# riveSunder/therldaisyworld

Hardware: AMD Instinct MI355X
Metric: cell-updates/sec (grid x batch), fused stencil+growth step (higher is better)
Workload: dtype f32

## Files before the change

### therldaisyworld_amd/csrc/dw_api.hip

```cpp
#include <hip/hip_runtime.h>

#include <cmath>
#include <cstdarg>
#include <cstdio>
#include <cstdlib>
#include <cstring>
#include <memory>
#include <new>
#include <optional>
#include <type_traits>
#include <vector>

#include "../../include/daisyworld_hip.h"
#include "dw_kernels.hpp"
#include "dw_host_util.hpp"
#include "dw_plan.hpp"
#include "dw_series.hpp"
#include "dw_episode_staging.hpp"

using namespace dw;

static thread_local char g_err[512] = "";

static int fail(int code, const char* fmt, ...) {
    va_list ap;
    va_start(ap, fmt);
    vsnprintf(g_err, sizeof(g_err), fmt, ap);
    va_end(ap);
    return code;
}

#define HIPCHK(expr)                                                                           \
    do {                                                                                       \
        hipError_t e_ = (expr);                                                                \
        if (e_ != hipSuccess)                                                                  \
            return fail(e_ == hipErrorOutOfMemory ? DW_ENOMEM : DW_EHIP, "%s failed: %s (%s:%d)", \
                        #expr, hipGetErrorString(e_), __FILE__, __LINE__);                      \
    } while (0)

#define NEED(cond, code, ...)                      \
    do {                                           \
        if (!(cond)) return fail(code, __VA_ARGS__); \
    } while (0)

enum UnqKind { UNQ_F64 = 1, UNQ_F32 = 2 };
enum UnqOwner { OWN_NONE = 0, OWN_CUR = 1, OWN_PREV = 2 };

static thread_local int t_fail_in = 0;
struct DeviceMem {
    static int alloc(void** p, size_t n) {
        if (t_fail_in > 0 && --t_fail_in == 0) return hipErrorOutOfMemory;
        return hipMalloc(p, n);
    }
    static int release(void* p) { return hipFree(p); }
};
struct PinnedMem {
    static int alloc(void** p, size_t n) { return hipHostMalloc(p, n, hipHostMallocDefault); }
    static int release(void* p) { return hipHostFree(p); }
};
template <class T> using DevBuf = Buf<T, DeviceMem>;
template <class T> using PinnedBuf = Buf<T, PinnedMem>;

struct dw_handle {
    dw_params prm;
    hipStream_t stream = nullptr;
    bool own_stream = false;
    size_t cells = 0;
    DevBuf<plane_t> L16[2];
    DevBuf<plane_t> D16[2];
    int cur = 0;
    DevBuf<double> L64;
    DevBuf<double> D64;
    DevBuf<float> U32L;
    DevBuf<float> U32D;
    UnqKind unq_kind = UNQ_F64;
    UnqOwner unq = OWN_NONE;
    bool have_state = false;
    bool stepped = false;
    double L_last = 0.0;
    bool L_per_world = false;
    bool P_per_world = false;
    DevBuf<int> idx;
    DevBuf<double> st;
    DevBuf<int> action;
    DevBuf<int> action_tmp;
    bool have_agents = false;
    DevBuf<StatsDev> stats2[2];
    size_t stats_bytes = 0;
    int sp = 0;
    DevBuf<uint4> fixq;
    unsigned int qcap = 0;
    DevBuf<int> redo_tiles;
    Switches sw{};
    StepPlan plan{};
    DevBuf<int> done_at;
    DevBuf<int> agents_done_at;
    DevBuf<int> n_alive;
    DevBuf<double> scratch;
    DevBuf<unsigned char> ep_buf;
    DevBuf<double> mlp_w;
    int mlp_members = 0;
    PinnedBuf<unsigned char> ep_pinned;
    DevBuf<double> reward_d;
    DevBuf<unsigned char> done_d;
    hipEvent_t ev0 = nullptr, ev1 = nullptr;
    hipEvent_t evf0 = nullptr, evf1 = nullptr;
    int fused_launches = 0;
    DevBuf<StatsDev> side_stats;
    DevBuf<StatsDev> trace_d;
    DevBuf<TempStatsDev> temp_d;
    DevBuf<TempPartial> temp_part;
    DevBuf<unsigned char> pw_tab;
    PinnedBuf<unsigned char> pw_pinned;
    PinnedBuf<unsigned char> pinned;
    struct Snapshot {
        DevBuf<plane_t> L, D;
        DevBuf<plane_t> PL, PD;
        bool stepped = false;
        double L_last = 0.0;
        bool L_per_world = false, P_per_world = false;
        UnqOwner unq = OWN_NONE;
        DevBuf<int> idx;
        DevBuf<double> st;
        DevBuf<unsigned char> stats;
        bool valid = false, agents = false;
    } snap[DW_SNAPSHOT_SLOTS];
    std::vector<std::pair<const void*, size_t>> lds_limit;
    bool created = false;
};

static inline bool cur_quantised(const dw_handle* h) { return h->unq != OWN_CUR; }

static inline bool lacks_shared_L(const dw_handle* h) { return h->stepped && h->L_per_world; }
#define NEED_SHARED_L(h, what)                                                                                          \
    NEED(!lacks_shared_L(h), DW_ESTATE,                                                                                 \
         "%s derives its temperature channels from the last step's luminosity, and the last step "                      \
         "(dw_step_n_trace_per_world) took a per-world luminosity: take a shared-L step or upload a state first", what)
static inline bool lacks_shared_constants(const dw_handle* h) { return lacks_shared_L(h) && h->P_per_world; }
#define NEED_SHARED_CONSTANTS(h, what)                                                                                  \
    NEED(!lacks_shared_constants(h), DW_ESTATE,                                                                         \
         "%s evaluates the last step's input state with one set of constants, and the last step "                       \
         "(dw_step_n_trace_ensemble) took per-world constants: take a shared-L step or upload a state first", what)

template <int V> using int_c = std::integral_constant<int, V>;

template <int V, int... Vs, class F>
static decltype(auto) with_int(int v, F&& f) {
    if constexpr (sizeof...(Vs) == 0) return f(int_c<V>{});
    else return v == V ? f(int_c<V>{}) : with_int<Vs...>(v, f);
}

template <class F>
static decltype(auto) with_bool(bool b, F&& f) { return b ? f(std::true_type{}) : f(std::false_type{}); }

template <class P> using elem_t = std::remove_cv_t<std::remove_pointer_t<P>>;

template <class F>
static decltype(auto) with_unq_planes(const dw_handle* h, F&& f) {
    return h->unq_kind == UNQ_F64 ? f(h->L64.get(), h->D64.get()) : f(h->U32L.get(), h->U32D.get());
}

template <class F>
static decltype(auto) with_planes(const dw_handle* h, bool unq, int buf, F&& f) {
    return unq ? with_unq_planes(h, f) : f(h->L16[buf].get(), h->D16[buf].get());
// ... 225 lines not shown
    }
    return DW_OK;
}

static dim3 generic_grid(const dw_params& p, int* cpt) {
    *cpt = generic_cells_per_thread(p.batch, (long long)p.height * p.width);
    return dim3((unsigned)(((long long)p.height * p.width + 256LL * *cpt - 1) / (256LL * *cpt)), (unsigned)p.batch);
}

template <class T, int PREC>
static auto launch_generic(dw_handle* h, const T* iL, const T* iD, const StepOut& o, const FirstStepBound& fb = {}) {
    const dw_params& p = h->prm;
    int cpt;
    const dim3 grid = generic_grid(p, &cpt);
    hipLaunchKernelGGL((step_generic<T, PREC>), grid, dim3(256), 0, h->stream, iL, iD, o.L, o.D, p.height, p.width, o.P, o.P64,
                       o.stats, o.fixups, o.zero_me, o.zero_n, cpt, fb);
}

static int launch_first_step(dw_handle* h, double L, const StepOut& o) {
    const StepPlan& pl = h->plan;
    const FirstStepBound fb = pl.first_prec == 3 ? derive_first_bound(h->prm, L, o.P, h->unq_kind == UNQ_F64, h->sw.first_slack)
                                                 : FirstStepBound{};
    if (pl.first_stream) {
        const dim3 grid((unsigned)((pl.first_geom.nstrips + 3) / 4));
        with_unq_planes(h, [&](auto* iL, auto* iD) {
            with_int<1, 3>(pl.first_prec, [&](auto PR) {
                with_int<0, 1, 2, 3>(pl.halo, [&](auto HL) {
                    hipLaunchKernelGGL((step_first_stream<elem_t<decltype(iL)>, PR, HL>), grid, dim3(256), 0, h->stream, iL, iD,
                                       o.L, o.D, pl.first_geom, o.P, o.P64, o.stats, o.fixups, o.zero_me, o.zero_n, fb);
                });
            });
        });
    } else {
        with_unq_planes(h, [&](auto* iL, auto* iD) {
            with_int<1, 3, 2>(pl.first_prec, [&](auto PR) { launch_generic<elem_t<decltype(iL)>, PR>(h, iL, iD, o, fb); });
        });
    }
    HIPCHK(hipGetLastError());
    return DW_OK;
}

static int launch_step(dw_handle* h, const StepOut& o) {
    const dw_params& p = h->prm;
    const StepPlan& pl = h->plan;
    const plane_t* iL = h->L16[h->cur].get();
    const plane_t* iD = h->D16[h->cur].get();
    const bool ex = p.precision == DW_PRECISION_EXACT;
    if (pl.kind == STEP_GENERIC) {
        const int prec = p.precision == DW_PRECISION_F64 ? 2 : (ex ? 0 : 1);
        with_int<2, 0, 1>(prec, [&](auto PR) { launch_generic<plane_t, PR>(h, iL, iD, o); });
    } else if (pl.kind == STEP_STREAM && ex) {
        const StreamExactArgs A{iL, iD, o.L, o.D, pl.sgeom, o.P, o.stats, o.fixups, o.zero_me, o.zero_n, o.P64};
        with_int<0, 1, 2, 3>(pl.halo, [&](auto HL) {
            with_bool(pl.sym_albedo, [&](auto SYM) {
                hipLaunchKernelGGL((step_stream_exact<HL, SYM>), dim3((unsigned)pl.sgeom.chunk * 8u), dim3(256), 0, h->stream, A);
            });
        });
    } else if (pl.kind == STEP_STREAM) {
        with_int<0, 1, 2, 3>(pl.halo, [&](auto HL) {
            hipLaunchKernelGGL((step_stream_fast<HL>), dim3((unsigned)pl.sgeom.chunk * 8u), dim3(256), 0, h->stream, iL, iD, o.L,
                               o.D, pl.sgeom, o.P, o.P64, o.stats, o.fixups, o.zero_me, o.zero_n);
        });
    } else {
        FixQ fq;
        fq.entries = h->fixq.get();
        fq.counts = reinterpret_cast<unsigned int*>(o.stats + p.batch + 1);
        fq.qcap = h->qcap;
        fq.redo_tiles = h->redo_tiles.get();
        auto tiled = [&](auto TCQ, auto RPT) {
            return with_bool(ex, [&](auto EX) { return launch_tiled<TCQ, RPT, EX>(h, iL, iD, o, fq); });
        };
        if (pl.tcq == 64) return with_int<8, 4, 2>(pl.rpt, [&](auto RPT) { return tiled(int_c<64>{}, RPT); });
        return pl.tcq == 32 ? tiled(int_c<32>{}, int_c<4>{}) : tiled(int_c<16>{}, int_c<2>{});
    }
    HIPCHK(hipGetLastError());
    return DW_OK;
}

static void step_done(dw_handle* h, double L, bool stepped, bool per_world = false, bool per_world_constants = false) {
    h->cur = 1 - h->cur;
    h->sp = 1 - h->sp;
    h->unq = h->unq == OWN_CUR ? OWN_PREV : OWN_NONE;
    h->stepped = stepped;
    h->L_last = L;
    h->L_per_world = per_world;
    h->P_per_world = per_world && per_world_constants;
    release_unquantised(h);
}

static void episode_done(dw_handle* h, double L_last, bool per_world) {
    h->unq = OWN_NONE;
    h->stepped = true;
    h->L_last = per_world ? 0.0 : L_last;
    h->L_per_world = per_world;
    h->P_per_world = per_world;
}

static int launch_forward(dw_handle* h, double L) {
    const dw_params& p = h->prm;
    NEED(h->have_state, DW_ESTATE, "no state uploaded (call dw_upload_state_* or dw_init_random)");
    StepOut o = step_out(h);
    o.P = derive_f32(p, L);
    o.P64 = make_f64(p, L);
#ifdef DW_TUNING
    if (const char* e = std::getenv("DW_ABLATE")) {
        if (std::strcmp(e, "copy") == 0) {
            const int in = h->cur;
            const size_t n4 = h->cells * sizeof(plane_t) / 16;
            hipLaunchKernelGGL(copy_planes, dim3((unsigned)((n4 + 255) / 256)), dim3(256), 0, h->stream,
                               reinterpret_cast<const float4*>(h->L16[in].get()), reinterpret_cast<const float4*>(h->D16[in].get()),
                               reinterpret_cast<float4*>(o.L), reinterpret_cast<float4*>(o.D), n4);
            HIPCHK(hipGetLastError());
            step_done(h, L, true);
            return DW_OK;
        }
        const int v = std::strcmp(e, "nomath") == 0 ? 1 : 0;
        HIPCHK(hipMemcpyToSymbolAsync(HIP_SYMBOL(g_ablate), &v, sizeof(int), 0, hipMemcpyHostToDevice, h->stream));
    }
#endif
    if (int rc = h->unq == OWN_CUR ? launch_first_step(h, L, o) : launch_step(h, o)) return rc;
    step_done(h, L, true);
    return DW_OK;
}

static int launch_forward_pw(dw_handle* h, const PhysF32* row32, const PhysF64* row64, const FirstStepBound* rowfb, bool sym,
                             bool constants) {
    const dw_params& p = h->prm;
    const StepPlan& pl = h->plan;
    const StepOut o = step_out(h);
    const bool ex = p.precision == DW_PRECISION_EXACT;
    auto generic = [&](auto* iL, auto* iD, auto PR) {
        int cpt;
        const dim3 grid = generic_grid(p, &cpt);
        hipLaunchKernelGGL((step_generic_pw<elem_t<decltype(iL)>, PR>), grid, dim3(256), 0, h->stream, iL, iD, o.L, o.D,
                           p.height, p.width, row32, row64, rowfb, o.stats, o.fixups, o.zero_me, o.zero_n, cpt);
    };
    const plane_t* iL = h->L16[h->cur].get();
    const plane_t* iD = h->D16[h->cur].get();
    if (h->unq == OWN_CUR) {
        with_unq_planes(h, [&](auto* uL, auto* uD) {
            with_int<1, 3, 2>(pl.first_prec, [&](auto PR) { generic(uL, uD, PR); });
        });
    } else if (pl.pw_stream && ex) {
        const StreamExactPwArgs A{iL, iD, o.L, o.D, pl.sgeom, row32, row64, o.stats, o.fixups, o.zero_me, o.zero_n};
        with_int<0, 1, 2>(pl.halo, [&](auto HL) {
            with_bool(sym, [&](auto SYM) {
                hipLaunchKernelGGL((step_stream_exact_pw<HL, SYM>), dim3((unsigned)pl.sgeom.chunk * 8u), dim3(256), 0, h->stream, A);
            });
        });
    } else if (pl.pw_stream) {
        with_int<0, 1, 2>(pl.halo, [&](auto HL) {
            hipLaunchKernelGGL((step_stream_fast_pw<HL>), dim3((unsigned)pl.sgeom.chunk * 8u), dim3(256), 0, h->stream, iL, iD, o.L,
                               o.D, pl.sgeom, row32, row64, o.stats, o.fixups, o.zero_me, o.zero_n);
        });
    } else {
        const int prec = p.precision == DW_PRECISION_F64 ? 2 : (ex ? 0 : 1);
        with_int<2, 0, 1>(prec, [&](auto PR) { generic(iL, iD, PR); });
    }
    HIPCHK(hipGetLastError());
    step_done(h, 0.0, true, true, constants);
    return DW_OK;
}

static int launch_forward_fused2_pw(dw_handle* h, const PairPw* row, StatsDev* trace) {
    const StepPlan& pl = h->plan;
    const StepOut o = step_out(h);
    const FusedGeom& g = pl.fgeom;
    const dim3 grid((unsigned)g.chunk * 8u);
    const plane_t *inL = h->L16[h->cur].get(), *inD = h->D16[h->cur].get();
    with_int<kFusedRot, kFusedOvl>(pl.fused_mode, [&](auto MODE) {
        hipLaunchKernelGGL((trace_pair_fast_pw<MODE>), grid, dim3(256), 0, h->stream, inL, inD, o.L, o.D, g, row, o.zero_me,
                           o.zero_n, trace);
    });
    HIPCHK(hipGetLastError());
    step_done(h, 0.0, false, true, true);
    return DW_OK;
}

static int temp_chunks(const dw_handle* h) {
    return (int)(((long long)h->prm.height * h->prm.width + kTempChunk - 1) / kTempChunk);
}
static size_t temp_part_bytes(const dw_handle* h) { return sizeof(TempPartial) * (size_t)h->prm.batch * temp_chunks(h); }

static int launch_temp_moments(dw_handle* h, bool current, double L, const PhysF64* row64, TempStatsDev* out) {
    const dw_params& p = h->prm;
    const int chunks = temp_chunks(h);
    const PhysF64 P = row64 ? PhysF64{} : make_f64(p, L);
    TempPartial* part = h->temp_part.get();
    auto reduce = [&](auto* iL, auto* iD) {
        with_bool(row64 != nullptr, [&](auto TABLE) {
            hipLaunchKernelGGL((temp_moments_pw<elem_t<decltype(iL)>, TABLE>), dim3((unsigned)chunks, (unsigned)p.batch), dim3(256),
                               0, h->stream, iL, iD, p.height, p.width, P, row64, part);
        });
    };
    if (current) with_planes(h, h->unq == OWN_CUR, h->cur, reduce);
    else with_derived_from(h, [&](auto* iL, auto* iD, auto) { reduce(iL, iD); });
    HIPCHK(hipGetLastError());
    hipLaunchKernelGGL(temp_moments_finish_pw, dim3((unsigned)((p.batch + 63) / 64)), dim3(64), 0, h->stream, part, p.batch, chunks,
                       (double)p.height * (double)p.width, out);
    HIPCHK(hipGetLastError());
    return DW_OK;
}

template <class F>
static auto with_fused_layout(const StepPlan& pl, F&& f) {
    if (pl.packed) return f(int_c<kFusedRot>{}, std::true_type{});
    return with_int<kFusedRot, kFusedRing, kFusedOvl>(pl.fused_mode, [&](auto MODE) { return f(MODE, std::false_type{}); });
}

static int launch_forward_fused2(dw_handle* h, double L1, double L2, unsigned int* pstats = nullptr,
                                 float thr_hi = 0.f, StatsDev* trace = nullptr) {
    const dw_params& p = h->prm;
    const StepPlan& pl = h->plan;
    const bool exact = p.precision == DW_PRECISION_EXACT;
    PhysF32 P1, P2;
    if (exact) derive_f32_pair(p, L1, L2, &P1, &P2);
    else { P1 = derive_f32(p, L1); P2 = derive_f32(p, L2); }
    const StepOut o = step_out(h);
    const FusedGeom& g = pl.fgeom;
    const dim3 grid((unsigned)g.chunk * 8u);
    const plane_t *inL = h->L16[h->cur].get(), *inD = h->D16[h->cur].get();
    auto exact_args = [&] {
        return FusedExactArgs{inL, inD, o.L, o.D, g, P1, lum_part(P2), o.zero_me, o.zero_n, pstats, thr_hi, make_f64(p, L1), L1, L2};
    };
    if (trace && exact) {
        const TraceExactArgs A{exact_args(), trace, h->sw.force_rescan ? 1 : 0};
        with_int<kFusedRot, kFusedOvl>(pl.fused_mode, [&](auto MODE) {
            with_bool(pl.sym_albedo, [&](auto SYM) {
                hipLaunchKernelGGL((trace_pair_exact<MODE, SYM>), grid, dim3(256), 0, h->stream, A);
            });
        });
    } else if (trace) {
        with_int<kFusedRot, kFusedOvl>(pl.fused_mode, [&](auto MODE) {
            hipLaunchKernelGGL((trace_pair_fast<MODE>), grid, dim3(256), 0, h->stream, inL, inD, o.L, o.D, g, P1, P2, o.zero_me,
                               o.zero_n, trace);
        });
    } else if (pl.seam_strips && !pstats && !exact) {
        const FusedGeom &gs = pl.seam_geom, &gl = pl.left_geom;
        hipLaunchKernelGGL(step_stream_fused2_seam_pw, dim3((unsigned)gs.chunk * 8u), dim3(256), 0, h->stream, inL, inD, o.L, o.D,
                           gs, P1, P2, o.zero_me, o.zero_n);
        if (gl.nstrips)
            hipLaunchKernelGGL(step_stream_fused2_left_pw, dim3((unsigned)gl.chunk * 8u), dim3(256), 0, h->stream, inL, inD, o.L,
                               o.D, gl, P1, P2, o.zero_me, 0);
    } else if (pl.fmt_planes && !pstats && !exact) {
        hipLaunchKernelGGL((step_stream_fused2_fmt_pw<kFusedOvl>), grid, dim3(256), 0, h->stream, inL, inD, o.L, o.D, g, P1, P2,
                           o.zero_me, o.zero_n);
    } else if (exact) {
        const FusedExactArgs A = exact_args();
        with_bool(pstats != nullptr, [&](auto STATS) {
            with_fused_layout(pl, [&](auto MODE, auto PACK) {
                with_bool(pl.sym_albedo, [&](auto SYM) {
                    hipLaunchKernelGGL((step_stream_fused2_exact<MODE, PACK, STATS, SYM>), grid, dim3(256), 0, h->stream, A);
                });
            });
        });
    } else {
        with_bool(pstats != nullptr, [&](auto STATS) {
            with_fused_layout(pl, [&](auto MODE, auto PACK) {
                hipLaunchKernelGGL((step_stream_fused2<MODE, PACK, STATS>), grid, dim3(256), 0, h->stream, inL, inD, o.L, o.D, g,
                                   P1, P2, o.zero_me, o.zero_n, pstats, thr_hi);
            });
        });
    }
    HIPCHK(hipGetLastError());
    step_done(h, L2, false);
    return DW_OK;
}

static int launch_agents(dw_handle* h, const int* d_action, int act_b, int act_n, bool standalone = false,
                         double* d_reward = nullptr, unsigned char* d_done = nullptr, unsigned char* d_ok = nullptr) {
    const dw_params& p = h->prm;
    if (p.n_agents == 0) return DW_OK;
    NEED(h->have_state, DW_ESTATE, "no state uploaded");
    NEED(h->have_agents, DW_ESTATE, "no agents uploaded (call dw_upload_agents or dw_init_random)");
    NEED(p.collision_mode == 0 || standalone, DW_EINVAL,
         "collision_mode=1: call dw_update_agents, apply the collision pass (it consumes the caller's RNG) to the "
         "downloaded agent states, upload them, then dw_step without actions");
    const int blocks = (p.batch + 63) / 64;
    with_planes(h, h->unq == OWN_CUR, h->cur, [&](auto* L, auto* D) {
        using T = elem_t<decltype(L)>;
        hipLaunchKernelGGL(agents_update<T>, dim3(blocks), dim3(64), 0, h->stream, L, D, h->idx.get(), h->st.get(), d_action,
                           act_b, act_n, p.batch, p.n_agents, p.height, p.width, p.agent_gamma,
                           p.collision_mode == 0 ? 1 : 0, d_reward, d_done, d_ok);
    });
    HIPCHK(hipGetLastError());
    return DW_OK;
}

static int stage_host_actions(dw_handle* h, const int32_t* action, int b, int n) {
    const dw_params& p = h->prm;
    NEED(b >= 0 && n >= 0 && b <= p.batch && n <= p.n_agents, DW_EINVAL,
         "action block %dx%d exceeds (B,N)=(%d,%d)", b, n, p.batch, p.n_agents);
    if ((size_t)b * n)
        HIPCHK(hipMemcpyAsync(h->action_tmp.get(), action, sizeof(int) * (size_t)b * n, hipMemcpyHostToDevice,
                              h->stream));
    return DW_OK;
}

static int clear_stats(dw_handle* h) {
    for (int i = 0; i < 2; ++i) HIPCHK(hipMemsetAsync(h->stats2[i].get(), 0, h->stats_bytes, h->stream));
    return DW_OK;
}

static void state_arrived(dw_handle* h, UnqOwner unq, UnqKind kind = UNQ_F64) {
    if (unq == OWN_CUR) h->unq_kind = kind;
    h->unq = unq;
    h->have_state = true;
    h->stepped = false;
    for (auto& sn : h->snap) sn.valid = false;
}

template <class T>
static auto init_random_into(dw_handle* h, uint64_t seed, T* L, T* D) {
    const dw_params& p = h->prm;
    if (int crc = clear_stats(h)) return crc;
    const int ncell = p.height * p.width;
    const dim3 g((unsigned)((ncell + kInitChunk - 1) / kInitChunk), (unsigned)p.batch);
    hipLaunchKernelGGL((init_random_cells<T>), g, dim3(256), 0, h->stream, L, D, ncell,
                       (long long)p.world_offset, (unsigned long long)seed, (float)p.light_proportion,
                       (float)p.dark_proportion, (float)p.initial_al, (float)p.initial_ad, h->stats2[h->sp].get());
    HIPCHK(hipGetLastError());
    if (p.n_agents) {
        const int bn = p.batch * p.n_agents;
        hipLaunchKernelGGL(init_random_agents, dim3((bn + 255) / 256), dim3(256), 0, h->stream, h->idx.get(), h->st.get(),
                           p.batch, p.n_agents, p.height, p.width, (long long)p.world_offset,
                           (unsigned long long)seed);
        HIPCHK(hipGetLastError());
    }
    h->have_agents = true;
    return (int)DW_OK;
}

extern "C" {

const char* dw_last_error(void) { return g_err; }
int dw_abi_version(void) { return DW_ABI_VERSION; }

int dw_pinned_alloc(size_t bytes, void** out) {
    NEED(out && bytes > 0, DW_EINVAL, "null argument");
    int ndev = 0;
    NEED(hipGetDeviceCount(&ndev) == hipSuccess && ndev > 0, DW_ENODEVICE, "no HIP device");
    HIPCHK(hipHostMalloc(out, bytes, hipHostMallocDefault));
    return DW_OK;
}
int dw_pinned_free(void* p) {
    if (p) HIPCHK(hipHostFree(p));
    return DW_OK;
}

#ifndef DW_BUILD_ID
#define DW_BUILD_ID "unknown"
#endif
static const char kBuildId[] = "DW_BUILD_ID=" DW_BUILD_ID;
const char* dw_build_id(void) { return kBuildId + 12; }

int dw_default_params(dw_params* p, int32_t batch, int32_t height, int32_t width, int32_t n_agents) {
    NEED(p, DW_EINVAL, "null params");
    std::memset(p, 0, sizeof(*p));
    p->abi_version = DW_ABI_VERSION;
    p->batch = batch; p->height = height; p->width = width; p->n_agents = n_agents;
    p->device = 0; p->precision = DW_PRECISION_EXACT; p->obs_mask = 0x0BA; p->collision_mode = 0;
    p->world_offset = 0;
    p->p = 1.0; p->g = 0.003265; p->S = 1000.0; p->sigma = 5.67e-8; p->gamma = 0.25;
    p->q = 0.2 * p->S / p->sigma; p->q2 = p->q / 8.0; p->dt = 1.0;
    p->albedo_bare = 0.5; p->albedo_light = 0.75; p->albedo_dark = 0.25; p->temp_optimal = 295.5;
    p->agent_gamma = 0.05; p->food_chain_penalty = 0.5;
    p->initial_al = 0.2; p->initial_ad = 0.2; p->light_proportion = 0.33; p->dark_proportion = 0.33;
    return DW_OK;
}

static int check_params(const dw_params* p) {
    NEED(p, DW_EINVAL, "null params");
    NEED(p->abi_version == DW_ABI_VERSION, DW_EINVAL, "ABI version %d != %d", p->abi_version, DW_ABI_VERSION);
    NEED(p->batch >= 1 && p->height >= 3 && p->width >= 3, DW_EINVAL,
         "need batch>=1 and grid >= 3x3 (got B=%d H=%d W=%d)", p->batch, p->height, p->width);
    NEED(p->height <= 65535 && p->width <= 65532, DW_EINVAL, "grid dimension too large");
    NEED((long long)p->height * p->width <= 0x7fffffffLL, DW_EINVAL,
         "a world of %dx%d cells exceeds the 2^31-1 cells per world the kernels index", p->height, p->width);
    NEED(p->n_agents >= 0, DW_EINVAL, "n_agents < 0");
    NEED(p->precision >= 0 && p->precision <= 2, DW_EINVAL, "bad precision %d", p->precision);
    NEED(p->precision == DW_PRECISION_F64 || p->g >= 0.0, DW_EINVAL,
         "g < 0 (a growth curve opening upwards) is evaluated by DW_PRECISION_F64 only");
    NEED((double)p->batch * p->height * p->width < 9.0e18, DW_EINVAL, "too many cells");
    return DW_OK;
}

int dw_create(const dw_params* p, dw_handle** out) {
    NEED(out, DW_EINVAL, "null out");
    *out = nullptr;
    int rc = check_params(p);
    if (rc) return rc;
    int ndev = 0;
    if (hipGetDeviceCount(&ndev) != hipSuccess || ndev <= 0)
        return fail(DW_ENODEVICE, "no HIP device available (this library has no CPU fallback)");
    NEED(p->device >= 0 && p->device < ndev, DW_ENODEVICE, "device %d out of range (%d devices)", p->device, ndev);
    HIPCHK(hipSetDevice(p->device));
    hipDeviceProp_t prop;
    HIPCHK(hipGetDeviceProperties(&prop, p->device));
    if (std::strncmp(prop.gcnArchName, "gfx950", 6) != 0)
        return fail(DW_ENODEVICE, "device %d is %s; this library is built for gfx950 only", p->device,
                    prop.gcnArchName);
    std::unique_ptr<dw_handle, int (*)(dw_handle*)> h(new (std::nothrow) dw_handle(), dw_destroy);
    NEED(h, DW_ENOMEM, "host allocation failed");
    h->prm = *p;
    h->cells = (size_t)p->batch * p->height * p->width;
    HIPCHK(hipStreamCreateWithFlags(&h->stream, hipStreamNonBlocking));
    h->own_stream = true;
    const size_t bn = (size_t)p->batch * (p->n_agents > 0 ? p->n_agents : 1);
    const size_t pb = sizeof(plane_t) * h->cells;
    h->stats_bytes = sizeof(StatsDev) * (p->batch + 1) + sizeof(unsigned int) * (kNumQueues + 1) * 16;
    if (int rc = alloc_group(h.get(), "the handle's state",
                             {{h->L16[0], pb}, {h->D16[0], pb}, {h->L16[1], pb}, {h->D16[1], pb},
                              {h->idx, sizeof(int) * bn * 2}, {h->st, sizeof(double) * bn}, {h->action, sizeof(int) * bn},
                              {h->action_tmp, sizeof(int) * bn}, {h->reward_d, sizeof(double) * bn}, {h->done_d, bn},
                              {h->agents_done_at, sizeof(int) * bn}, {h->done_at, sizeof(int) * p->batch},
                              {h->n_alive, sizeof(int)}, {h->stats2[0], h->stats_bytes}, {h->stats2[1], h->stats_bytes},
                              {h->side_stats, sizeof(StatsDev) * (p->batch + 1)}}))
        return rc;
    for (int i = 0; i < 2; ++i) HIPCHK(hipMemsetAsync(h->stats2[i].get(), 0, h->stats_bytes, h->stream));
    h->sw = read_switches();
    h->plan = plan_steps(*p, h->sw);
    if (int rc = ensure_fixq(h.get(), h->plan)) return rc;
    HIPCHK(hipMemsetAsync(h->action.get(), 0, sizeof(int) * bn, h->stream));
    HIPCHK(hipMemsetAsync(h->done_at.get(), 0, sizeof(int) * p->batch, h->stream));
    HIPCHK(hipMemsetAsync(h->agents_done_at.get(), 0, sizeof(int) * bn, h->stream));
    HIPCHK(hipMemsetAsync(h->n_alive.get(), 0, sizeof(int), h->stream));
    HIPCHK(hipEventCreate(&h->ev0));
    HIPCHK(hipEventCreate(&h->ev1));
    HIPCHK(hipEventCreate(&h->evf0));
    HIPCHK(hipEventCreate(&h->evf1));
    h->created = true;
    *out = h.release();
    return DW_OK;
}

int dw_destroy(dw_handle* h) {
    if (!h) return DW_OK;
    (void)hipSetDevice(h->prm.device);
    if (h->stream) (void)hipStreamSynchronize(h->stream);
    if (h->ev0) (void)hipEventDestroy(h->ev0);
    if (h->ev1) (void)hipEventDestroy(h->ev1);
    if (h->evf0) (void)hipEventDestroy(h->evf0);
    if (h->evf1) (void)hipEventDestroy(h->evf1);
    if (h->own_stream && h->stream) (void)hipStreamDestroy(h->stream);
    delete h;
    return DW_OK;
}

int dw_set_params(dw_handle* h, const dw_params* p) {
    NEED(h, DW_EINVAL, "null handle");
    int rc = check_params(p);
    if (rc) return rc;
    const dw_params& o = h->prm;
    NEED(p->batch == o.batch && p->height == o.height && p->width == o.width && p->n_agents == o.n_agents &&
             p->device == o.device,
         DW_EINVAL, "dw_set_params cannot change shape or device; create a new handle");
    HIPCHK(hipSetDevice(p->device));
    const StepPlan plan = plan_steps(*p, h->sw);
    if ((rc = ensure_fixq(h, plan))) return rc;
    h->prm = *p;
    h->plan = plan;
    return DW_OK;
}

int dw_get_params(const dw_handle* h, dw_params* out) {
    NEED(h && out, DW_EINVAL, "null argument");
    *out = h->prm;
    return DW_OK;
}


static int refresh_stats(dw_handle* h) {
    const dw_params& p = h->prm;
    if (int rc = clear_stats(h)) return rc;
    const int n = p.height * p.width;
    const dim3 g((unsigned)((n + kInitChunk - 1) / kInitChunk), (unsigned)p.batch);
    auto reduce = [&](auto* L, auto* D) {
        hipLaunchKernelGGL((stats_only<elem_t<decltype(L)>>), g, dim3(256), 0, h->stream, L, D, n, h->stats2[h->sp].get());
    };
    if (cur_quantised(h)) reduce(h->L16[h->cur].get(), h->D16[h->cur].get());
    else with_unq_planes(h, reduce);
    HIPCHK(hipGetLastError());
    return DW_OK;
}

int dw_upload_state_f64(dw_handle* h, const double* light, const double* dark) {
    NEED(h && light && dark, DW_EINVAL, "null argument");
    HIPCHK(hipSetDevice(h->prm.device));
    if (int arc = ensure_f64(h)) return arc;
    HIPCHK(hipMemcpyAsync(h->L64.get(), light, sizeof(double) * h->cells, hipMemcpyHostToDevice, h->stream));
    HIPCHK(hipMemcpyAsync(h->D64.get(), dark, sizeof(double) * h->cells, hipMemcpyHostToDevice, h->stream));
    state_arrived(h, OWN_CUR, UNQ_F64);
    int rc = refresh_stats(h);
    if (rc) return rc;
    HIPCHK(hipStreamSynchronize(h->stream));
    return DW_OK;
}

int dw_upload_state_f32(dw_handle* h, const float* light, const float* dark, int quantised) {
    NEED(h && light && dark, DW_EINVAL, "null argument");
    HIPCHK(hipSetDevice(h->prm.device));
    const unsigned blocks = (unsigned)((h->cells + 255) / 256);
    if (quantised) {
        int rc = ensure_scratch(h, sizeof(float) * 2 * h->cells);
        if (rc) return rc;
        float* sL = reinterpret_cast<float*>(h->scratch.get());
        float* sD = sL + h->cells;
        HIPCHK(hipMemcpyAsync(sL, light, sizeof(float) * h->cells, hipMemcpyHostToDevice, h->stream));
        HIPCHK(hipMemcpyAsync(sD, dark, sizeof(float) * h->cells, hipMemcpyHostToDevice, h->stream));
        hipLaunchKernelGGL(f32nat_to_plane, dim3(blocks), dim3(256), 0, h->stream, sL, h->L16[h->cur].get(), h->cells);
        hipLaunchKernelGGL(f32nat_to_plane, dim3(blocks), dim3(256), 0, h->stream, sD, h->D16[h->cur].get(), h->cells);
        HIPCHK(hipGetLastError());
        state_arrived(h, OWN_NONE);
    } else {
        int rc = ensure_u32(h);
        if (rc) return rc;
        HIPCHK(hipMemcpyAsync(h->U32L.get(), light, sizeof(float) * h->cells, hipMemcpyHostToDevice, h->stream));
        HIPCHK(hipMemcpyAsync(h->U32D.get(), dark, sizeof(float) * h->cells, hipMemcpyHostToDevice, h->stream));
        hipLaunchKernelGGL(f32nat_to_permille, dim3(blocks), dim3(256), 0, h->stream, h->U32L.get(), h->U32L.get(), h->cells);
        hipLaunchKernelGGL(f32nat_to_permille, dim3(blocks), dim3(256), 0, h->stream, h->U32D.get(), h->U32D.get(), h->cells);
        HIPCHK(hipGetLastError());
        state_arrived(h, OWN_CUR, UNQ_F32);
    }
    int rc = refresh_stats(h);
    if (rc) return rc;
    HIPCHK(hipStreamSynchronize(h->stream));
    return DW_OK;
}

int dw_upload_agents(dw_handle* h, const int32_t* indices, const double* states) {
    NEED(h, DW_EINVAL, "null handle");
    const dw_params& p = h->prm;
    HIPCHK(hipSetDevice(p.device));
    const size_t bn = (size_t)p.batch * p.n_agents;
    if (bn) {
        NEED(indices && states, DW_EINVAL, "null argument");
        for (size_t i = 0; i < bn; ++i) {
            NEED(indices[2 * i] >= 0 && indices[2 * i] < p.height && indices[2 * i + 1] >= 0 &&
                     indices[2 * i + 1] < p.width,
                 DW_EINVAL, "agent %zu position (%d,%d) outside the %dx%d grid", i, indices[2 * i],
                 indices[2 * i + 1], p.height, p.width);
        }
        HIPCHK(hipMemcpyAsync(h->idx.get(), indices, sizeof(int) * bn * 2, hipMemcpyHostToDevice, h->stream));
        HIPCHK(hipMemcpyAsync(h->st.get(), states, sizeof(double) * bn, hipMemcpyHostToDevice, h->stream));
        HIPCHK(hipStreamSynchronize(h->stream));
    }
    h->have_agents = true;
    return DW_OK;
}

int dw_download_agents(dw_handle* h, int32_t* indices, double* states) {
    NEED(h, DW_EINVAL, "null handle");
    const dw_params& p = h->prm;
    HIPCHK(hipSetDevice(p.device));
    const size_t bn = (size_t)p.batch * p.n_agents;
    if (bn) {
        NEED(h->have_agents, DW_ESTATE, "no agents");
        if (indices) HIPCHK(hipMemcpyAsync(indices, h->idx.get(), sizeof(int) * bn * 2, hipMemcpyDeviceToHost, h->stream));
        if (states) HIPCHK(hipMemcpyAsync(states, h->st.get(), sizeof(double) * bn, hipMemcpyDeviceToHost, h->stream));
    }
    HIPCHK(hipStreamSynchronize(h->stream));
    return DW_OK;
}

int dw_init_random(dw_handle* h, uint64_t seed) {
    NEED(h, DW_EINVAL, "null handle");
    HIPCHK(hipSetDevice(h->prm.device));
    if (int rc = ensure_u32(h)) return rc;
    if (int rc = init_random_into(h, seed, h->U32L.get(), h->U32D.get())) return rc;
    state_arrived(h, OWN_CUR, UNQ_F32);
    return DW_OK;
}

int dw_init_random_quantised(dw_handle* h, uint64_t seed) {
    NEED(h, DW_EINVAL, "null handle");
    HIPCHK(hipSetDevice(h->prm.device));
    if (int rc = init_random_into(h, seed, h->L16[h->cur].get(), h->D16[h->cur].get())) return rc;
    state_arrived(h, OWN_NONE);
    release_unquantised(h);
    return DW_OK;
}

int dw_download_planes(dw_handle* h, int which, double* light, double* dark) {
    NEED(h, DW_EINVAL, "null handle");
    NEED(h->have_state, DW_ESTATE, "no state");
    HIPCHK(hipSetDevice(h->prm.device));
    NEED(which == DW_STATE_CURRENT || which == DW_STATE_PREVIOUS, DW_EINVAL, "bad state selector");
    NEED(which == DW_STATE_CURRENT || h->stepped, DW_ESTATE, "no previous state before the first step");
    const int buf = which == DW_STATE_CURRENT ? h->cur : 1 - h->cur;
    const bool unq = (which == DW_STATE_CURRENT && h->unq == OWN_CUR) || (which == DW_STATE_PREVIOUS && h->unq == OWN_PREV);
    const size_t bytes = sizeof(double) * h->cells;
    if (unq && h->unq_kind == UNQ_F64) {
        if (light) HIPCHK(hipMemcpyAsync(light, h->L64.get(), bytes, hipMemcpyDeviceToHost, h->stream));
        if (dark) HIPCHK(hipMemcpyAsync(dark, h->D64.get(), bytes, hipMemcpyDeviceToHost, h->stream));
    } else {
        int rc = ensure_scratch(h, bytes);
        if (rc) return rc;
        const unsigned blocks = (unsigned)((h->cells + 255) / 256);
        for (int pl = 0; pl < 2; ++pl) {
            double* dst = pl == 0 ? light : dark;
            if (!dst) continue;
            if (unq)
                hipLaunchKernelGGL((plane_to_f64<float>), dim3(blocks), dim3(256), 0, h->stream,
                                   pl == 0 ? h->U32L.get() : h->U32D.get(), h->scratch.get(), h->cells);
            else
                hipLaunchKernelGGL((plane_to_f64<plane_t>), dim3(blocks), dim3(256), 0, h->stream,
                                   pl == 0 ? h->L16[buf].get() : h->D16[buf].get(), h->scratch.get(), h->cells);
            HIPCHK(hipGetLastError());
            HIPCHK(hipMemcpyAsync(dst, h->scratch.get(), bytes, hipMemcpyDeviceToHost, h->stream));
        }
    }
    HIPCHK(hipStreamSynchronize(h->stream));
    return DW_OK;
}

static int run_materialise(dw_handle* h, double L, double* d_grid7, double* d_temps, double* d_betas,
                           double* d_growth, double* d_teff) {
    const dw_params& p = h->prm;
    const dim3 g((unsigned)((p.height * p.width + 255) / 256), (unsigned)p.batch);
    const PhysF64 P = make_f64(p, h->stepped && !h->L_per_world ? h->L_last : L);
    const plane_t* cL = h->L16[h->cur].get();
    const plane_t* cD = h->D16[h->cur].get();
    with_derived_from(h, [&](auto* pL, auto* pD, auto POST) {
        hipLaunchKernelGGL((materialise<elem_t<decltype(pL)>, POST>), g, dim3(256), 0, h->stream, pL, pD, cL, cD, p.height,
                           p.width, P, d_grid7, d_temps, d_betas, d_growth, d_teff);
    });
    HIPCHK(hipGetLastError());
    if (h->stepped && d_grid7 && p.n_agents && h->have_agents) {
        hipLaunchKernelGGL(agents_stamp, dim3((p.batch + 63) / 64), dim3(64), 0, h->stream, d_grid7, h->idx.get(),
                           h->st.get(), p.batch, p.n_agents, p.height, p.width);
        HIPCHK(hipGetLastError());
    }
    return DW_OK;
}

int dw_download_grid(dw_handle* h, double L_init, double* grid7) {
    NEED(h && grid7, DW_EINVAL, "null argument");
    NEED(h->have_state, DW_ESTATE, "no state");
    NEED_SHARED_L(h, "dw_download_grid");
    HIPCHK(hipSetDevice(h->prm.device));
    const size_t bytes = sizeof(double) * 7 * h->cells;
    int rc = ensure_scratch(h, bytes);
    if (rc) return rc;
    rc = run_materialise(h, L_init, h->scratch.get(), nullptr, nullptr, nullptr, nullptr);
    if (rc) return rc;
    HIPCHK(hipMemcpyAsync(grid7, h->scratch.get(), bytes, hipMemcpyDeviceToHost, h->stream));
    HIPCHK(hipStreamSynchronize(h->stream));
    return DW_OK;
}

int dw_download_caches(dw_handle* h, double L, double* temps, double* betas, double* growth,
                       double* temp_effective) {
    NEED(h, DW_EINVAL, "null handle");
    NEED(h->have_state, DW_ESTATE, "no state");
    NEED_SHARED_CONSTANTS(h, "dw_download_caches");
    HIPCHK(hipSetDevice(h->prm.device));
    const size_t n = h->cells;
    int rc = ensure_scratch(h, sizeof(double) * 9 * n);
    if (rc) return rc;
    double* d_t = h->scratch.get();
    double* d_b = d_t + 3 * n;
    double* d_g = d_b + 3 * n;
    double* d_e = d_g + 2 * n;
    rc = run_materialise(h, L, nullptr, temps ? d_t : nullptr, betas ? d_b : nullptr, growth ? d_g : nullptr,
                         temp_effective ? d_e : nullptr);
    if (rc) return rc;
    if (temps) HIPCHK(hipMemcpyAsync(temps, d_t, sizeof(double) * 3 * n, hipMemcpyDeviceToHost, h->stream));
    if (betas) HIPCHK(hipMemcpyAsync(betas, d_b, sizeof(double) * 3 * n, hipMemcpyDeviceToHost, h->stream));
    if (growth) HIPCHK(hipMemcpyAsync(growth, d_g, sizeof(double) * 2 * n, hipMemcpyDeviceToHost, h->stream));
    if (temp_effective) HIPCHK(hipMemcpyAsync(temp_effective, d_e, sizeof(double) * n, hipMemcpyDeviceToHost, h->stream));
    HIPCHK(hipStreamSynchronize(h->stream));
    return DW_OK;
}

int dw_reduce_temperature(dw_handle* h, double L, dw_temp_stats* per_world) {
    NEED(h && per_world, DW_EINVAL, "null argument");
    NEED(h->have_state, DW_ESTATE, "no state");
    NEED_SHARED_CONSTANTS(h, "dw_reduce_temperature");
    static_assert(sizeof(dw_temp_stats) == sizeof(TempStatsDev), "temperature record layout");
    HIPCHK(hipSetDevice(h->prm.device));
    const size_t bytes = sizeof(TempStatsDev) * (size_t)h->prm.batch;
    if (int rc = alloc_group(h, "the temperature reduction", {{h->temp_part, temp_part_bytes(h)}, {h->temp_d, bytes}})) return rc;
    if (int rc = launch_temp_moments(h, false, h->stepped && !h->L_per_world ? h->L_last : L, nullptr, h->temp_d.get())) return rc;
    HIPCHK(hipMemcpyAsync(per_world, h->temp_d.get(), bytes, hipMemcpyDeviceToHost, h->stream));
    HIPCHK(hipStreamSynchronize(h->stream));
    return DW_OK;
}


int dw_update_agents(dw_handle* h, const int32_t* action, int32_t action_b, int32_t action_n) {
    NEED(h && action, DW_EINVAL, "null argument");
    HIPCHK(hipSetDevice(h->prm.device));
    int rc = stage_host_actions(h, action, action_b, action_n);
    if (rc) return rc;
    return launch_agents(h, h->action_tmp.get(), action_b, action_n, true);
}

int dw_step(dw_handle* h, const int32_t* action, int32_t action_b, int32_t action_n, double L) {
    NEED(h, DW_EINVAL, "null handle");
    HIPCHK(hipSetDevice(h->prm.device));
    if (action) {
        int rc = stage_host_actions(h, action, action_b, action_n);
        if (rc) return rc;
        rc = launch_agents(h, h->action_tmp.get(), action_b, action_n);
        if (rc) return rc;
    }
    return launch_forward(h, L);
}

int dw_step_device_actions(dw_handle* h, double L) {
    NEED(h, DW_EINVAL, "null handle");
    HIPCHK(hipSetDevice(h->prm.device));
    int rc = launch_agents(h, h->action.get(), h->prm.batch, h->prm.n_agents);
    if (rc) return rc;
    return launch_forward(h, L);
}

int dw_upload_actions(dw_handle* h, const int32_t* action) {
    NEED(h && action, DW_EINVAL, "null argument");
    HIPCHK(hipSetDevice(h->prm.device));
    const size_t bn = (size_t)h->prm.batch * h->prm.n_agents;
    if (bn) {
        HIPCHK(hipMemcpyAsync(h->action.get(), action, sizeof(int) * bn, hipMemcpyHostToDevice, h->stream));
        HIPCHK(hipStreamSynchronize(h->stream));
    }
    return DW_OK;
}

int dw_download_actions(dw_handle* h, int32_t* action) {
    NEED(h && action, DW_EINVAL, "null argument");
    HIPCHK(hipSetDevice(h->prm.device));
    const size_t bn = (size_t)h->prm.batch * h->prm.n_agents;
    if (bn) HIPCHK(hipMemcpyAsync(action, h->action.get(), sizeof(int) * bn, hipMemcpyDeviceToHost, h->stream));
    HIPCHK(hipStreamSynchronize(h->stream));
    return DW_OK;
}

int dw_step_n(dw_handle* h, int32_t nsteps, double* L_io, double dL, double min_L, double max_L,
              int use_device_actions) {
    NEED(h && L_io, DW_EINVAL, "null argument");
    NEED(nsteps >= 0, DW_EINVAL, "nsteps < 0");
    HIPCHK(hipSetDevice(h->prm.device));
    double L = *L_io;
    auto advance = [&]() { L += dL; L = L > max_L ? max_L : L; L = L < min_L ? min_L : L; };
    int s0 = 0;
    h->fused_launches = 0;
    if (!use_device_actions && nsteps >= 1 && h->have_state && !cur_quantised(h)) {
        int rc = launch_forward(h, L);
        if (rc) return rc;
        advance();
        s0 = 1;
    }
    const bool big_packed = h->plan.allow_fuse && h->plan.packed && h->cells >= ((size_t)1 << 23);
    if (!use_device_actions && nsteps - s0 > 1 && h->have_state && h->prm.height * h->prm.width <= 4096 && !big_packed &&
        episode_kernel_applies(h)) {
        std::vector<double> Ls;
        while (s0 < nsteps) {
            const int k = nsteps - s0 < 4096 ? nsteps - s0 : 4096;
            Ls.resize(k);
            for (int i = 0; i < k; ++i) { Ls[i] = L; advance(); }
            int rc = run_episode_impl(h, k, Ls.data(), kPolicySkipAgents, nullptr, nullptr, 5, nullptr, nullptr);
            if (rc) return rc;
            s0 += k;
        }
        *L_io = L;
        return DW_OK;
    }
    if (!use_device_actions && h->plan.allow_fuse && h->have_state && nsteps - s0 >= 3) {
        drop_unquantised_previous(h);
        HIPCHK(hipEventRecord(h->evf0, h->stream));
        int launched = 0;
        while (nsteps - s0 >= 3) {
            const double L1 = L;
            advance();
            const double L2 = L;
            advance();
            int rc = launch_forward_fused2(h, L1, L2);
            if (rc) return rc;
            s0 += 2;
            launched += 1;
        }
        HIPCHK(hipEventRecord(h->evf1, h->stream));
        h->fused_launches = launched;
    }
    for (int s = s0; s < nsteps; ++s) {
        int rc;
        if (use_device_actions) {
            rc = launch_agents(h, h->action.get(), h->prm.batch, h->prm.n_agents);
            if (rc) return rc;
        }
        rc = launch_forward(h, L);
        if (rc) return rc;
        advance();
    }
    *L_io = L;
    return DW_OK;
}

static bool ensemble_pairs(const dw_handle* h) { return h->plan.trace_pairs && h->prm.precision == DW_PRECISION_FAST; }

static int check_per_world(const WorldRows& rows, const dw_world_params* worlds, const double* L_schedule, size_t nsteps, size_t B) {
    for (size_t i = 0; i < nsteps * B; ++i)
        NEED(std::isfinite(L_schedule[i]) && L_schedule[i] >= 0.0, DW_EINVAL,
             "L_schedule[step %zu][world %zu] = %g: a luminosity is finite and not negative", i / B, i % B, L_schedule[i]);
    for (size_t b = 0; worlds && b < B; ++b) {
        if (check_params(&rows.params(b)) != DW_OK) {
            char why[sizeof(g_err)];
            snprintf(why, sizeof(why), "%s", g_err);
            return fail(DW_EINVAL, "worlds[%zu].g = %g: %s", b, worlds[b].g, why);
        }
    }
    return DW_OK;
}

struct PwTable {
    dw_handle* h;
    const PwLayout lay;
    hipEvent_t uploaded = nullptr;
    bool in_flight = false;
    PwTable(dw_handle* h_, const PwLayout& lay_) : h(h_), lay(lay_) {}
    PwTable(const PwTable&) = delete;
    ~PwTable() { if (uploaded) (void)hipEventDestroy(uploaded); }
    unsigned char* img() const { return h->pw_pinned.get(); }
    unsigned char* dev() const { return h->pw_tab.get(); }
    GroupItem<DeviceMem> item() const { return {h->pw_tab, lay.bytes}; }
    int alloc(const char* what, std::initializer_list<GroupItem<DeviceMem>> group) {
        if (int rc = alloc_group(h, what, group)) return rc;
        if (int rc = reserve(h->pw_pinned, "the page-locked image of the per-world constants", lay.bytes)) {
            h->pw_tab.reset();
            return rc;
        }
        HIPCHK(hipEventCreateWithFlags(&uploaded, hipEventDisableTiming));
        return DW_OK;
    }
    int next_chunk(const SeriesSchedule& q, size_t c, const double* Ls, WorldRows& worlds, bool first_bound = false) {
        if (in_flight) HIPCHK(hipEventSynchronize(uploaded));
        fill_chunk(q, c, Ls, worlds, lay, img());
        if (first_bound) worlds.first_bound(Ls, lay.p32(img(), 0), h->unq_kind == UNQ_F64, h->sw.first_slack, lay.fb(img()));
        auto part = [&](size_t off, size_t bytes) { return hipMemcpyAsync(dev() + off, img() + off, bytes, hipMemcpyHostToDevice, h->stream); };
        const size_t singles = q.chunks[c].singles, pairs = q.chunks[c].pairs;
        if (singles) {
            HIPCHK(part(0, sizeof(PhysF32) * singles * lay.B));
            HIPCHK(part(lay.o64, sizeof(PhysF64) * singles * lay.B));
        }
        if (first_bound) HIPCHK(part(lay.ofb, sizeof(FirstStepBound) * lay.B));
        if (pairs) HIPCHK(part(lay.opair, sizeof(PairPw) * pairs * lay.B));
        HIPCHK(hipEventRecord(uploaded, h->stream));
        in_flight = true;
        return DW_OK;
    }
};

struct SeriesRun {
    dw_handle* h;
    const SeriesSchedule& q;
    const double* Ls;
    dw_world_stats* trace;
    dw_temp_stats* temps;
    PwTable* table;
    bool sym, constants;
    size_t B, row_bytes, trow_bytes;
    bool first_pair = true;
    bool keep_rows() const { return trace || q.even; }

    int alloc() {
        const GroupItem<DeviceMem> tr{h->trace_d, keep_rows() ? q.rows * row_bytes : 0}, part{h->temp_part, temp_part_bytes(h)},
            td{h->temp_d, q.rows * trow_bytes};
        if (!table) return temps ? alloc_group(h, "the trace buffer and the temperature reduction", {tr, part, td})
                                 : alloc_group(h, "the trace buffer", {tr});
        if (temps) return table->alloc("the per-world constants, the trace buffer and the temperature reduction", {table->item(), tr, part, td});
        return keep_rows() ? table->alloc("the per-world constants and the trace buffer", {table->item(), tr})
                           : table->alloc("the per-world constants", {table->item()});
    }
    int step(int t) {
        const size_t sr = (size_t)t % q.rows, tr = table ? q.row_of[(size_t)t] : 0;
        StatsDev* row = keep_rows() ? h->trace_d.get() + sr * B : nullptr;
        unsigned char* tab = table ? table->dev() : nullptr;
        if (q.is_pair[(size_t)t]) {
            if (first_pair) drop_unquantised_previous(h);
            first_pair = false;
            return table ? launch_forward_fused2_pw(h, table->lay.pair(tab, tr), row)
                         : launch_forward_fused2(h, Ls[t], Ls[t + 1], nullptr, 0.f, row);
        }
        const PhysF64* r64 = table ? table->lay.p64(tab, tr) : nullptr;
        if (temps)
            if (int rc = launch_temp_moments(h, true, table ? 0.0 : Ls[t], r64, h->temp_d.get() + sr * B)) return rc;
        if (int rc = table ? launch_forward_pw(h, table->lay.p32(tab, tr), r64, table->lay.fb(tab), sym, constants)
                           : launch_forward(h, Ls[t])) return rc;
        if (row) HIPCHK(hipMemcpyAsync(row, h->stats2[h->sp].get(), row_bytes, hipMemcpyDeviceToDevice, h->stream));
        return DW_OK;
    }
    int run(WorldRows* worlds) {
        const int nsteps = (int)q.is_pair.size();
        const bool first_bound = h->unq == OWN_CUR && h->plan.first_prec == 3;
        size_t c = 0;
        for (int t = 0; t < nsteps; t += q.took(t)) {
            const size_t sr = (size_t)t % q.rows, left = (size_t)(nsteps - t), filled = sr + (size_t)q.took(t);
            if (table && t == (c ? q.chunks[c - 1].end : 0)) {
                if (int rc = table->next_chunk(q, c, Ls, *worlds, c == 0 && first_bound)) return rc;
                ++c;
            }
            if (q.even && sr == 0)
                HIPCHK(hipMemsetAsync(h->trace_d.get(), 0, (left < q.rows ? left : q.rows) * row_bytes, h->stream));
            if (int rc = step(t)) return rc;
            if (filled != q.rows && t + q.took(t) != nsteps) continue;
            const size_t r0 = ((size_t)t - sr) * B;
            if (temps) HIPCHK(hipMemcpyAsync(temps + r0, h->temp_d.get(), filled * trow_bytes, hipMemcpyDeviceToHost, h->stream));
            if (trace) HIPCHK(hipMemcpyAsync(trace + r0, h->trace_d.get(), filled * row_bytes, hipMemcpyDeviceToHost, h->stream));
        }
        return DW_OK;
    }
};

enum SeriesForm { SHARED_L, PER_WORLD_L, PER_WORLD_CONSTANTS };
static int run_series(dw_handle* h, int32_t nsteps, const double* L_schedule, dw_world_stats* trace, dw_temp_stats* temps,
                      bool always_even, bool may_pair, SeriesForm form = SHARED_L, const dw_world_params* worlds = nullptr) {
    const bool pw = form != SHARED_L;
    NEED(nsteps >= 0, DW_EINVAL, "nsteps < 0");
    if (nsteps == 0) return DW_OK;
    NEED(h->have_state, DW_ESTATE, "no state uploaded (call dw_upload_state_* or dw_init_random)");
    static_assert(sizeof(dw_world_stats) == sizeof(StatsDev), "stats layout");
    static_assert(sizeof(dw_temp_stats) == sizeof(TempStatsDev), "temperature record layout");
    const dw_params& p = h->prm;
    const size_t B = (size_t)p.batch;
    std::unique_ptr<WorldRows> rows(pw ? new WorldRows(p, worlds, B) : nullptr);
    if (int rc = pw ? check_per_world(*rows, worlds, L_schedule, (size_t)nsteps, B) : DW_OK) return rc;
    const bool sym = worlds ? worlds_symmetric(worlds, B) && !h->sw.no_sym : h->plan.sym_albedo;
    HIPCHK(hipSetDevice(p.device));
    const SeriesSchedule q = plan_series(SeriesSpec{nsteps, B, sizeof(StatsDev), sizeof(TempStatsDev), h->sw.trace_rows, always_even,
                                                    may_pair, cur_quantised(h), temps != nullptr, pw ? L_schedule : nullptr});
    std::unique_ptr<PwTable> table(pw ? new PwTable(h, PwLayout(B, q.trows, q.prows)) : nullptr);
    SeriesRun run{h, q, L_schedule, trace, temps, table.get(), sym, form == PER_WORLD_CONSTANTS, B, sizeof(StatsDev) * B, sizeof(TempStatsDev) * B};
    if (int rc = run.alloc()) return rc;
    SyncOnExit sync(h->stream);
    h->fused_launches = 0;
    if (int rc = run.run(rows.get())) return rc;
    HIPCHK(hipStreamSynchronize(h->stream));
    sync.disarm();
    return DW_OK;
}

int dw_step_n_trace(dw_handle* h, int32_t nsteps, const double* L_schedule, dw_world_stats* trace) {
    NEED(h && L_schedule && trace, DW_EINVAL, "null argument");
    return run_series(h, nsteps, L_schedule, trace, nullptr, true, h->plan.trace_pairs);
}

int dw_step_n_trace_per_world(dw_handle* h, int32_t nsteps, const double* L_schedule, dw_world_stats* trace) {
    NEED(h && L_schedule, DW_EINVAL, "null argument");
    return run_series(h, nsteps, L_schedule, trace, nullptr, false, false, PER_WORLD_L);
}

int dw_world_params_of(const dw_handle* h, dw_world_params* out) {
    NEED(h && out, DW_EINVAL, "null argument");
    *out = world_params_of(h->prm);
    return DW_OK;
}

int dw_step_n_trace_ensemble(dw_handle* h, int32_t nsteps, const dw_world_params* worlds, const double* L_schedule,
                             dw_world_stats* trace, dw_temp_stats* temps) {
    static_assert(sizeof(dw_world_params) == 96, "dw_world_params layout");
    NEED(h && worlds && L_schedule, DW_EINVAL, "null argument");
    return run_series(h, nsteps, L_schedule, trace, temps, false, ensemble_pairs(h), PER_WORLD_CONSTANTS, worlds);
}

int dw_step_n_trace_temperature(dw_handle* h, int32_t nsteps, const double* L_schedule, int per_world, dw_world_stats* trace,
                                dw_temp_stats* temps) {
    NEED(h && L_schedule && temps, DW_EINVAL, "null argument");
    return run_series(h, nsteps, L_schedule, trace, temps, false, false, per_world ? PER_WORLD_L : SHARED_L);
}

int dw_last_step_n_timing(dw_handle* h, float* fused_ms, int32_t* fused_launches, int32_t* plane_elem_bytes) {
    NEED(h && fused_ms && fused_launches && plane_elem_bytes, DW_EINVAL, "null argument");
    HIPCHK(hipSetDevice(h->prm.device));
    *fused_ms = 0.f;
    *fused_launches = h->fused_launches;
    *plane_elem_bytes = (int32_t)sizeof(plane_t);
    if (h->fused_launches > 0) {
        HIPCHK(hipEventSynchronize(h->evf1));
        HIPCHK(hipEventElapsedTime(fused_ms, h->evf0, h->evf1));
    }
    return DW_OK;
}

int dw_forward_f64(dw_handle* h, const double* light, const double* dark, double L, double* grid7,
                   double* temps, double* betas, double* growth, double* temp_effective) {
    NEED(h && light && dark && grid7, DW_EINVAL, "null argument");
    const dw_params& p = h->prm;
    HIPCHK(hipSetDevice(p.device));
    const size_t n = h->cells;
    int rc = ensure_scratch(h, sizeof(double) * 18 * n + sizeof(plane_t) * 2 * n + 16);
    if (rc) return rc;
    double* dL = h->scratch.get();
    double* dD = dL + n;
    double* dG = dD + n;
    double* d_t = dG + 7 * n;
    double* d_b = d_t + 3 * n;
    double* d_g = d_b + 3 * n;
    double* d_e = d_g + 2 * n;
    plane_t* nL = reinterpret_cast<plane_t*>(d_e + n);
    plane_t* nD = nL + n;
    StatsDev* tmp_stats = h->side_stats.get();
    HIPCHK(hipMemsetAsync(tmp_stats, 0, sizeof(StatsDev) * (p.batch + 1), h->stream));
    HIPCHK(hipMemcpyAsync(dL, light, sizeof(double) * n, hipMemcpyHostToDevice, h->stream));
    {
        const hipError_t e2 = hipMemcpyAsync(dD, dark, sizeof(double) * n, hipMemcpyHostToDevice, h->stream);
        if (e2 != hipSuccess) {
            (void)hipStreamSynchronize(h->stream);
            return fail(DW_EHIP, "dw_forward_f64: %s", hipGetErrorString(e2));
        }
    }
    const PhysF32 P = derive_f32(p, L);
    const PhysF64 P64 = make_f64(p, L);
    const dim3 g((unsigned)((p.height * p.width + 255) / 256), (unsigned)p.batch);
    unsigned long long* tmp_fix = &tmp_stats[p.batch].sum_l;
    hipLaunchKernelGGL((step_generic<double, 2>), g, dim3(256), 0, h->stream, dL, dD, nL, nD, p.height, p.width, P,
                       P64, tmp_stats, tmp_fix, (unsigned long long*)nullptr, 0);
    hipLaunchKernelGGL((materialise<double, true>), g, dim3(256), 0, h->stream, dL, dD, nL, nD, p.height, p.width,
                       P64, dG, temps ? d_t : (double*)nullptr, betas ? d_b : (double*)nullptr,
                       growth ? d_g : (double*)nullptr, temp_effective ? d_e : (double*)nullptr);
    hipError_t le = hipGetLastError();
    if (le == hipSuccess && p.n_agents && h->have_agents) {
        hipLaunchKernelGGL(agents_stamp, dim3((p.batch + 63) / 64), dim3(64), 0, h->stream, dG, h->idx.get(), h->st.get(),
                           p.batch, p.n_agents, p.height, p.width);
        le = hipGetLastError();
    }
    if (le == hipSuccess) le = hipMemcpyAsync(grid7, dG, sizeof(double) * 7 * n, hipMemcpyDeviceToHost, h->stream);
    if (le == hipSuccess && temps) le = hipMemcpyAsync(temps, d_t, sizeof(double) * 3 * n, hipMemcpyDeviceToHost, h->stream);
    if (le == hipSuccess && betas) le = hipMemcpyAsync(betas, d_b, sizeof(double) * 3 * n, hipMemcpyDeviceToHost, h->stream);
    if (le == hipSuccess && growth) le = hipMemcpyAsync(growth, d_g, sizeof(double) * 2 * n, hipMemcpyDeviceToHost, h->stream);
    if (le == hipSuccess && temp_effective)
        le = hipMemcpyAsync(temp_effective, d_e, sizeof(double) * n, hipMemcpyDeviceToHost, h->stream);
    const hipError_t se = hipStreamSynchronize(h->stream);
    if (le == hipSuccess) le = se;
    if (le != hipSuccess) return fail(DW_EHIP, "dw_forward_f64: %s", hipGetErrorString(le));
    return DW_OK;
}

int dw_conv3x3_f64(dw_handle* h, const double* plane, const double kernel[9], double* out) {
    NEED(h && plane && kernel && out, DW_EINVAL, "null argument");
    const dw_params& p = h->prm;
    HIPCHK(hipSetDevice(p.device));
    const size_t n = h->cells;
    int rc = ensure_scratch(h, sizeof(double) * 2 * n);
    if (rc) return rc;
    double* d_in = h->scratch.get();
    double* d_out = d_in + n;
    Kernel9 K;
    for (int i = 0; i < 9; ++i) K.k[i] = kernel[i];
    SyncOnExit guard(h->stream);
    HIPCHK(hipMemcpyAsync(d_in, plane, sizeof(double) * n, hipMemcpyHostToDevice, h->stream));
    const dim3 g((unsigned)((p.height * p.width + 255) / 256), (unsigned)p.batch);
    hipLaunchKernelGGL(conv3x3_f64, g, dim3(256), 0, h->stream, d_in, d_out, p.height, p.width, K);
    HIPCHK(hipGetLastError());
    HIPCHK(hipMemcpyAsync(out, d_out, sizeof(double) * n, hipMemcpyDeviceToHost, h->stream));
    HIPCHK(hipStreamSynchronize(h->stream));
    guard.disarm();
    return DW_OK;
}

int dw_stage_f64(dw_handle* h, int stage, const double* in, double* out, double L, const double kernel[9]) {
    NEED(h && in && out, DW_EINVAL, "null argument");
    NEED(stage >= kStageAlbedo && stage <= kStageGrowth, DW_EINVAL, "bad stage %d", stage);
    NEED(kernel || stage > kStageDensity, DW_EINVAL, "the stencil stages need their 3x3 kernel");
    const dw_params& p = h->prm;
    HIPCHK(hipSetDevice(p.device));
    const size_t n = h->cells, nin = (size_t)stage_inputs(stage), nout = (size_t)stage_outputs(stage);
    int rc = ensure_scratch(h, sizeof(double) * (nin + nout) * n);
    if (rc) return rc;
    double* d_in = h->scratch.get();
    double* d_out = d_in + nin * n;
    Kernel9 K{};
    if (kernel) for (int i = 0; i < 9; ++i) K.k[i] = kernel[i];
    const PhysF64 P = make_f64(p, L);
    SyncOnExit guard(h->stream);
    HIPCHK(hipMemcpyAsync(d_in, in, sizeof(double) * nin * n, hipMemcpyHostToDevice, h->stream));
    const dim3 g((unsigned)((p.height * p.width + 255) / 256), (unsigned)p.batch);
    with_int<kStageAlbedo, kStageDensity, kStageTemperature, kStageGrowthRate, kStageGrowth>(stage, [&](auto S) {
        hipLaunchKernelGGL((stage_f64<S>), g, dim3(256), 0, h->stream, d_in, d_out, p.batch, p.height, p.width, P, K);
    });
    HIPCHK(hipGetLastError());
    HIPCHK(hipMemcpyAsync(out, d_out, sizeof(double) * nout * n, hipMemcpyDeviceToHost, h->stream));
    HIPCHK(hipStreamSynchronize(h->stream));
    guard.disarm();
    return DW_OK;
}

int dw_get_obs(dw_handle* h, double L_init, double* obs) {
    NEED(h, DW_EINVAL, "null handle");
    const dw_params& p = h->prm;
    HIPCHK(hipSetDevice(p.device));
    const size_t bn = (size_t)p.batch * p.n_agents;
    if (bn == 0) return DW_OK;
    NEED(obs, DW_EINVAL, "null obs");
    NEED(h->have_state && h->have_agents, DW_ESTATE, "no state / agents");
    int rc = observe_into_scratch(h, L_init, 0);
    if (rc) return rc;
    HIPCHK(hipMemcpyAsync(obs, h->scratch.get(), sizeof(double) * bn * 63, hipMemcpyDeviceToHost, h->stream));
    HIPCHK(hipStreamSynchronize(h->stream));
    return DW_OK;
}

int dw_env_step(dw_handle* h, const int32_t* action, int32_t action_b, int32_t action_n, double L, double* obs,
                double* reward, uint8_t* done) {
    NEED(h, DW_EINVAL, "null handle");
    const dw_params& p = h->prm;
    HIPCHK(hipSetDevice(p.device));
    const size_t bn = (size_t)p.batch * p.n_agents;
    auto up = [](size_t v) { return (v + 255) / 256 * 256; };
    const bool big_obs = sizeof(double) * bn * 63 > ((size_t)512 << 10);
    const size_t o_act = 0, o_obs = up(sizeof(int) * bn), o_rew = o_obs + sizeof(double) * bn * 63;
    const size_t total = up(o_rew + sizeof(double) * bn + bn) + 256;
    if (int rc = reserve(h->pinned, "the page-locked step staging", total)) return rc;
    if (action) {
        NEED(action_b >= 0 && action_n >= 0 && action_b <= p.batch && action_n <= p.n_agents, DW_EINVAL,
             "action block %dx%d exceeds (B,N)=(%d,%d)", action_b, action_n, p.batch, p.n_agents);
        const size_t na = (size_t)action_b * action_n;
        if (na) {
            std::memcpy(h->pinned.get() + o_act, action, sizeof(int) * na);
            HIPCHK(hipMemcpyAsync(h->action_tmp.get(), h->pinned.get() + o_act, sizeof(int) * na, hipMemcpyHostToDevice, h->stream));
        }
        int rc = launch_agents(h, h->action_tmp.get(), action_b, action_n);
        if (rc) return rc;
    }
    int rc = launch_forward(h, L);
    if (rc) return rc;
    if (bn) {
        NEED(h->have_agents, DW_ESTATE, "no agents");
        const size_t d_rew = sizeof(double) * bn * 63, d_done = d_rew + sizeof(double) * bn, d_total = d_done + bn;
        rc = observe_into_scratch(h, L, d_total - d_rew + 64, true);
        if (rc) return rc;
        unsigned char* blk = reinterpret_cast<unsigned char*>(h->scratch.get());
        if (big_obs) {
            if (obs) HIPCHK(hipMemcpyAsync(obs, blk, d_rew, hipMemcpyDeviceToHost, h->stream));
            HIPCHK(hipMemcpyAsync(h->pinned.get() + o_rew, blk + d_rew, d_total - d_rew, hipMemcpyDeviceToHost, h->stream));
        } else {
            HIPCHK(hipMemcpyAsync(h->pinned.get() + o_obs, blk, d_total, hipMemcpyDeviceToHost, h->stream));
        }
        HIPCHK(hipStreamSynchronize(h->stream));
        const unsigned char* src = big_obs ? h->pinned.get() + o_rew - d_rew : h->pinned.get() + o_obs;
        if (obs && !big_obs) std::memcpy(obs, src, d_rew);
        if (reward) std::memcpy(reward, src + d_rew, sizeof(double) * bn);
        if (done) std::memcpy(done, src + d_done, bn);
    }
    return DW_OK;
}

int dw_get_reward_done(dw_handle* h, double* reward, uint8_t* done) {
    NEED(h, DW_EINVAL, "null handle");
    const dw_params& p = h->prm;
    HIPCHK(hipSetDevice(p.device));
    const int bn = p.batch * p.n_agents;
    if (bn == 0) return DW_OK;
    NEED(h->have_agents, DW_ESTATE, "no agents");
    hipLaunchKernelGGL(reward_done, dim3((bn + 255) / 256), dim3(256), 0, h->stream, h->st.get(), h->reward_d.get(), h->done_d.get(), bn);
    HIPCHK(hipGetLastError());
    if (reward) HIPCHK(hipMemcpyAsync(reward, h->reward_d.get(), sizeof(double) * bn, hipMemcpyDeviceToHost, h->stream));
    if (done) HIPCHK(hipMemcpyAsync(done, h->done_d.get(), (size_t)bn, hipMemcpyDeviceToHost, h->stream));
    HIPCHK(hipStreamSynchronize(h->stream));
    return DW_OK;
}

int dw_reduce(dw_handle* h, dw_world_stats* per_world) {
    NEED(h && per_world, DW_EINVAL, "null argument");
    NEED(h->have_state, DW_ESTATE, "no state");
    static_assert(sizeof(dw_world_stats) == sizeof(StatsDev), "stats layout");
    HIPCHK(hipSetDevice(h->prm.device));
    HIPCHK(hipMemcpyAsync(per_world, h->stats2[h->sp].get(), sizeof(StatsDev) * h->prm.batch, hipMemcpyDeviceToHost,
                          h->stream));
    HIPCHK(hipStreamSynchronize(h->stream));
    return DW_OK;
}

static int launch_policy_greedy(dw_handle* h, int argmin, const int* agent_mode, int codes) {
    const dw_params& p = h->prm;
    const int bn = p.batch * p.n_agents;
    const dim3 g((unsigned)((bn + 255) / 256));
    if (h->unq == OWN_CUR && h->unq_kind == UNQ_F32)
        hipLaunchKernelGGL(policy_greedy<float>, g, dim3(256), 0, h->stream, h->U32L.get(), h->U32D.get(), h->idx.get(), p.batch, p.n_agents,
                           p.height, p.width, p.obs_mask, argmin, agent_mode, h->action.get(), codes);
    else
        hipLaunchKernelGGL(policy_greedy<plane_t>, g, dim3(256), 0, h->stream, h->L16[h->cur].get(), h->D16[h->cur].get(), h->idx.get(),
                           p.batch, p.n_agents, p.height, p.width, p.obs_mask, argmin, agent_mode, h->action.get(), codes);
    HIPCHK(hipGetLastError());
    return DW_OK;
}

int dw_policy_greedy(dw_handle* h, int mode) {
    NEED(h, DW_EINVAL, "null handle");
    const dw_params& p = h->prm;
    HIPCHK(hipSetDevice(p.device));
    const int bn = p.batch * p.n_agents;
    if (bn == 0) return DW_OK;
    NEED(h->have_state && h->have_agents, DW_ESTATE, "no state / agents");
    NEED(mode == DW_POLICY_ARGMAX || mode == DW_POLICY_ARGMIN, DW_EINVAL, "bad policy mode");
    NEED(cur_quantised(h) || h->unq_kind != UNQ_F64, DW_ESTATE,
         "device policy on an exact float64 initial state is not supported; compute the action on the host");
    return launch_policy_greedy(h, mode == DW_POLICY_ARGMIN ? 1 : 0, nullptr, 0);
}

int dw_policy_per_agent(dw_handle* h, const int32_t* agent_mode) {
    NEED(h && agent_mode, DW_EINVAL, "null argument");
    const dw_params& p = h->prm;
    HIPCHK(hipSetDevice(p.device));
    const int bn = p.batch * p.n_agents;
    if (bn == 0) return DW_OK;
    NEED(h->have_state && h->have_agents, DW_ESTATE, "no state / agents");
    NEED(cur_quantised(h) || h->unq_kind != UNQ_F64, DW_ESTATE,
         "device policy on an exact float64 initial state is not supported; compute the action on the host");
    for (int n = 0; n < p.n_agents; ++n)
        NEED(agent_mode[n] == DW_POLICY_ARGMAX || agent_mode[n] == DW_POLICY_ARGMIN || agent_mode[n] == DW_POLICY_TABLE,
             DW_EINVAL, "agent %d: bad policy mode %d", n, agent_mode[n]);
    std::vector<int> m(p.n_agents);
    for (int n = 0; n < p.n_agents; ++n) m[n] = agent_mode[n] == DW_POLICY_TABLE ? 2 : agent_mode[n];
    HIPCHK(hipMemcpyAsync(h->action_tmp.get(), m.data(), sizeof(int) * p.n_agents, hipMemcpyHostToDevice, h->stream));
    const int prc = launch_policy_greedy(h, 0, h->action_tmp.get(), 0);
    HIPCHK(hipStreamSynchronize(h->stream));
    return prc;
}

static int observe_into_scratch(dw_handle* h, double L_init, size_t extra_bytes, bool reward_tail) {
    const dw_params& p = h->prm;
    const size_t bn = (size_t)p.batch * p.n_agents;
    NEED_SHARED_L(h, "an observation");
    int rc = ensure_scratch(h, sizeof(double) * bn * 63 + extra_bytes);
    if (rc) return rc;
    double* d_rew = reward_tail ? h->scratch.get() + bn * 63 : nullptr;
    unsigned char* d_done = reward_tail ? reinterpret_cast<unsigned char*>(h->scratch.get() + bn * 64) : nullptr;
    const int threads = (int)(bn * 9);
    const dim3 g((threads + 127) / 128);
    const PhysF64 P = make_f64(p, h->stepped ? h->L_last : L_init);
    const plane_t* cL = h->L16[h->cur].get();
    const plane_t* cD = h->D16[h->cur].get();
    with_derived_from(h, [&](auto* pL, auto* pD, auto POST) {
        hipLaunchKernelGGL((observe<elem_t<decltype(pL)>, POST>), g, dim3(128), 0, h->stream, pL, pD, cL, cD, h->idx.get(),
                           h->st.get(), p.batch, p.n_agents, p.height, p.width, P, p.obs_mask, h->scratch.get(), d_rew, d_done);
    });
    HIPCHK(hipGetLastError());
    return DW_OK;
}

static int policy_mlp_impl(dw_handle* h, const double* params, int32_t n_members, const int32_t* world_member,
                           int32_t agent_begin, int32_t agent_end, double L_init) {
    const dw_params& p = h->prm;
    NEED(agent_begin >= 0 && agent_begin <= agent_end && agent_end <= p.n_agents, DW_EINVAL, "bad agent range");
    NEED(h->have_state && h->have_agents, DW_ESTATE, "no state / agents");
    const size_t bn = (size_t)p.batch * p.n_agents;
    if (bn == 0 || agent_begin == agent_end) return DW_OK;
    if (world_member)
        for (int b = 0; b < p.batch; ++b)
            NEED(world_member[b] >= 0 && world_member[b] < n_members, DW_EINVAL, "world %d: member %d out of range", b,
                 world_member[b]);
    const size_t wbytes = sizeof(double) * 1808 * (size_t)n_members;
    const size_t mbytes = world_member ? sizeof(int) * (size_t)p.batch : 0;
    int rc = observe_into_scratch(h, L_init, wbytes + mbytes + 16);
    if (rc) return rc;
    double* d_w = h->scratch.get() + bn * 63;
    int* d_m = world_member ? reinterpret_cast<int*>(d_w + 1808 * (size_t)n_members) : nullptr;
    SyncOnExit guard(h->stream);
    HIPCHK(hipMemcpyAsync(d_w, params, wbytes, hipMemcpyHostToDevice, h->stream));
    if (world_member) HIPCHK(hipMemcpyAsync(d_m, world_member, mbytes, hipMemcpyHostToDevice, h->stream));
    const int n = p.batch * (agent_end - agent_begin);
    hipLaunchKernelGGL(policy_mlp, dim3((n + 3) / 4), dim3(64), 0, h->stream, h->scratch.get(), d_w, d_m, p.batch,
                       p.n_agents, agent_begin, agent_end, h->action.get());
    HIPCHK(hipGetLastError());
    HIPCHK(hipStreamSynchronize(h->stream));
    guard.disarm();
    return DW_OK;
}

int dw_policy_mlp(dw_handle* h, const double* params, int32_t n_params, int32_t agent_begin, int32_t agent_end,
                  double L_init) {
    NEED(h && params, DW_EINVAL, "null argument");
    HIPCHK(hipSetDevice(h->prm.device));
    NEED(n_params == 63 * 16 + 16 * 32 + 32 * 9, DW_EINVAL, "the MLP policy has 1808 parameters (63-16-32-9), got %d", n_params);
    return policy_mlp_impl(h, params, 1, nullptr, agent_begin, agent_end, L_init);
}

int dw_policy_mlp_population(dw_handle* h, const double* params, int32_t n_members, const int32_t* world_member,
                             int32_t agent_begin, int32_t agent_end, double L_init) {
    NEED(h && params && world_member, DW_EINVAL, "null argument");
    HIPCHK(hipSetDevice(h->prm.device));
    NEED(n_members >= 1, DW_EINVAL, "n_members < 1");
    return policy_mlp_impl(h, params, n_members, world_member, agent_begin, agent_end, L_init);
}

int dw_run_episode_mlp(dw_handle* h, int32_t nsteps, const double* L_schedule, const double* params, int32_t n_members,
                       const int32_t* member_a, const int32_t* member_b, int32_t split, double L_init, double* reward,
                       uint8_t* done) {
    NEED(h && L_schedule, DW_EINVAL, "null argument");
    const dw_params& p = h->prm;
    HIPCHK(hipSetDevice(p.device));
    NEED(nsteps >= 1 && nsteps <= 4096, DW_EINVAL, "nsteps must be in 1..4096");
    NEED(n_members >= 1, DW_EINVAL, "n_members < 1");
    NEED(params || (h->mlp_w.get() && h->mlp_members == n_members), DW_ESTATE,
         "params == NULL but no parameter sets of %d members are on the device", n_members);
    NEED(p.collision_mode == 0, DW_EINVAL, "collision_mode=1 is not implemented on the device");
    NEED(split >= 0 && split <= p.n_agents, DW_EINVAL, "split outside 0..n_agents");
    NEED(h->have_state && h->have_agents, DW_ESTATE, "no state / agents");
    const int B = p.batch, N = p.n_agents;
    const size_t K = (size_t)nsteps, bn = (size_t)B * N;
    NEED(bn > 0, DW_EINVAL, "no agents");
    for (int b = 0; b < B; ++b) {
        NEED(!member_a || (member_a[b] >= 0 && member_a[b] < n_members), DW_EINVAL, "world %d: member out of range", b);
        NEED(!member_b || (member_b[b] >= 0 && member_b[b] < n_members), DW_EINVAL, "world %d: member out of range", b);
    }
    NEED(n_members == 1 || (member_a && member_b), DW_EINVAL, "several parameter sets need both member maps");
    const size_t wbytes = sizeof(double) * 1808 * (size_t)n_members;
    EpisodeRegions regions;
    regions.rows = K; regions.mlp = true;
    const EpisodeStaging S(K, (size_t)B, (size_t)N, regions);
    using R = EpisodeStaging;
    const size_t o_ma = S.off[R::MEMBER_A], o_mb = S.off[R::MEMBER_B], o_p32 = S.off[R::P32], o_ls = S.off[R::LS];
    if (int erc = ensure_ep_buf(h, S.total)) return erc;
    if (params) {
        if (h->mlp_members != n_members) {
            h->mlp_w.reset();
            h->mlp_members = 0;
            if (int rc = reserve(h->mlp_w, "the parameter sets", wbytes)) return rc;
            h->mlp_members = n_members;
        }
    }
    const double* d_w = h->mlp_w.get();
    const int* d_ma = member_a ? reinterpret_cast<const int*>(h->ep_buf.get() + o_ma) : nullptr;
    const int* d_mb = member_b ? reinterpret_cast<const int*>(h->ep_buf.get() + o_mb) : nullptr;
    double* d_r = S.at<double>(h->ep_buf.get(), R::REWARD);
    unsigned char* d_d = S.at<unsigned char>(h->ep_buf.get(), R::DONE);
    SyncOnExit guard(h->stream);
    if (params) HIPCHK(hipMemcpyAsync(h->mlp_w.get(), params, wbytes, hipMemcpyHostToDevice, h->stream));
    if (member_a) HIPCHK(hipMemcpyAsync(h->ep_buf.get() + o_ma, member_a, sizeof(int) * B, hipMemcpyHostToDevice, h->stream));
    if (member_b) HIPCHK(hipMemcpyAsync(h->ep_buf.get() + o_mb, member_b, sizeof(int) * B, hipMemcpyHostToDevice, h->stream));
    const int Cc = p.height * p.width;
    const int wpb = worlds_per_block(Cc);
    size_t lds = 0;
    const EpisodeForm form = episode_mlp_form(h, &lds);
    const bool wave_kernel = form == EPISODE_WAVE, small = form != EPISODE_STEPWISE;
    std::vector<PhysF32> p32;
    SyncOnExit guard2(h->stream);
    size_t t = 0;
    while (t < K) {
        if (small && cur_quantised(h) && h->stepped && h->unq == OWN_NONE) {
            NEED_SHARED_L(h, "the episode's first observation");
            const size_t Kr = K - t;
            p32.resize(Kr);
            for (size_t i = 0; i < Kr; ++i) p32[i] = derive_f32(p, L_schedule[t + i]);
            HIPCHK(hipMemcpyAsync(h->ep_buf.get() + o_p32, p32.data(), sizeof(PhysF32) * Kr, hipMemcpyHostToDevice, h->stream));
            HIPCHK(hipMemcpyAsync(h->ep_buf.get() + o_ls, L_schedule + t, sizeof(double) * Kr, hipMemcpyHostToDevice, h->stream));
            StatsDev* stats = h->stats2[h->sp].get();
            if (!wave_kernel) HIPCHK(hipMemsetAsync(stats, 0, sizeof(StatsDev) * (B + 1), h->stream));
            EpisodeMlpIO io;
            fill_episode_io(io, h, S);
            io.weights = d_w; io.member_a = d_ma; io.member_b = d_mb;
            io.reward = d_r + t * bn; io.done = d_d + t * bn;
            io.action = h->action.get();
            const bool ex = p.precision == DW_PRECISION_EXACT;
            if (wave_kernel) {
                auto kern = ex ? episode_mlp_wave<true> : episode_mlp_wave<false>;
                if (int rc = set_lds_limit(h, kern, lds)) return rc;
                const EpisodeMlpWaveArgs A{io, B, N, p.height, p.width, (int)Kr, p.obs_mask, (int)split, p.agent_gamma,
                                           h->L_last, make_f64(p, L_schedule[t])};
                hipLaunchKernelGGL(kern, dim3((unsigned)((B + 3) / 4)), dim3(256), lds, h->stream, A);
            } else {
                auto kern = ex ? episode_mlp<true> : episode_mlp<false>;
                if (int rc = set_lds_limit(h, kern, lds)) return rc;
                hipLaunchKernelGGL(kern, dim3((unsigned)((B + wpb - 1) / wpb)), dim3(256), lds, h->stream, io, B, N, p.height,
                                   p.width, wpb, (int)Kr, p.obs_mask, p.agent_gamma, make_f64(p, L_schedule[t]), h->L_last,
                                   (int)split);
            }
            HIPCHK(hipGetLastError());
            h->stepped = true;
            h->L_last = L_schedule[K - 1];
            h->L_per_world = false;
            t = K;
            break;
        }
        int rc = observe_into_scratch(h, L_init, 0);
        if (rc) return rc;
        hipLaunchKernelGGL(policy_mlp, dim3((unsigned)((bn + 3) / 4)), dim3(64), 0, h->stream, h->scratch.get(), d_w, d_ma, B, N,
                           0, N, h->action.get(), d_mb, split);
        HIPCHK(hipGetLastError());
        rc = launch_agents(h, h->action.get(), B, N, false, d_r + t * bn, d_d + t * bn);
        if (rc) return rc;
        rc = launch_forward(h, L_schedule[t]);
        if (rc) return rc;
        ++t;
    }
    if (reward) HIPCHK(hipMemcpyAsync(reward, d_r, sizeof(double) * K * bn, hipMemcpyDeviceToHost, h->stream));
    if (done) HIPCHK(hipMemcpyAsync(done, d_d, K * bn, hipMemcpyDeviceToHost, h->stream));
    HIPCHK(hipStreamSynchronize(h->stream));
    guard2.disarm();
    guard.disarm();
    return DW_OK;
}

int dw_lifespan_reset(dw_handle* h) {
    NEED(h, DW_EINVAL, "null handle");
    const dw_params& p = h->prm;
    HIPCHK(hipSetDevice(p.device));
    const size_t bn = (size_t)p.batch * (p.n_agents > 0 ? p.n_agents : 1);
    HIPCHK(hipMemsetAsync(h->done_at.get(), 0, sizeof(int) * p.batch, h->stream));
    HIPCHK(hipMemsetAsync(h->agents_done_at.get(), 0, sizeof(int) * bn, h->stream));
    HIPCHK(hipMemsetAsync(h->n_alive.get(), 0, sizeof(int), h->stream));
    return DW_OK;
}

int dw_lifespan_accumulate(dw_handle* h, uint32_t threshold_k) {
    NEED(h, DW_EINVAL, "null handle");
    const dw_params& p = h->prm;
    HIPCHK(hipSetDevice(p.device));
    HIPCHK(hipMemsetAsync(h->n_alive.get(), 0, sizeof(int), h->stream));
    const int n = p.batch * (p.n_agents > 0 ? p.n_agents : 1);
    hipLaunchKernelGGL(lifespan_accumulate, dim3((n + 255) / 256), dim3(256), 0, h->stream, h->stats2[h->sp].get(), h->st.get(), p.batch,
                       p.n_agents, threshold_k, h->done_at.get(), h->agents_done_at.get(), h->n_alive.get());
    HIPCHK(hipGetLastError());
    return DW_OK;
}

int dw_lifespan_download(dw_handle* h, int32_t* done_at, int32_t* agents_done_at, int32_t* n_worlds_alive) {
    NEED(h, DW_EINVAL, "null handle");
    const dw_params& p = h->prm;
    HIPCHK(hipSetDevice(p.device));
    if (done_at) HIPCHK(hipMemcpyAsync(done_at, h->done_at.get(), sizeof(int) * p.batch, hipMemcpyDeviceToHost, h->stream));
    if (agents_done_at && p.n_agents)
        HIPCHK(hipMemcpyAsync(agents_done_at, h->agents_done_at.get(), sizeof(int) * (size_t)p.batch * p.n_agents,
                              hipMemcpyDeviceToHost, h->stream));
    if (n_worlds_alive) HIPCHK(hipMemcpyAsync(n_worlds_alive, h->n_alive.get(), sizeof(int), hipMemcpyDeviceToHost, h->stream));
    HIPCHK(hipStreamSynchronize(h->stream));
    return DW_OK;
}

int dw_run_episode(dw_handle* h, int32_t nsteps, const double* L_schedule, int policy_mode,
                   const uint8_t* use_table, const int8_t* table, uint32_t threshold_k, uint8_t* world_alive,
                   uint8_t* agent_ok) {
    NEED(h && L_schedule, DW_EINVAL, "null argument");
    NEED(policy_mode >= 0 && policy_mode <= 3, DW_EINVAL, "bad policy mode");
    return run_episode_impl(h, nsteps, L_schedule, policy_mode, use_table, table, threshold_k, world_alive, agent_ok);
}

static EpisodeForm episode_form(const dw_handle* h) {
    const dw_params& p = h->prm;
    const int C = p.height * p.width, N = p.n_agents;
    if (C > 4096 || p.precision == DW_PRECISION_F64 || p.collision_mode != 0 || h->sw.no_episode_kernel)
        return EPISODE_STEPWISE;
    return C <= kEwMaxCells && N <= 64 && !h->sw.no_episode_wave ? EPISODE_WAVE : EPISODE_WORKGROUP;
}

static EpisodeForm episode_mlp_form(const dw_handle* h, size_t* lds_bytes) {
    const dw_params& p = h->prm;
    const int Cc = p.height * p.width, N = p.n_agents;
    const int wpb = worlds_per_block(Cc);
    const bool wave_kernel = Cc <= kEwMaxCells && 16 * N <= 64 && !h->sw.no_episode_wave;
    const size_t lds = wave_kernel ? episode_wave_shared_bytes() + episode_mlp_wave_world_bytes(Cc, N) * 4
                                   : episode_mlp_world_bytes(Cc, N) * wpb;
    if (lds_bytes) *lds_bytes = lds;
    const bool small = Cc <= 4096 && lds <= 160 * 1024 && p.precision != DW_PRECISION_F64 && p.collision_mode == 0 &&
                       !h->sw.no_episode_kernel;
    return !small ? EPISODE_STEPWISE : (wave_kernel ? EPISODE_WAVE : EPISODE_WORKGROUP);
}

static bool episode_kernel_applies(const dw_handle* h) { return episode_form(h) != EPISODE_STEPWISE && cur_quantised(h); }

static int launch_policy(dw_handle* h, int policy_mode, bool from_table, const unsigned char* codes, unsigned char* d_ok = nullptr) {
    const size_t bn = (size_t)h->prm.batch * h->prm.n_agents;
    if (policy_mode == DW_POLICY_TABLE || from_table) {
        hipLaunchKernelGGL(actions_from_table, dim3((unsigned)((bn + 255) / 256)), dim3(256), 0, h->stream,
                           reinterpret_cast<const signed char*>(codes), (int)bn, h->action.get());
        if (int rc = launch_policy_greedy(h, 0, nullptr, 1)) return rc;
    } else if (policy_mode == DW_POLICY_ZEROS) {
        HIPCHK(hipMemsetAsync(h->action.get(), 0, sizeof(int) * bn, h->stream));
    } else if (int rc = launch_policy_greedy(h, policy_mode == DW_POLICY_ARGMIN ? 1 : 0, nullptr, 0)) {
        return rc;
    }
    HIPCHK(hipGetLastError());
    return launch_agents(h, h->action.get(), h->prm.batch, h->prm.n_agents, false, nullptr, nullptr, d_ok);
}

static EpisodeIO episode_io(const dw_handle* h, int policy_mode, const EpisodeStaging& S, size_t t0, bool wave, bool have_use_table,
                            bool have_table) {
    using R = EpisodeStaging;
    unsigned char* dev = h->ep_buf.get();
    EpisodeIO io{};
    fill_episode_io(io, h, S);
    io.use_table = wave && !have_use_table ? nullptr : dev + S.off[R::USE_TABLE] + t0;
    io.table = wave && !have_table ? nullptr : reinterpret_cast<const signed char*>(dev + S.off[R::TABLE] + t0 * S.bn);
    io.world_alive = dev + S.off[R::WORLD_ALIVE] + t0 * S.B;
    io.agent_ok = dev + S.off[R::AGENT_OK] + t0 * S.bn;
    io.action = (h->prm.n_agents > 0 && policy_mode != kPolicySkipAgents) ? h->action.get() : nullptr;
    return io;
}

static int run_episode_stepwise(dw_handle* h, int32_t nsteps, const double* L_schedule, int policy_mode,
                                const uint8_t* use_table, const int8_t* table, uint32_t threshold_k, uint8_t* world_alive,
                                uint8_t* agent_ok, dw_world_stats* trace, WorldRows* worlds = nullptr, bool sym = false) {
    using R = EpisodeStaging;
    const dw_params& p = h->prm;
    const int N = p.n_agents, B = p.batch;
    const size_t K = (size_t)nsteps, Bz = (size_t)B, bn = Bz * N;
    const bool plain = !trace && !worlds;
    EpisodeRegions regions;
    regions.trace = trace != nullptr; regions.pairs = plain; regions.slack = 256;
    EpisodeBuffers E(h, EpisodeStaging(K, Bz, (size_t)N, regions));
    SeriesSchedule q;
    std::optional<PwTable> tab;
    if (worlds) {
        q = plan_series(SeriesSpec{nsteps, Bz, sizeof(StatsDev), 0, 0, false, false, true, false, L_schedule});
        tab.emplace(h, PwLayout(Bz, q.trows));
    }
    if (int rc = E.alloc(false)) return rc;
    if (tab)
        if (int rc = tab->alloc("the per-world constants", {tab->item()})) return rc;
    SyncOnExit guard(h->stream);
    if (int rc = E.upload(nullptr, 0, true, nullptr, table)) return rc;
    unsigned char* const d_tab = E.dev(R::TABLE);
    unsigned char* const d_wa = E.dev(R::WORLD_ALIVE);
    unsigned char* const d_ok = E.dev(R::AGENT_OK);
    unsigned char* const d_code = E.dev(R::CODE);
    StatsDev* const rows = E.dev<StatsDev>(R::TRACE);
// ... 64 lines not shown
        if (trace)
            hipLaunchKernelGGL(episode_stats_row_pw, dim3((unsigned)((B + 255) / 256)), dim3(256), 0, h->stream,
                               h->stats2[h->sp].get(), B, rows + t * Bz);
        HIPCHK(hipGetLastError());
    }
    if (int rc = E.finish(world_alive, agent_ok, trace)) return rc;
    guard.disarm();
    return DW_OK;
}

static int check_episode_call(const dw_handle* h, int32_t nsteps, int policy_mode, const uint8_t* use_table, const int8_t* table) {
    const dw_params& p = h->prm;
    NEED(nsteps >= 1 && nsteps <= 4096, DW_EINVAL, "nsteps must be in 1..4096");
    NEED(p.precision != DW_PRECISION_F64, DW_EINVAL, "dw_run_episode supports exact and fast precision");
    NEED(p.collision_mode == 0, DW_EINVAL, "collision_mode=1 is not implemented on the device");
    NEED(h->have_state, DW_ESTATE, "no state uploaded");
    NEED(p.n_agents == 0 || h->have_agents, DW_ESTATE, "no agents uploaded");
    NEED(cur_quantised(h), DW_ESTATE, "the current state is not quantised yet; take the first step with dw_step");
    NEED(policy_mode != DW_POLICY_TABLE || table, DW_EINVAL, "DW_POLICY_TABLE needs a table");
    if (use_table && !table)
        for (int t = 0; t < nsteps; ++t) NEED(!use_table[t], DW_EINVAL, "use_table set but no table given");
    return DW_OK;
}

static int run_episode_impl(dw_handle* h, int32_t nsteps, const double* L_schedule, int policy_mode,
                            const uint8_t* use_table, const int8_t* table, uint32_t threshold_k,
                            uint8_t* world_alive, uint8_t* agent_ok, dw_world_stats* trace) {
    const dw_params& p = h->prm;
    HIPCHK(hipSetDevice(p.device));
    if (int rc = check_episode_call(h, nsteps, policy_mode, use_table, table)) return rc;
    const int C = p.height * p.width, N = p.n_agents, B = p.batch;
    const EpisodeForm form = episode_form(h);
    if (form == EPISODE_STEPWISE || (trace && form != EPISODE_WAVE))
        return run_episode_stepwise(h, nsteps, L_schedule, policy_mode, use_table, table, threshold_k, world_alive, agent_ok, trace);
    const bool wave_kernel = form == EPISODE_WAVE;
    const int wpb = worlds_per_block(C);
    const size_t world_bytes = wave_kernel ? episode_wave_world_bytes(C, N) : episode_world_bytes(C, N);
    const size_t lds = trace ? episode_wave_stats_lds_bytes(C, N)
                             : world_bytes * wpb + (wave_kernel ? episode_wave_shared_bytes() : 0);
    NEED(lds <= 160 * 1024, DW_EINVAL, "too many agents for the LDS-resident episode kernel");
    const size_t K = (size_t)nsteps;
    EpisodeRegions regions;
    regions.rows = K; regions.use_table = true; regions.trace = trace != nullptr;
    EpisodeBuffers E(h, EpisodeStaging(K, (size_t)B, (size_t)N, regions));
    if (int rc = E.alloc(E.S.fits_image())) return rc;
    PhysF32* p32 = E.p32();
    for (size_t t = 0; t < K; ++t) p32[t] = derive_f32(p, L_schedule[t]);
    SyncOnExit guard(h->stream);
    if (int rc = E.upload(L_schedule, K, true, use_table, table)) return rc;
    StatsDev* stats = h->stats2[h->sp].get();
    if (!wave_kernel) HIPCHK(hipMemsetAsync(stats, 0, sizeof(StatsDev) * (B + 1), h->stream));
    const EpisodeIO io = episode_io(h, policy_mode, E.S, 0, wave_kernel, use_table != nullptr, table && E.S.bn);
    const PhysF64 P64 = make_f64(p, L_schedule[0]);
    const dim3 grid((unsigned)((B + wpb - 1) / wpb));
    const bool ex = p.precision == DW_PRECISION_EXACT;
    if (trace) {
        auto kern = ex ? episode_wave_stats_pw<true> : episode_wave_stats_pw<false>;
        const EpisodeWaveStatsArgs A{io, E.dev<StatsDev>(EpisodeStaging::TRACE), B, N, p.height, p.width, nsteps,
                                     policy_mode, p.obs_mask, threshold_k, p.agent_gamma, P64};
        hipLaunchKernelGGL(kern, grid, dim3(256), lds, h->stream, A);
    } else if (wave_kernel) {
        auto kern = ex ? episode_wave<true> : episode_wave<false>;
        if (int rc = set_lds_limit(h, kern, lds)) return rc;
        const EpisodeWaveArgs A{io, B, N, p.height, p.width, nsteps, policy_mode, p.obs_mask, threshold_k, p.agent_gamma, P64};
        hipLaunchKernelGGL(kern, grid, dim3(256), lds, h->stream, A);
    } else {
        auto kern = ex ? episode_small<true> : episode_small<false>;
        if (int rc = set_lds_limit(h, kern, lds)) return rc;
        hipLaunchKernelGGL(kern, grid, dim3(256), lds, h->stream, io, B, N, p.height, p.width, wpb, nsteps, policy_mode,
                           p.obs_mask, p.agent_gamma, threshold_k, P64);
    }
    HIPCHK(hipGetLastError());
    episode_done(h, L_schedule[K - 1], false);
    release_unquantised(h);
    if (int rc = E.finish(world_alive, agent_ok, trace)) return rc;
    guard.disarm();
    return DW_OK;
}

int dw_run_episode_trace(dw_handle* h, int32_t nsteps, const double* L_schedule, int policy_mode,
                         const uint8_t* use_table, const int8_t* table, uint32_t threshold_k, uint8_t* world_alive,
                         uint8_t* agent_ok, dw_world_stats* trace) {
    NEED(h && L_schedule, DW_EINVAL, "null argument");
    NEED(trace, DW_EINVAL, "dw_run_episode_trace needs a trace array");
    NEED(policy_mode >= 0 && policy_mode <= 3, DW_EINVAL, "bad policy mode");
    return run_episode_impl(h, nsteps, L_schedule, policy_mode, use_table, table, threshold_k, world_alive, agent_ok, trace);
}

int dw_run_episode_ensemble(dw_handle* h, int32_t nsteps, const dw_world_params* worlds, const double* L_schedule, int policy_mode,
                            const uint8_t* use_table, const int8_t* table, uint32_t threshold_k, uint8_t* world_alive,
                            uint8_t* agent_ok) {
    NEED(h && worlds && L_schedule, DW_EINVAL, "null argument");
    NEED(policy_mode >= 0 && policy_mode <= 3, DW_EINVAL, "bad policy mode");
    const dw_params& p = h->prm;
    HIPCHK(hipSetDevice(p.device));
    if (int rc = check_episode_call(h, nsteps, policy_mode, use_table, table)) return rc;
    const int C = p.height * p.width, N = p.n_agents, B = p.batch;
    const size_t K = (size_t)nsteps, Bz = (size_t)B;
    const bool wave = episode_form(h) == EPISODE_WAVE;
    WorldRows rows_of(p, worlds, Bz, !wave);
    if (int rc = check_per_world(rows_of, worlds, L_schedule, K, Bz)) return rc;
    if (!wave)
        return run_episode_stepwise(h, nsteps, L_schedule, policy_mode, use_table, table, threshold_k, world_alive, agent_ok, nullptr,
                                    &rows_of, worlds_symmetric(worlds, Bz) && !h->sw.no_sym);
    const size_t lds = episode_wave_pw_shared_bytes() + episode_wave_pw_world_bytes(C, N) * 4;
    NEED(lds <= 160 * 1024, DW_EINVAL, "too many agents for the LDS-resident episode kernel");
    const size_t row_bytes = (sizeof(PhysF32) + sizeof(double)) * Bz;
    size_t rows = ((size_t)32 << 20) / row_bytes / kEwSeg * kEwSeg;
    rows = rows < (size_t)kEwSeg ? (size_t)kEwSeg : rows;
    rows = rows > K ? K : rows;
    EpisodeRegions regions;
    regions.rows = rows; regions.per_world = true; regions.use_table = true;
    EpisodeBuffers E(h, EpisodeStaging(K, Bz, (size_t)N, regions));
    if (int rc = E.alloc(true)) return rc;
    SyncOnExit guard(h->stream);
    PhysF64* p64 = E.S.at<PhysF64>(E.img, EpisodeStaging::P64);
    for (size_t b = 0; b < Bz; ++b) p64[b] = make_f64(rows_of.params(b), 0.0);
    const bool ex = p.precision == DW_PRECISION_EXACT;
    auto kern = ex ? episode_wave_pw<true> : episode_wave_pw<false>;
    if (int rc = set_lds_limit(h, kern, lds)) return rc;
    PhysF32* r32 = E.p32();
    for (size_t t0 = 0; t0 < K; t0 += rows) {
        const size_t kk = K - t0 < rows ? K - t0 : rows;
        if (t0) HIPCHK(hipStreamSynchronize(h->stream));
        for (size_t t = 0; t < kk; ++t) rows_of.single(L_schedule + (t0 + t) * Bz, r32 + t * Bz, nullptr);
        if (int rc = E.upload(L_schedule + t0 * Bz, kk * Bz, t0 == 0, use_table, table)) return rc;
        const EpisodeWavePwArgs A{episode_io(h, policy_mode, E.S, t0, true, use_table != nullptr, table && E.S.bn),
                                  E.dev<const PhysF64>(EpisodeStaging::P64), B, N, p.height, p.width, (int)kk, policy_mode,
                                  p.obs_mask, threshold_k, p.agent_gamma};
        hipLaunchKernelGGL(kern, dim3((unsigned)((B + 3) / 4)), dim3(256), lds, h->stream, A);
        HIPCHK(hipGetLastError());
        episode_done(h, 0.0, true);
    }
    release_unquantised(h);
    if (int rc = E.finish(world_alive, agent_ok, nullptr)) return rc;
    guard.disarm();
    return DW_OK;
}

struct CopyJobs {
    const void* src[8];
    void* dst[8];
    unsigned long long bytes[8];
    int n;
};
__global__ __launch_bounds__(256) void copy_regions(CopyJobs J) {
    const size_t stride = (size_t)gridDim.x * blockDim.x, t0 = (size_t)blockIdx.x * blockDim.x + threadIdx.x;
    for (int j = 0; j < J.n; ++j) {
        const size_t nb = J.bytes[j];
        const uint4* s16 = static_cast<const uint4*>(J.src[j]);
        uint4* d16 = static_cast<uint4*>(J.dst[j]);
        for (size_t i = t0; i < nb / 16; i += stride) d16[i] = s16[i];
        const unsigned char* s1 = static_cast<const unsigned char*>(J.src[j]);
        unsigned char* d1 = static_cast<unsigned char*>(J.dst[j]);
        for (size_t i = (nb & ~(size_t)15) + t0; i < nb; i += stride) d1[i] = s1[i];
    }
}
static int launch_copy_regions(dw_handle* h, const CopyJobs& J) {
    size_t most = 0;
    for (int j = 0; j < J.n; ++j) {
        NEED(J.src[j] && J.dst[j], DW_EINVAL, "snapshot region not allocated");
        NEED(((reinterpret_cast<uintptr_t>(J.src[j]) | reinterpret_cast<uintptr_t>(J.dst[j])) & 15) == 0, DW_EINVAL,
             "snapshot region not 16-byte aligned");
        most = J.bytes[j] > most ? J.bytes[j] : most;
    }
    if (J.n == 0 || most == 0) return DW_OK;
    size_t blocks = (most / 16 + 255) / 256;
    blocks = blocks < 1 ? 1 : (blocks > 8192 ? 8192 : blocks);
    hipLaunchKernelGGL(copy_regions, dim3((unsigned)blocks), dim3(256), 0, h->stream, J);
    HIPCHK(hipGetLastError());
    return DW_OK;
}

int dw_snapshot_save_slot(dw_handle* h, int32_t slot) {
    NEED(h, DW_EINVAL, "null handle");
    NEED(slot >= 0 && slot < DW_SNAPSHOT_SLOTS, DW_EINVAL, "snapshot slot out of range");
    const dw_params& p = h->prm;
    HIPCHK(hipSetDevice(p.device));
    NEED(h->have_state, DW_ESTATE, "no state uploaded");
    NEED(cur_quantised(h), DW_ESTATE, "the current state is an un-quantised upload; take a step first");
    dw_handle::Snapshot& sn = h->snap[slot];
    sn.valid = false;
    const size_t bn = (size_t)p.batch * p.n_agents;
    const size_t pb = sizeof(plane_t) * h->cells;
    const int rc = bn ? alloc_group(h, "a snapshot", {{sn.L, pb}, {sn.D, pb}, {sn.stats, h->stats_bytes},
                                                      {sn.idx, sizeof(int) * 2 * bn}, {sn.st, sizeof(double) * bn}})
                      : alloc_group(h, "a snapshot", {{sn.L, pb}, {sn.D, pb}, {sn.stats, h->stats_bytes}});
    if (rc) return rc;
    const bool keep_prev = h->stepped && h->unq != OWN_PREV;
    if (keep_prev)
        if (int prc = alloc_group(h, "a snapshot's previous state", {{sn.PL, pb}, {sn.PD, pb}})) return prc;
    CopyJobs J;
    J.n = 0;
    auto job = [&J](void* dst, const void* src, size_t bytes) { J.dst[J.n] = dst; J.src[J.n] = src; J.bytes[J.n] = bytes; ++J.n; };
    job(sn.L.get(), h->L16[h->cur].get(), pb);
    job(sn.D.get(), h->D16[h->cur].get(), pb);
    job(sn.stats.get(), h->stats2[h->sp].get(), h->stats_bytes);
    if (keep_prev) {
        job(sn.PL.get(), h->L16[1 - h->cur].get(), pb);
        job(sn.PD.get(), h->D16[1 - h->cur].get(), pb);
    }
    sn.stepped = h->stepped;
    sn.L_last = h->L_last;
    sn.L_per_world = h->L_per_world;
    sn.P_per_world = h->P_per_world;
    sn.unq = h->unq;
    sn.agents = bn && h->have_agents;
    if (sn.agents) {
        job(sn.idx.get(), h->idx.get(), sizeof(int) * 2 * bn);
        job(sn.st.get(), h->st.get(), sizeof(double) * bn);
    }
    if (int crc = launch_copy_regions(h, J)) return crc;
    sn.valid = true;
    return DW_OK;
}

int dw_snapshot_restore_slot(dw_handle* h, int32_t slot) {
    NEED(h, DW_EINVAL, "null handle");
    NEED(slot >= 0 && slot < DW_SNAPSHOT_SLOTS, DW_EINVAL, "snapshot slot out of range");
    const dw_params& p = h->prm;
    HIPCHK(hipSetDevice(p.device));
    const dw_handle::Snapshot& sn = h->snap[slot];
    NEED(sn.valid, DW_ESTATE, "no snapshot saved in this slot (or a later upload / dw_init_random invalidated it)");
    const size_t bn = (size_t)p.batch * p.n_agents;
    const size_t pb = sizeof(plane_t) * h->cells;
    CopyJobs J;
    J.n = 0;
    auto job = [&J](void* dst, const void* src, size_t bytes) { J.dst[J.n] = dst; J.src[J.n] = src; J.bytes[J.n] = bytes; ++J.n; };
    job(h->L16[h->cur].get(), sn.L.get(), pb);
    job(h->D16[h->cur].get(), sn.D.get(), pb);
    job(h->stats2[h->sp].get(), sn.stats.get(), h->stats_bytes);
    if (sn.agents) {
        job(h->idx.get(), sn.idx.get(), sizeof(int) * 2 * bn);
        job(h->st.get(), sn.st.get(), sizeof(double) * bn);
    }
    if (sn.stepped && sn.unq != OWN_PREV) {
        job(h->L16[1 - h->cur].get(), sn.PL.get(), pb);
        job(h->D16[1 - h->cur].get(), sn.PD.get(), pb);
    }
    if (int rc = launch_copy_regions(h, J)) return rc;
    HIPCHK(hipMemsetAsync(h->stats2[1 - h->sp].get(), 0, h->stats_bytes, h->stream));
    h->unq = sn.unq;
    h->stepped = sn.stepped;
    h->L_last = sn.L_last;
    h->L_per_world = sn.L_per_world;
    h->P_per_world = sn.P_per_world;
    return DW_OK;
}

int dw_snapshot_save(dw_handle* h) { return dw_snapshot_save_slot(h, 0); }
int dw_snapshot_restore(dw_handle* h) { return dw_snapshot_restore_slot(h, 0); }


int dw_set_stream(dw_handle* h, void* hip_stream) {
    NEED(h, DW_EINVAL, "null handle");
    HIPCHK(hipSetDevice(h->prm.device));
    HIPCHK(hipStreamSynchronize(h->stream));
    if (h->own_stream) HIPCHK(hipStreamDestroy(h->stream));
    h->stream = reinterpret_cast<hipStream_t>(hip_stream);
    h->own_stream = false;
    return DW_OK;
}

int dw_sync(dw_handle* h) {
    NEED(h, DW_EINVAL, "null handle");
    HIPCHK(hipSetDevice(h->prm.device));
    HIPCHK(hipStreamSynchronize(h->stream));
    return DW_OK;
}

int dw_timer_start(dw_handle* h) {
    NEED(h, DW_EINVAL, "null handle");
    HIPCHK(hipSetDevice(h->prm.device));
    HIPCHK(hipEventRecord(h->ev0, h->stream));
    return DW_OK;
}

int dw_timer_stop(dw_handle* h, float* elapsed_ms) {
    NEED(h && elapsed_ms, DW_EINVAL, "null argument");
    HIPCHK(hipSetDevice(h->prm.device));
    HIPCHK(hipEventRecord(h->ev1, h->stream));
    HIPCHK(hipEventSynchronize(h->ev1));
    HIPCHK(hipEventElapsedTime(elapsed_ms, h->ev0, h->ev1));
    return DW_OK;
}

int dw_device_planes(dw_handle* h, int which, void** light, void** dark) {
    NEED(h && light && dark, DW_EINVAL, "null argument");
    NEED(which == DW_STATE_CURRENT || which == DW_STATE_PREVIOUS, DW_EINVAL, "bad state selector");
    const int buf = which == DW_STATE_CURRENT ? h->cur : 1 - h->cur;
    NEED(which != DW_STATE_CURRENT || cur_quantised(h), DW_ESTATE,
         "the current state is an un-quantised upload: it has no binary16 planes before the first step");
    *light = h->L16[buf].get();
    *dark = h->D16[buf].get();
    return DW_OK;
}

int dw_kernel_info(dw_handle* h, char* buf, size_t buflen) {
    NEED(h && buf && buflen, DW_EINVAL, "null argument");
    const dw_params& p = h->prm;
    const StepPlan& pl = h->plan;
    const char* prec = p.precision == DW_PRECISION_EXACT ? "exact" : (p.precision == DW_PRECISION_FAST ? "fast" : "f64");
    static const char* const halo_name[] = {"rotate", "dpp-old", "general", "packed"};
    if (pl.kind == STEP_STREAM) {
        const StripGeom& g = pl.sgeom;
        snprintf(buf, buflen,
                 "step_stream_%s<halo=%s> wave-strip=%dx256 cells, register window + DPP neighbours, %d-row blocks in "
                 "flight%s, %d strips, grid=%d x 256 threads (4 strips each), XCD-chunked",
                 prec, halo_name[pl.halo], g.SR,
                 p.precision == DW_PRECISION_EXACT ? DW_STREAM_RB_EXACT : DW_STREAM_RB_FAST,
                 p.precision == DW_PRECISION_EXACT ? ", in-wave float64 fix-up from an LDS queue" : "", g.nstrips,
                 g.chunk * 8);
        if (pl.allow_fuse) {
            const size_t n = std::strlen(buf);
            snprintf(buf + n, buflen - n, "; dw_step_n fuses step pairs (step_stream_fused2%s%s",
                     p.precision == DW_PRECISION_EXACT ? "_exact" : "",
                     pl.seam_strips ? "_seam_pw, format buffer accesses" : (pl.fmt_planes ? "_fmt_pw, format buffer accesses" : ""));
            if (pl.seam_strips) {
                const size_t m = std::strlen(buf);
                snprintf(buf + m, buflen - m, ", seam strips: %d x %d columns + %d columns of %d row bands per wave", pl.seam_geom.ncs,
                         kSeamCols, pl.left_geom.cols_per_strip, pl.left_geom.wpr);
            }
            const size_t m = std::strlen(buf);
            snprintf(buf + m, buflen - m, ")");
        }
    } else if (pl.kind == STEP_TILED) {
        const int TR = (256 / pl.tcq) * pl.rpt;
        snprintf(buf, buflen,
                 "step_tiled<TCQ=%d,RPT=%d,%s> tile=%dx%d cells, %zu B LDS/workgroup, %d tiles, grid=%d x 256 threads, "
                 "XCD-chunked",
                 pl.tcq, pl.rpt, prec, TR, pl.tcq * 4, pl.tile_lds, pl.geom.ntiles, pl.geom.chunk * 8);
    } else {
        snprintf(buf, buflen, "step_generic<%s> one thread per cell, grid=(%d,%d) x 256 threads", prec,
                 (p.height * p.width + 255) / 256, p.batch);
    }
    {
        const size_t n = std::strlen(buf);
        snprintf(buf + n, buflen - n, pl.trace_pairs ? "; trace: step pairs" : "; trace: single steps");
    }
    {
        const size_t n = std::strlen(buf);
        snprintf(buf + n, buflen - n, pl.pw_stream ? "; per-world L: wave strips" : "; per-world L: generic");
    }
    {
        static const char* const form_name[] = {"launches per step", "workgroup (LDS)", "one wave per world"};
        const size_t n = std::strlen(buf);
        snprintf(buf + n, buflen - n, "; episode: %s; mlp episode: %s", form_name[episode_form(h)], form_name[episode_mlp_form(h)]);
    }
    {
        const size_t n = std::strlen(buf);
        snprintf(buf + n, buflen - n, "; ensemble episode: %s", episode_form(h) == EPISODE_WAVE ? "one wave per world" : "launches per step");
    }
    {
        const size_t n = std::strlen(buf);
        snprintf(buf + n, buflen - n, "; episode trace: %s", episode_form(h) == EPISODE_WAVE ? "one wave per world" : "launches per step");
    }
    if (pl.first_stream) {
        const size_t n = std::strlen(buf);
        snprintf(buf + n, buflen - n, "; first step: wave-strip=%dx256", pl.first_geom.SR);
    }
    if (h->sw.text[0]) {
        const size_t n = std::strlen(buf);
        snprintf(buf + n, buflen - n, "; switches[%s]", h->sw.text);
    }
    {
        const size_t n = std::strlen(buf);
        snprintf(buf + n, buflen - n, "; per-world constants: %s",
                 ensemble_pairs(h) ? "step pairs" : (pl.pw_stream ? "wave strips" : "generic"));
    }
    return DW_OK;
}

int dw_audit_tie_bound(dw_handle* h, double L, double out[4]) {
    NEED(h && out, DW_EINVAL, "null argument");
    const dw_params& p = h->prm;
    HIPCHK(hipSetDevice(p.device));
    NEED(h->have_state && cur_quantised(h), DW_ESTATE, "the audit needs a quantised current state");
    const StepPlan& pl = h->plan;
    int rc = ensure_scratch(h, 4 * sizeof(unsigned long long));
    if (rc) return rc;
    unsigned long long* d = reinterpret_cast<unsigned long long*>(h->scratch.get());
    HIPCHK(hipMemsetAsync(d, 0, 4 * sizeof(unsigned long long), h->stream));
    const dim3 g((unsigned)((p.height * p.width + 255) / 256), (unsigned)p.batch);
    hipLaunchKernelGGL(tie_audit, g, dim3(256), 0, h->stream, h->L16[h->cur].get(), h->D16[h->cur].get(), p.height, p.width,
                       derive_f32(p, L), make_f64(p, L), d, pl.sym_albedo && pl.kind == STEP_STREAM ? 1 : 0);
    HIPCHK(hipGetLastError());
    unsigned long long r[4];
    HIPCHK(hipMemcpyAsync(r, d, sizeof(r), hipMemcpyDeviceToHost, h->stream));
    HIPCHK(hipStreamSynchronize(h->stream));
    std::memcpy(&out[0], &r[0], sizeof(double));
    std::memcpy(&out[1], &r[1], sizeof(double));
    out[2] = (double)r[2];
    out[3] = (double)r[3];
    return DW_OK;
}

int dw_last_fixup_count(dw_handle* h, uint64_t* count) {
    NEED(h && count, DW_EINVAL, "null argument");
    HIPCHK(hipSetDevice(h->prm.device));
    std::vector<StatsDev> st((size_t)h->prm.batch + 1);
    HIPCHK(hipMemcpyAsync(st.data(), h->stats2[h->sp].get(), sizeof(StatsDev) * st.size(), hipMemcpyDeviceToHost, h->stream));
    HIPCHK(hipStreamSynchronize(h->stream));
    unsigned long long v = st[h->prm.batch].sum_l;
    for (int b = 0; b < h->prm.batch; ++b) v += st[b].reserved;
    *count = v;
    return DW_OK;
}

}
```

### therldaisyworld_amd/csrc/dw_plan.hpp

```cpp
#pragma once
#include <climits>
#include <cmath>
#include <cstddef>
#include <cstdio>
#include <cstdlib>
#include <cstring>

#include "../../include/daisyworld_hip.h"
#include "dw_types.hpp"

namespace dw {

struct Switches {
    bool no_sym = false, no_pack = false, no_fuse = false, no_ring = false, no_fmt_planes = false, no_seam_strips = false,
         no_episode_kernel = false,
         no_episode_wave = false, no_agent_fuse = false, no_agent_preapply = false, first_f64 = false,
         first_generic = false, force_rescan = false, test_hooks = false;
    int pack_min_strips = -1, strip_rows = 0, tile_rpt = 0, queue_cap = -1, mismatch_cap = -1, trace_rows = 0;
    double first_slack = -1.0;
    char kernel[16] = {0};
    char text[256] = {0};
};
inline const char* test_hook(const char* name) {
    return std::getenv("DW_TEST_HOOKS") ? std::getenv(name) : nullptr;
}
inline Switches read_switches() {
    Switches w;
    auto note = [&](const char* name, const char* val) {
        const size_t n = std::strlen(w.text);
        snprintf(w.text + n, sizeof(w.text) - n, "%s%s%s%s", n ? " " : "", name, val ? "=" : "", val ? val : "");
    };
    auto flag = [&](const char* name, bool& dst) { if (std::getenv(name)) { dst = true; note(name, nullptr); } };
    auto num = [&](const char* name, int& dst, bool test) {
        if (const char* e = test ? test_hook(name) : std::getenv(name)) { dst = std::atoi(e); note(name, e); }
    };
    w.test_hooks = std::getenv("DW_TEST_HOOKS") != nullptr;
    flag("DW_NO_SYM", w.no_sym); flag("DW_NO_PACK", w.no_pack); flag("DW_NO_FUSE", w.no_fuse); flag("DW_NO_RING", w.no_ring);
    flag("DW_NO_FMT_PLANES", w.no_fmt_planes); flag("DW_NO_SEAM_STRIPS", w.no_seam_strips);
    flag("DW_NO_EPISODE_KERNEL", w.no_episode_kernel); flag("DW_NO_EPISODE_WAVE", w.no_episode_wave);
    flag("DW_NO_AGENT_FUSE", w.no_agent_fuse); flag("DW_NO_AGENT_PREAPPLY", w.no_agent_preapply);
    flag("DW_FIRST_STEP_F64", w.first_f64); flag("DW_FIRST_GENERIC", w.first_generic);
    num("DW_PACK_MIN_STRIPS", w.pack_min_strips, false); num("DW_STRIP_ROWS", w.strip_rows, false);
    num("DW_TILE_RPT", w.tile_rpt, false);
    num("DW_TEST_QUEUE_CAP", w.queue_cap, true); num("DW_TEST_MISMATCH_CAP", w.mismatch_cap, true);
    num("DW_TEST_TRACE_ROWS", w.trace_rows, true);
    if (test_hook("DW_TEST_FORCE_RESCAN")) { w.force_rescan = true; note("DW_TEST_FORCE_RESCAN", nullptr); }
    if (const char* e = test_hook("DW_TEST_FIRST_SLACK")) { w.first_slack = std::atof(e); note("DW_TEST_FIRST_SLACK", e); }
    if (const char* e = std::getenv("DW_KERNEL")) { snprintf(w.kernel, sizeof(w.kernel), "%s", e); note("DW_KERNEL", e); }
    return w;
}

inline dw_params with_world_params(dw_params p, const dw_world_params& w) {
    p.p = w.p; p.g = w.g; p.S = w.S; p.sigma = w.sigma; p.gamma = w.gamma; p.q = w.q; p.q2 = w.q2; p.dt = w.dt;
    p.albedo_bare = w.albedo_bare; p.albedo_light = w.albedo_light; p.albedo_dark = w.albedo_dark;
    p.temp_optimal = w.temp_optimal;
    return p;
}
inline dw_world_params world_params_of(const dw_params& p) {
    return dw_world_params{p.p, p.g, p.S, p.sigma, p.gamma, p.q, p.q2, p.dt, p.albedo_bare, p.albedo_light, p.albedo_dark,
                           p.temp_optimal};
}
inline bool albedo_symmetric(double bare, double light, double dark) { return (dark - bare) == -(light - bare); }
inline bool worlds_symmetric(const dw_world_params* worlds, size_t B) {
    for (size_t b = 0; b < B; ++b)
        if (!albedo_symmetric(worlds[b].albedo_bare, worlds[b].albedo_light, worlds[b].albedo_dark)) return false;
    return true;
}

inline PhysF64 make_f64(const dw_params& p, double L) {
    PhysF64 P;
    P.p = p.p; P.g = p.g; P.S = p.S; P.sigma = p.sigma; P.gamma = p.gamma; P.q = p.q; P.q2 = p.q2;
    P.dt = p.dt; P.ab = p.albedo_bare; P.al = p.albedo_light; P.ad = p.albedo_dark;
    P.To = p.temp_optimal; P.L = L;
    const double e1 = std::exp(-1.0), e2 = std::exp(-2.0);
    const double s = 1.0 + 4.0 * e1 + 4.0 * e2;
    P.w0 = 1.0 / s; P.w1 = e1 / s; P.w2 = e2 / s;
    return P;
}

inline double cbeta_host(const dw_params& p) {
    const double cbeta = p.g * p.temp_optimal * p.temp_optimal;
    return cbeta > 1e-30 ? 1.0 / std::sqrt(cbeta) : 0x1p60;
}

inline void split_hi_lo(double v, double scale, float* hi, float* lo) {
    const double h = std::nearbyint(v * scale) / scale;
    *hi = (float)h;
    *lo = (float)(v - h);
}

inline float round_up(double v) {
    const float f = (float)v;
    return (double)f < v ? std::nextafterf(f, INFINITY) : f;
}

struct EConst { double c0l, c0d; };
inline EConst e_const(const dw_params& p, double L) {
    const double To4 = std::pow(p.temp_optimal, 4), K = p.S * L / p.sigma;
    const double e0 = K * (1.0 - p.albedo_bare * p.p) / To4 - 1.0;
    return EConst{e0 + p.q2 * (p.albedo_bare * p.p - p.albedo_light) / To4,
                  e0 + p.q2 * (p.albedo_bare * p.p - p.albedo_dark) / To4};
}

struct TieChain {
    double emin, emax, vlo;
    bool admissible;
    double ew;
    double kbmax;
    double pu, safety;
};
inline TieChain tie_chain(const dw_params& p, const EConst& c, double a1, double a2, double a3, double a4, double de) {
    const double u = std::ldexp(1.0, -24), kmax = 1000.0;
    TieChain t;
    const double pos = (std::fmax(a1, 0.0) + std::fmax(a2, 0.0)) * 8 * kmax + (std::fmax(a3, 0.0) + std::fmax(a4, 0.0)) * kmax;
    const double neg = (std::fmin(a1, 0.0) + std::fmin(a2, 0.0)) * 8 * kmax + (std::fmin(a3, 0.0) + std::fmin(a4, 0.0)) * kmax;
    t.emax = std::fmax(c.c0l, c.c0d) + pos;
    t.emin = std::fmin(c.c0l, c.c0d) + neg;
    const double vmin = 1.0 + t.emin, vmax = 1.0 + t.emax;
    t.admissible = vmin > 0.02;
    t.vlo = std::fmax(vmin, 0.02);
    const double smax = std::sqrt(std::fmax(vmax, t.vlo));
// ... 41 lines not shown
    P.c0ls = (float)((double)P.c0lh + P.c0ll); P.c0ds = (float)((double)P.c0dh + c0dl);
    const double kbe = cbeta_host(p);
    P.kbeta = (float)kbe;
    const PhysF64 P64 = make_f64(p, L);
    P.dw0 = (float)(p.dt * P64.w0); P.dw1 = (float)(p.dt * P64.w1); P.dw2 = (float)(p.dt * P64.w2);
    P.p = (float)p.p; P.ck = p.dt != 0.0 ? (float)(0.001 / p.dt) : 0.f;
    P.ngamma = (float)(-p.gamma);
    const double u = std::ldexp(1.0, -24);
    const double lo_mag = std::ldexp(1.0, -(hb + 1)) * 18.0 * kmax + std::ldexp(1.0, -(hb + 1));
    const double de_abs = 6.0 * u * lo_mag + 1e-9;
    const TieChain t = tie_chain(p, c0, a1, a2, a3, a4, de_abs);
    auto e_over_D2 = [&](double e) {
        const double v = std::fmax(1.0 + e, t.vlo), sv = std::sqrt(v), yv = std::sqrt(sv);
        const double D = kbe * (yv + 1.0) * (sv + 1.0);
        return std::fabs(e) / (D * D);
    };
    const double Ae = 2.0 * de_abs * std::fmax(e_over_D2(t.emin), e_over_D2(t.emax));
    double A0 = t.safety * (kmax * std::fabs(p.dt) * t.kbmax * Ae + 2e-6);
    if (!t.admissible) A0 = 1.0;
    const double eA = t.safety * 13.0 * u;
    const double eK0d = t.safety * (6.0 * std::fabs(p.p) + t.pu + t.kbmax + 8.0 * std::fabs(p.gamma)) * u;
    const double eK1d = t.safety * ((6.0 * std::fabs(p.p) + t.pu) * u + t.kbmax * (u + 2.0 * t.ew));
    P.tie_lo = (float)(0.5 - A0);
    if ((double)P.tie_lo > 0.5 - A0) P.tie_lo = std::nextafterf(P.tie_lo, -INFINITY);
    P.eA = round_up(eA);
    const float eK0 = round_up(eK0d), eK1 = round_up(eK1d);
    P.eK0s = p.dt < 0.0 ? eK0 : -eK0;
    P.eK1s = p.dt < 0.0 ? eK1 : -eK1;
    P.neK1s = -P.eK1s;
    P.eK01s = (float)((double)P.eK0s + (double)P.eK1s);
    if (std::fabs((double)P.eK01s) < std::fabs((double)P.eK0s + (double)P.eK1s))
        P.eK01s = std::nextafterf(P.eK01s, P.eK01s < 0.f ? -1.f : 1.f);
    return P;
}

inline void derive_f32_pair(const dw_params& p, double L1, double L2, PhysF32* P1, PhysF32* P2) {
    const PhysF32 a = derive_f32(p, L1), b = derive_f32(p, L2);
    const int hb = a.hi_bits < b.hi_bits ? a.hi_bits : b.hi_bits;
    *P1 = derive_f32(p, L1, hb);
    *P2 = derive_f32(p, L2, hb);
    const float tie_lo = P1->tie_lo < P2->tie_lo ? P1->tie_lo : P2->tie_lo;
    P1->tie_lo = tie_lo;
    P2->tie_lo = tie_lo;
}

inline FirstStepBound derive_first_bound(const dw_params& p, double L, const PhysF32& P, bool from_f64,
                                         double test_slack = -1.0) {
    const double u = std::ldexp(1.0, -24), iota = from_f64 ? u : 0.0;
    const double kmax = 1000.0;
    const double a1 = std::fabs((double)P.a1), a2 = std::fabs((double)P.a2), a3 = std::fabs((double)P.a3), a4 = std::fabs((double)P.a4);
    const EConst c0 = e_const(p, L);
    const double c0m = std::fmax(std::fabs(c0.c0l), std::fabs(c0.c0d));
    const double Mmax = (a1 + a2) * 8 * kmax + (a3 + a4) * kmax;
    const double de_max = (8.0 * u + iota) * Mmax + u * c0m;
    const TieChain t = tie_chain(p, c0, P.a1, P.a2, P.a3, P.a4, de_max);
    const double kbe = cbeta_host(p);
    const double Dmin = kbe * (std::sqrt(std::sqrt(t.vlo)) + 1.0) * (std::sqrt(t.vlo) + 1.0);
    const double kK = 5.0 * u + iota;
    const double safety = t.safety, pu = t.pu, kbmax = t.kbmax;
    FirstStepBound B;
    B.a1 = round_up(a1); B.a2 = round_up(a2); B.a3 = round_up(a3); B.a4 = round_up(a4);
    B.c_de = round_up(safety * (8.0 * u + iota) * (1.0 + 8.0 * u));
    B.c_c0 = round_up(safety * u * c0m);
    B.eK0 = round_up(safety * (pu + (kK + 2.0 * u) * std::fabs(p.p) + kbmax * u + ((kK + 3.0 * u) + u) * std::fabs(p.gamma)));
    B.eK1 = round_up(safety * (pu + (kK + 2.0 * u) * std::fabs(p.p) + kbmax * (u + 2.0 * t.ew)));
    B.cW = round_up(safety * 2.0 * kbmax / Dmin);
    B.eA = round_up(safety * ((kK + 3.0 * u) + u + (kK + u)));
    B.cS = round_up(safety * u);
    B.slack = t.admissible ? 4e-6f : 1.0f;
    if (test_slack > (double)B.slack) B.slack = (float)test_slack;
    return B;
}

enum StepKind { STEP_GENERIC, STEP_TILED, STEP_STREAM };
struct StepPlan {
    StepKind kind = STEP_GENERIC;
    int halo = 0;
    bool packed = false;
    bool allow_fuse = false;
    int fused_mode = kFusedOvl;
    bool fmt_planes = false;
    bool seam_strips = false;
    FusedGeom seam_geom{}, left_geom{};
    bool trace_pairs = false;
    bool sym_albedo = false;
    int tcq = 0, rpt = 0;
    Geom geom{};
    size_t tile_lds = 0;
    StripGeom sgeom{};
    FusedGeom fgeom{};
    int first_prec = 2;
    bool first_stream = false;
    FirstGeom first_geom{};
    bool need_fixq = false;
    bool pw_stream = false;
};

inline int halo_form(int W) { return W < 256 ? 3 : (W == 256 ? 0 : (W % 256 == 0 ? 1 : 2)); }

inline int strip_rows(long groups, int H, long target) {
    int sr = 64;
    while (sr > 8 && groups * ((H + sr - 1) / sr) < target) sr >>= 1;
    return H < sr ? H : sr;
}

inline int strip_rows_or_override(const Switches& sw, int cap, long groups, int H, long target) {
    if (sw.strip_rows < 1) return strip_rows(groups, H, target);
    const int want = sw.strip_rows < cap ? sw.strip_rows : cap;
    return H < want ? H : want;
}

inline long seam_waves_per_world(int W, int nrs) {
    const int n_full = W / kSeamCols, L = W - kSeamCols * n_full;
    const int G = L ? 64 / (L / 4 + 2) : 1;
    return (long)nrs * n_full + (L ? (nrs + G - 1) / G : 0);
}
inline bool seam_layout(const FusedGeom& f, FusedGeom* seam, FusedGeom* left) {
    const int n_full = f.W / kSeamCols, L = f.W - kSeamCols * n_full;
    if (n_full < 1 || seam_waves_per_world(f.W, f.nrs) >= (long)f.nrs * f.ncs) return false;
    auto launch = [](FusedGeom& g, long nstrips) {
        g.nstrips = (int)nstrips;
        g.nwg = (g.nstrips + 3) / 4;
        g.chunk = (g.nwg + 7) / 8;
    };
    *seam = f;
    seam->cols_per_strip = kSeamCols;
    seam->ncs = n_full;
    launch(*seam, (long)f.B * f.nrs * n_full);
    *left = *seam;
    left->cols_per_strip = L;
    left->lpw = L ? L / 4 + 2 : 64;
    left->wpr = 64 / left->lpw;
    launch(*left, L ? (long)f.B * ((f.nrs + left->wpr - 1) / left->wpr) : 0);
    return true;
}

inline StepPlan plan_steps(const dw_params& p, const Switches& sw) {
    StepPlan s;
    s.sym_albedo = albedo_symmetric(p.albedo_bare, p.albedo_light, p.albedo_dark) && !sw.no_sym;
    s.halo = halo_form(p.width);
    const int lpw = p.width / 4, wpr = lpw ? 64 / lpw : 0;
    const bool pack_shape = p.width >= 8 && p.width < 256 && wpr >= 1 && wpr * lpw * 10 >= 64 * 7 && !sw.no_pack;
    const long pack_strips = pack_shape ? (long)((p.batch + wpr - 1) / wpr) * ((p.height + 63) / 64) : 0;
    const bool packable = pack_shape && pack_strips >= (sw.pack_min_strips >= 0 ? sw.pack_min_strips : 512);
    const bool quads = p.precision != DW_PRECISION_F64 && p.width % 4 == 0;
    if (quads && (p.width >= 256 || packable) && std::strcmp(sw.kernel, "tiled") != 0) {
        s.kind = STEP_STREAM;
        s.packed = p.width < 256;
        StripGeom& g = s.sgeom;
        g.B = p.batch; g.H = p.height; g.W = p.width;
        g.ncs = (p.width + 255) / 256;
        g.lpw = s.packed ? lpw : 64;
        g.wpr = s.packed ? wpr : 1;
        const long groups = s.packed ? (p.batch + wpr - 1) / wpr : p.batch;
        g.SR = strip_rows_or_override(sw, INT_MAX, groups * g.ncs, p.height, 2048);
        g.nrs = (p.height + g.SR - 1) / g.SR;
        g.nstrips = (int)(groups * g.nrs * g.ncs);
        g.nwg = (g.nstrips + 3) / 4;
        g.chunk = (g.nwg + 7) / 8;
        g.qcap = kWaveQueueCap;
        int mcap = kMismatchCap;
        if (sw.queue_cap >= 0 && sw.queue_cap < kWaveQueueCap) g.qcap = sw.queue_cap;
        if (sw.mismatch_cap >= 0 && sw.mismatch_cap < kMismatchCap) mcap = sw.mismatch_cap;
        g.force_rescan = sw.force_rescan ? 1 : 0;
        s.allow_fuse = !sw.no_fuse;
        const bool ring = p.width == 1024 && !sw.no_ring;
        s.fused_mode = p.width <= 256 ? kFusedRot : (ring ? kFusedRing : kFusedOvl);
        FusedGeom& f = s.fgeom;
        f.B = p.batch; f.H = p.height; f.W = p.width;
        f.SR = g.SR;
        f.nrs = g.nrs;
        f.lpw = g.lpw; f.wpr = g.wpr;
        f.cols_per_strip = p.width <= 256 ? 256 : (ring ? 1024 : 248);
        f.ncs = s.packed ? 1 : (p.width + f.cols_per_strip - 1) / f.cols_per_strip;
        f.nstrips = (int)(groups * f.nrs * f.ncs);
        f.nwg = ring ? f.nstrips : (f.nstrips + 3) / 4;
        f.chunk = (f.nwg + 7) / 8;
        f.qcap = g.qcap;
        f.mcap = mcap;
        f.sure_need = 9 * p.n_agents + 9 * mcap + 1;
        s.trace_pairs = s.allow_fuse && !s.packed && s.fused_mode != kFusedRing;
        s.fmt_planes = p.precision == DW_PRECISION_FAST && s.allow_fuse && !s.packed && s.fused_mode == kFusedOvl && !sw.no_fmt_planes &&
                       (size_t)p.height * p.width * sizeof(plane_t) < ((size_t)1 << 31);
        s.seam_strips = s.fmt_planes && !sw.no_seam_strips && seam_layout(f, &s.seam_geom, &s.left_geom);
    } else if (quads && p.width >= 64) {
        s.kind = STEP_TILED;
        const int Wq = p.width / 4;
        if (Wq >= 64) {
            s.tcq = 64; s.rpt = 4;
            if (sw.tile_rpt == 2 || sw.tile_rpt == 4 || sw.tile_rpt == 8) s.rpt = sw.tile_rpt;
        }
        else if (Wq >= 32) { s.tcq = 32; s.rpt = 4; }
        else { s.tcq = 16; s.rpt = 2; }
        const int TR = (256 / s.tcq) * s.rpt;
        Geom& g = s.geom;
        g.B = p.batch; g.H = p.height; g.W = p.width; g.Wq = Wq;
        g.tiles_r = (p.height + TR - 1) / TR;
        g.tiles_c = (Wq + s.tcq - 1) / s.tcq;
        g.ntiles = p.batch * g.tiles_r * g.tiles_c;
        g.chunk = (g.ntiles + 7) / 8;
        g.qcap = kMaxFix;
        if (sw.queue_cap >= 0 && sw.queue_cap < kMaxFix) g.qcap = sw.queue_cap;
        s.tile_lds = (size_t)2 * (TR + 2) * (s.tcq + 2) * 4 * sizeof(float);
    }
    s.need_fixq = p.precision == DW_PRECISION_EXACT && s.kind == STEP_TILED;
    s.pw_stream = s.kind == STEP_STREAM && !s.packed;
    s.first_prec = p.precision == DW_PRECISION_FAST ? 1 : (p.precision == DW_PRECISION_EXACT && !sw.first_f64 ? 3 : 2);
    s.first_stream = (p.width % 256 == 0 || s.kind == STEP_STREAM) && s.first_prec != 2 && !sw.first_generic;
    if (s.first_stream) {
        FirstGeom& fg = s.first_geom;
        fg.B = p.batch; fg.H = p.height; fg.W = p.width;
        fg.lpw = s.packed ? lpw : 64;
        fg.wpr = s.packed ? wpr : 1;
        fg.ncs = s.packed ? 1 : (p.width + 255) / 256;
        const long groups = s.packed ? (p.batch + fg.wpr - 1) / fg.wpr : p.batch;
        fg.SR = strip_rows_or_override(sw, 64, groups * fg.ncs, p.height, 4096);
        fg.nrs = (p.height + fg.SR - 1) / fg.SR;
        fg.nstrips = (int)(groups * fg.nrs * fg.ncs);
    }
    return s;
}

}
```

### therldaisyworld_amd/csrc/dw_step_fused.hpp

```cpp
#pragma once
#include <type_traits>
#include "dw_step_stream.hpp"
#include "dw_types.hpp"

namespace dw {


template <typename TI>
__device__ inline unsigned int exact1_word(const TI* __restrict__ pL, const TI* __restrict__ pD, int H, int W,
                                           int r, int c, const PhysF64& Pa) {
    const int rr = wrap_near2(r, H), cc = wrap_near2(c, W);
    const int ru = rr == 0 ? H - 1 : rr - 1, rd = rr == H - 1 ? 0 : rr + 1;
    const int cl = cc == 0 ? W - 1 : cc - 1, cr = cc == W - 1 ? 0 : cc + 1;
    const int rows[3] = {ru, rr, rd}, cols[3] = {cl, cc, cr};
    unsigned int w1[9];
#pragma unroll
    for (int x = 0; x < 3; ++x)
#pragma unroll
        for (int y = 0; y < 3; ++y) {
            const size_t o = (size_t)rows[x] * W + cols[y];
            w1[x * 3 + y] = (unsigned)(float)pL[o] | ((unsigned)(float)pD[o] << 16);
        }
    const NewCoverF64 s1 = cell_f64_lean(Pa, w1);
    return (unsigned)dw_round3_k(s1.nl) | ((unsigned)dw_round3_k(s1.nd) << 16);
}

template <typename TI>
__device__ inline void exact2_cell(const TI* __restrict__ pL, const TI* __restrict__ pD, int H, int W, int r,
                                   int c, const PhysF64& Pa, const PhysF64& Pb, float& kl, float& kd) {
    unsigned int w2[9];
#pragma unroll
    for (int a = 0; a < 3; ++a)
#pragma unroll
        for (int e = 0; e < 3; ++e) {
            int rr = r + a - 1, cc = c + e - 1;
            rr = rr < 0 ? rr + H : (rr >= H ? rr - H : rr);
            cc = cc < 0 ? cc + W : (cc >= W ? cc - W : cc);
            const int ru = rr == 0 ? H - 1 : rr - 1, rd = rr == H - 1 ? 0 : rr + 1;
            const int cl = cc == 0 ? W - 1 : cc - 1, cr = cc == W - 1 ? 0 : cc + 1;
            const int rows[3] = {ru, rr, rd}, cols[3] = {cl, cc, cr};
            unsigned int w1[9];
#pragma unroll
            for (int x = 0; x < 3; ++x)
#pragma unroll
                for (int y = 0; y < 3; ++y) {
                    const size_t o = (size_t)rows[x] * W + cols[y];
                    w1[x * 3 + y] = (unsigned)(float)pL[o] | ((unsigned)(float)pD[o] << 16);
                }
            const NewCoverF64 s1 = cell_f64_lean(Pa, w1);
            w2[a * 3 + e] = (unsigned)dw_round3_k(s1.nl) | ((unsigned)dw_round3_k(s1.nd) << 16);
        }
    const NewCoverF64 s2 = cell_f64_lean(Pb, w2);
    kl = (float)dw_round3_k(s2.nl);
    kd = (float)dw_round3_k(s2.nd);
}

template <int MODE, bool EXACT, bool PACK = false, bool STATS = false, bool SYM = false, typename TI = plane_t,
          typename TO = plane_t, bool TRACE = false, bool FMT = false, int SEAM = kSeamNone>
__device__ __forceinline__ void fused2_body(const TI* __restrict__ inL, const TI* __restrict__ inD,
                                            TO* __restrict__ outL, TO* __restrict__ outD, const FusedGeom& G,
                                            const PhysF32& P1_, const PhysF32& P2_, const PhysF64& P64,
                                            const double& La, const double& Lb,
                                            unsigned long long* __restrict__ zero_me, int zero_n,
                                            unsigned int* __restrict__ pstats = nullptr, float thr_hi = 0.f,
                                            StatsDev* __restrict__ trace = nullptr, int trace_rescan = 0) {
    constexpr bool ROT = MODE == kFusedRot, RING = MODE == kFusedRing;
    static_assert(!RING || !PACK, "the ring exchange is written for un-packed worlds");
    static_assert(!TRACE || (!PACK && !STATS && !RING), "the trace form exists for un-packed overlapped / rotating strips");
    static_assert(SEAM == kSeamNone || FMT, "the seam strips exist for the format-access kernel");
    static_assert(!FMT || (MODE == kFusedOvl && !EXACT && !PACK && !STATS && !TRACE), "the format-access form exists for the plain float32 kernel on overlapped strips");
    __shared__ float s_edge[RING ? 2 * 4 * 8 : 1];
    __shared__ uint4 s_queue[EXACT ? 4 * kWaveQueueCap * 3 : 1];
    __shared__ unsigned int s_mm[EXACT ? 4 * kMismatchCap : 1];
    const int bid = blockIdx.x;
    const int wg = (bid & 7) * G.chunk + (bid >> 3);
    if (wg >= G.nwg) return;
    const int tid = threadIdx.x, wv = tid >> 6, lane = tid & 63;
    if (wg == 0)
        for (int i = tid; i < zero_n; i += 256) zero_me[i] = 0ull;
    const int s = RING ? wg : __builtin_amdgcn_readfirstlane(wg * 4 + wv);
    if (!RING && s >= G.nstrips) return;
    uint4* q = s_queue + (EXACT ? wv * kWaveQueueCap * 3 : 0);
    unsigned int* mm = s_mm + (EXACT ? wv * kMismatchCap : 0);
    const int spw = SEAM == kSeamLeft ? (G.nrs + G.wpr - 1) / G.wpr : G.nrs * G.ncs;
    const int b = s / spw;
    const int sw = s - b * spw;
    const int rs = SEAM == kSeamLeft ? sw * G.wpr : sw / G.ncs, cs = SEAM == kSeamLeft ? G.ncs : sw - rs * G.ncs;
    const int r0 = rs * G.SR;
    const int nr = min(G.SR, G.H - r0);
    const int band_g = SEAM == kSeamLeft ? min(lane / G.lpw, G.wpr - 1) : 0;
    const int band_j = SEAM == kSeamLeft ? min(lane - band_g * G.lpw, G.lpw - 1) : 0;
    const int band_rs = SEAM == kSeamLeft ? min(rs + band_g, G.nrs - 1) : 0;
    const int band_dr = SEAM == kSeamLeft ? (band_rs - rs) * G.SR : 0;
    const int band_nr = SEAM == kSeamLeft ? min(G.SR, G.H - band_rs * G.SR) : 0;
    const int pw = PACK ? lane / G.lpw : 0, pj = PACK ? lane - pw * G.lpw : 0;
    const int lsrc = PACK ? (pj == 0 ? lane + G.lpw - 1 : lane - 1) : 0;
    const int rsrc = PACK ? (pj == G.lpw - 1 ? lane - (G.lpw - 1) : lane + 1) : 0;
    auto world_off = [&](int lc) -> size_t {
        return (size_t)(PACK ? min(b * G.wpr + min((lc >> 2) / G.lpw, G.wpr - 1), G.B - 1) : b) * G.H * G.W;
    };
    const size_t woff = world_off(4 * lane);
    const int c00 = ROT ? 0 : (RING ? 256 * __builtin_amdgcn_readfirstlane(wv)
                                    : (SEAM == kSeamStrip ? cs * kSeamCols : (SEAM == kSeamLeft ? cs * kSeamCols - 4 : cs * 248 - 4)));
    int col = PACK ? 4 * pj : c00 + 4 * (SEAM == kSeamLeft ? band_j : lane);
    col = col < 0 ? col + G.W : col;
    col = col >= G.W ? col - G.W : col;
    int col_b = col + 2;
    if (SEAM == kSeamStrip && lane == 63) col_b = c00 == 0 ? G.W - 2 : c00 - 2;
    const bool writes = SEAM == kSeamStrip ? lane < 63
                      : SEAM == kSeamLeft ? (lane < G.wpr * G.lpw && rs + band_g < G.nrs && band_j >= 1 && band_j <= G.lpw - 2)
                      : PACK ? (pw < G.wpr && b * G.wpr + pw < G.B)
                             : ((ROT || RING) ? true : (lane >= 1 && lane <= 62 && cs * 248 + 4 * (lane - 1) < G.W));
    bool need1[4] = {true, true, true, true};
    if (PACK) { need1[0] = need1[1] = need1[2] = need1[3] = writes; }
    if (EXACT && !ROT && !RING) {
        const bool wl = __builtin_amdgcn_update_dpp(0, writes ? 1 : 0, kDppWaveShr1, 0xf, 0xf, false) != 0;
        const bool wr = __builtin_amdgcn_update_dpp(0, writes ? 1 : 0, kDppWaveShl1, 0xf, 0xf, false) != 0;
        need1[0] = writes || wl;
        need1[1] = writes;
        need1[2] = writes;
        need1[3] = writes || wr;
    }
    constexpr bool LANE_BOOLS = PACK || (STATS && MODE == kFusedOvl);
    using TieT = std::conditional_t<LANE_BOOLS, bool, unsigned long long>;
    TieT need1m[4], writes_m;
    if constexpr (LANE_BOOLS) {
        for (int i = 0; i < 4; ++i) need1m[i] = need1[i];
        writes_m = writes;
    } else {
        for (int i = 0; i < 4; ++i) need1m[i] = lane_mask(need1[i]);
        writes_m = lane_mask(writes);
    }
    const TI* pL = inL + woff;
    const TI* pD = inD + woff;

    dw_i32x4 fmt_inL, fmt_inD, fmt_outL, fmt_outD;
    int fmt_col = 0, fmt_row = 0, fmt_col_b = 0;
    if constexpr (FMT) {
        const unsigned int world_bytes = (unsigned int)(G.H * G.W) * 2u;
        fmt_inL = fmt_plane_rsrc(inL, b, world_bytes, SEAM == kSeamStrip ? kFmtRsrcPairs : kFmtRsrcQuads);
        fmt_inD = fmt_plane_rsrc(inD, b, world_bytes, SEAM == kSeamStrip ? kFmtRsrcPairs : kFmtRsrcQuads);
        fmt_outL = fmt_plane_rsrc(outL, b, world_bytes);
        fmt_outD = fmt_plane_rsrc(outD, b, world_bytes);
        fmt_col = col * 2;
        fmt_col_b = col_b * 2;
        fmt_row = G.W * 2;
    }
    struct RawIn { std::conditional_t<FMT, float4, dw_f16x4> l, d; };
    auto load_raw = [&](int rr) -> RawIn {
        RawIn w;
        if constexpr (SEAM == kSeamLeft) {
            int lr = min(rr + band_dr, r0 + band_dr + band_nr + 1);
            lr = lr < 0 ? lr + G.H : lr;
            lr = lr >= G.H ? lr - G.H : lr;
            w.l = fmt_load4(fmt_inL, fmt_col + lr * fmt_row, 0);
            w.d = fmt_load4(fmt_inD, fmt_col + lr * fmt_row, 0);
            return w;
        }
        rr = min(rr, r0 + nr + 1);
        rr = rr < 0 ? rr + G.H : rr;
        rr = rr >= G.H ? rr - G.H : rr;
        if constexpr (SEAM == kSeamStrip) {
            w.l = fmt_load2x2(fmt_inL, fmt_col, fmt_col_b, rr * fmt_row);
            w.d = fmt_load2x2(fmt_inD, fmt_col, fmt_col_b, rr * fmt_row);
// ... 2 lines not shown
            w.d = fmt_load4(fmt_inD, fmt_col, rr * fmt_row);
        } else {
            w.l = stream_load4_raw(pL + (size_t)rr * G.W + col);
            w.d = stream_load4_raw(pD + (size_t)rr * G.W + col);
        }
        return w;
    };
    auto pin_edge_sums = [&](Row4& L, Row4& D) {
        asm volatile("" : "+v"(L.h2[0]), "+v"(L.h2[3]), "+v"(D.h2[0]), "+v"(D.h2[3]));
    };
    auto nbrs = [&](const float4& v, float& a, float& c) {
        if (PACK) { a = __shfl(v.w, lsrc, 64); c = __shfl(v.x, rsrc, 64); }
        else if (ROT || SEAM == kSeamStrip) { a = dpp_mov_nb<kDppWaveRor1>(v.w); c = dpp_mov_nb<kDppWaveRol1>(v.x); }
        else { a = dpp_mov_nb<kDppWaveShr1>(v.w); c = dpp_mov_nb<kDppWaveShl1>(v.x); }
    };
    auto to_rows4 = [&](const float4& l, const float4& d, Row4& L, Row4& D) {
        float a, c;
        nbrs(l, a, c);
        L = make_row(l, a, c);
        nbrs(d, a, c);
        D = make_row(d, a, c);
    };
    int ring_par = 0;
    auto rows_ring = [&](const float4* v, Row4* const* out, auto NC) {
        constexpr int n = decltype(NC)::value;
        float* mine = s_edge + (ring_par * 4 + wv) * 8;
        if (lane == 63) {
#pragma unroll
            for (int i = 0; i < n; ++i) mine[i] = v[i].w;
        }
        if (lane == 0) {
#pragma unroll
            for (int i = 0; i < n; ++i) mine[4 + i] = v[i].x;
        }
        __syncthreads();
        const float* lw = s_edge + (ring_par * 4 + ((wv + 3) & 3)) * 8;
        const float* rw = s_edge + (ring_par * 4 + ((wv + 1) & 3)) * 8 + 4;
#pragma unroll
        for (int i = 0; i < n; ++i) {
            const float a = dpp_mov<kDppWaveShr1>(lw[i], v[i].w);
            const float c = dpp_mov<kDppWaveShl1>(rw[i], v[i].x);
            *out[i] = make_row(v[i], a, c);
        }
        ring_par ^= 1;
    };
    unsigned int nq = 0;
#ifndef DW_PIN_CONSTS
#define DW_PIN_CONSTS -1
#endif
    PhysF32 P1 = P1_, P2 = P2_;
    constexpr int PIN = DW_PIN_CONSTS < 0 ? (MODE == kFusedOvl ? 14 : (MODE == kFusedRing ? 8 : 0)) : DW_PIN_CONSTS;
    if constexpr (EXACT && PIN != 0 && !STATS && !PACK) {
        if constexpr ((PIN & 1) != 0) asm volatile("" : "+v"(P1.c0l), "+v"(P2.c0l));
        if constexpr ((PIN & 2) != 0) { asm volatile("" : "+v"(P1.pck)); P2.pck = P1.pck; }
        if constexpr ((PIN & 4) != 0) { asm volatile("" : "+v"(P1.eKb)); P2.eKb = P1.eKb; }
        if constexpr ((PIN & 8) != 0) { asm volatile("" : "+v"(P1.gt)); P2.gt = P1.gt; }
    }
    constexpr bool CHEAP = STATS && !PACK;
    float st_m1 = 0.f, st_x1 = 0.f;
    unsigned int st_c2 = 0, st_nmm = 0, st_c2w = 0;
    bool st_sure1 = false;
    const unsigned long long writes_mask = CHEAP ? lane_mask(writes) : 0ull;
    const float thr_c2 = EXACT ? thr_hi + 1.0f : thr_hi;
    dw_f32x2 tr_l1 = dw_f32x2(0.f), tr_d1 = dw_f32x2(0.f), tr_l2 = dw_f32x2(0.f), tr_d2 = dw_f32x2(0.f);
    int tr_m1 = 0, tr_m2 = 0;
    float tr_fix_l1 = 0.f, tr_fix_d1 = 0.f, tr_fix_l2 = 0.f, tr_fix_d2 = 0.f;
    float tr_x1 = 0.f, tr_new2 = 0.f, tr_low2 = 0.f;
    auto trace_patch2 = [&](float o, float n) {
        tr_new2 = fmaxf(tr_new2, n);
        if (n < o) tr_low2 = fmaxf(tr_low2, o);
    };
    auto trace_step1 = [&](const float* ol, const float* od, const TieT* tie) {
        tr_l1 += dw_f32x2{ol[0], ol[1]} + dw_f32x2{ol[2], ol[3]};
        tr_d1 += dw_f32x2{od[0], od[1]} + dw_f32x2{od[2], od[3]};
#pragma unroll
        for (int i = 0; i < 4; ++i) {
            if constexpr (EXACT) {
                const float m = fmaxf(ol[i], od[i]);
                tr_m1 = max(tr_m1, __float_as_int(tie_lane(tie[i]) ? 0.f : m));
            } else {
                asm("v_max3_i32 %0, %0, %1, %2" : "+v"(tr_m1) : "v"(ol[i]), "v"(od[i]));
            }
        }
    };
    auto trace_step2 = [&](const float* ol, const float* od) {
        tr_l2 += dw_f32x2{ol[0], ol[1]} + dw_f32x2{ol[2], ol[3]};
        tr_d2 += dw_f32x2{od[0], od[1]} + dw_f32x2{od[2], od[3]};
#pragma unroll
        for (int i = 0; i < 4; ++i) asm("v_max3_i32 %0, %0, %1, %2" : "+v"(tr_m2) : "v"(ol[i]), "v"(od[i]));
    };
    auto row_cells = [&](const PhysF32& P, const Row4& upL, const Row4& miL, const Row4& dnL, const Row4& upD,
                         const Row4& miD, const Row4& dnD, float* ol, float* od, TieT* tie,
                         const TieT* use, float* sure_max = nullptr) {
        cells4<EXACT, SYM, TieT>(P, upL, miL, dnL, upD, miD, dnD, ol, od, tie);
        if (EXACT) {
#pragma unroll
            for (int i = 0; i < 4; ++i) tie[i] = tie[i] & use[i];
        }
        if (STATS && sure_max) {
            if (CHEAP) {
                *sure_max = fmaxf(fmaxf(fmaxf(ol[0], ol[1]), fmaxf(ol[2], ol[3])), fmaxf(fmaxf(od[0], od[1]), fmaxf(od[2], od[3])));
            } else {
                float m = 0.f;
#pragma unroll
                for (int i = 0; i < 4; ++i) m = fmaxf(m, (EXACT && tie_lane(tie[i])) ? 0.f : fmaxf(ol[i], od[i]));
                *sure_max = m;
            }
        }
    };
    auto row_queue = [&](const Row4& upL, const Row4& miL, const Row4& dnL, const Row4& upD, const Row4& miD,
                         const Row4& dnD, const float* ol, const float* od, const TieT* tie, int kind,
                         int lrow) {
        if (EXACT && tie_mask(TieT(tie[0] | tie[1] | tie[2] | tie[3])) != 0ull) {
            queue_tie<0>(tie[0], nq, q, (unsigned)G.qcap, kind, lrow, 4 * lane, upL, miL, dnL, upD, miD, dnD, ol, od);
            queue_tie<1>(tie[1], nq, q, (unsigned)G.qcap, kind, lrow, 4 * lane, upL, miL, dnL, upD, miD, dnD, ol, od);
            queue_tie<2>(tie[2], nq, q, (unsigned)G.qcap, kind, lrow, 4 * lane, upL, miL, dnL, upD, miD, dnD, ol, od);
            queue_tie<3>(tie[3], nq, q, (unsigned)G.qcap, kind, lrow, 4 * lane, upL, miL, dnL, upD, miD, dnD, ol, od);
        }
    };
    auto stats_step2 = [&](float sm) {
        if (CHEAP) st_c2w += (unsigned int)__popcll(__builtin_amdgcn_fcmpf(sm, thr_c2, 2 ) & writes_mask);
        else if (writes && sm > thr_hi) st_c2 += 1u;
    };
    auto stats_step1 = [&](float sm, const float* ol, const float* od, const TieT* tie, bool rows_mine) {
        if (!rows_mine) return;
        if (writes) st_m1 = fmaxf(st_m1, sm);
        if (CHEAP) st_sure1 = st_sure1 || (__builtin_amdgcn_fcmpf(sm, thr_hi + 1.0f, 2 ) & writes_mask) != 0ull;
        if (CHEAP && EXACT) {
            const unsigned long long eq = __builtin_amdgcn_fcmpf(sm, thr_hi + 1.0f, 1 ) & writes_mask;
            if (__builtin_expect(eq != 0ull, 0)) {
                float m = 0.f;
#pragma unroll
                for (int i = 0; i < 4; ++i) m = fmaxf(m, tie_lane(tie[i]) ? 0.f : fmaxf(ol[i], od[i]));
                st_x1 = fmaxf(st_x1, in_mask(eq) ? m : 0.f);
            }
        }
    };
    const TieT use2[4] = {writes_m, writes_m, writes_m, writes_m};

    unsigned int nmm = 0;
    bool redo = false;
    const int flush_at = G.qcap >> 1;
    auto world_of = [&](int lc) -> int {
        return PACK ? min(b * G.wpr + min((lc >> 2) / G.lpw, G.wpr - 1), G.B - 1) : b;
    };
    auto grid_rc = [&](int lrow, int lc, int& gr, int& gc) {
        gr = r0 - 2 + lrow;
        gr = gr < 0 ? gr + G.H : (gr >= G.H ? gr - G.H : gr);
        gc = c00 + lc;
        gc = gc < 0 ? gc + G.W : (gc >= G.W ? gc - G.W : gc);
    };
    auto locate = [&](int lrow, int lc, size_t& wo, int& gr, int& gc) -> bool {
        grid_rc(lrow, lc, gr, gc);
        wo = world_off(lc);
        if (!PACK) return true;
        const int pwc = (lc >> 2) / G.lpw;
        gc = lc - pwc * G.W;
        return pwc < G.wpr && b * G.wpr + pwc < G.B;
    };
    auto is_output = [&](int lrow, int lc) -> bool {
        if (lrow < 2 || lrow > nr + 1) return false;
        if (PACK) return (lc >> 2) / G.lpw < G.wpr && b * G.wpr + (lc >> 2) / G.lpw < G.B;
        if (ROT || RING) return true;
        const int ln = lc >> 2;
        return lc >= 4 && lc < 252 && cs * 248 + 4 * (ln - 1) < G.W;
    };
// ... 24 lines not shown
                        const unsigned int f32v = unpack_ld(e2.w);
                        const float pl = (float)(f32v & 0xffffu), pd = (float)(f32v >> 16);
                        if (e0.x == 1u) {
                            tr_fix_l1 += (float)kl - pl;
                            tr_fix_d1 += (float)kd - pd;
                            tr_x1 = fmaxf(tr_x1, (float)(kl > kd ? kl : kd));
                        } else {
                            tr_fix_l2 += (float)kl - pl;
                            tr_fix_d2 += (float)kd - pd;
                            trace_patch2(pl, (float)kl);
                            trace_patch2(pd, (float)kd);
                        }
                    }
                    if (e0.x == 1u) {
                        mism = (kl | (kd << 16)) != unpack_ld(e2.w);
                        if (STATS && is_output((int)(where >> 16), (int)(where & 0xffffu))) {
                            const unsigned int mx = kl > kd ? kl : kd;
                            if (PACK) atomicMax(&pstats[2 * world_of((int)(where & 0xffffu))], mx);
                            else st_x1 = fmaxf(st_x1, (float)mx);
                        }
                    } else {
                        int gr, gc;
                        size_t wo;
                        locate((int)(where >> 16), (int)(where & 0xffffu), wo, gr, gc);
                        const size_t off = wo + (size_t)gr * G.W + gc;
                        outL[off] = (TO)(float)kl;
                        outD[off] = (TO)(float)kd;
                    }
                }
                const unsigned long long mask = lane_mask(mism);
                if (mism) {
                    const unsigned int slot = nmm + __builtin_amdgcn_mbcnt_hi((unsigned)(mask >> 32),
                                                                             __builtin_amdgcn_mbcnt_lo((unsigned)mask, 0u));
                    if (slot < (unsigned)G.mcap) mm[slot] = where;
                }
                nmm += (unsigned)__popcll(mask);
            }
            __builtin_amdgcn_fence(__ATOMIC_RELEASE, "wavefront");
            __builtin_amdgcn_wave_barrier();
        }
        nq = 0;
    };

    Row4 IL[3], ID[3], SL[3], SD[3];
    {
        const RawIn p0 = load_raw(r0 - 2), p1 = load_raw(r0 - 1), p2 = load_raw(r0);
        if constexpr (RING) {
            const float4 va[4] = {widen4(p0.l), widen4(p0.d), widen4(p1.l), widen4(p1.d)};
            const float4 vb[2] = {widen4(p2.l), widen4(p2.d)};
            Row4* const oa[4] = {&IL[0], &ID[0], &IL[1], &ID[1]};
            Row4* const ob[2] = {&IL[2], &ID[2]};
            rows_ring(va, oa, std::integral_constant<int, 4>{});
            rows_ring(vb, ob, std::integral_constant<int, 2>{});
        } else {
            to_rows4(widen4(p0.l), widen4(p0.d), IL[0], ID[0]);
            to_rows4(widen4(p1.l), widen4(p1.d), IL[1], ID[1]);
            to_rows4(widen4(p2.l), widen4(p2.d), IL[2], ID[2]);
        }
    }
    using U0 = std::integral_constant<int, 0>;
    using U1 = std::integral_constant<int, 1>;
    using U2 = std::integral_constant<int, 2>;
    auto iter = [&](auto U, auto D1, auto D2, int j, auto ST, auto MINE) {
        constexpr int u = decltype(U)::value;
        constexpr bool do1 = decltype(D1)::value, do2 = decltype(D2)::value;
        constexpr bool st_on = STATS && decltype(ST)::value;
        RawIn nx;
        if (do1) nx = load_raw(r0 + j);
        __builtin_amdgcn_sched_barrier(0);
        float l1[4], d1[4], l2[4], d2[4];
        TieT tie1[4], tie2[4];
        float sm1 = 0.f, sm2 = 0.f;
        if (do2)
            row_cells(P2, SL[u], SL[(u + 1) % 3], SL[(u + 2) % 3], SD[u], SD[(u + 1) % 3], SD[(u + 2) % 3], l2, d2, tie2,
                      use2, st_on ? &sm2 : nullptr);
        if (do1)
            row_cells(P1, IL[(u + 2) % 3], IL[u], IL[(u + 1) % 3], ID[(u + 2) % 3], ID[u], ID[(u + 1) % 3], l1, d1, tie1,
                      need1m, st_on ? &sm1 : nullptr);
        if (do2) {
            row_queue(SL[u], SL[(u + 1) % 3], SL[(u + 2) % 3], SD[u], SD[(u + 1) % 3], SD[(u + 2) % 3], l2, d2, tie2, 2,
                      j - 2);
            if (st_on) stats_step2(sm2);
            if constexpr (TRACE) trace_step2(l2, d2);
            if constexpr (SEAM == kSeamLeft) {
                if (writes && j - 4 < band_nr) {
                    const int voff = fmt_col + (r0 + band_dr + j - 4) * fmt_row;
                    fmt_store4(fmt_outL, voff, 0, make_float4(l2[0], l2[1], l2[2], l2[3]));
                    fmt_store4(fmt_outD, voff, 0, make_float4(d2[0], d2[1], d2[2], d2[3]));
                }
            } else if constexpr (FMT) {
                if (writes) {
                    fmt_store4(fmt_outL, fmt_col, (r0 + j - 4) * fmt_row, make_float4(l2[0], l2[1], l2[2], l2[3]));
                    fmt_store4(fmt_outD, fmt_col, (r0 + j - 4) * fmt_row, make_float4(d2[0], d2[1], d2[2], d2[3]));
                }
            } else if (writes) {
                const size_t off = woff + (size_t)(r0 + j - 4) * G.W + col;
                stream_store4(outL + off, make_float4(l2[0], l2[1], l2[2], l2[3]));
                stream_store4(outD + off, make_float4(d2[0], d2[1], d2[2], d2[3]));
            }
        }
        if (do1) {
            row_queue(IL[(u + 2) % 3], IL[u], IL[(u + 1) % 3], ID[(u + 2) % 3], ID[u], ID[(u + 1) % 3], l1, d1, tie1, 1, j);
            if (st_on) stats_step1(sm1, l1, d1, tie1, j >= 2 && j <= nr + 1);
            if constexpr (TRACE) {
                if (decltype(MINE)::value || (j >= 2 && j <= nr + 1)) trace_step1(l1, d1, tie1);
            }
            if constexpr (RING) {
                const float4 v[4] = {make_float4(l1[0], l1[1], l1[2], l1[3]), make_float4(d1[0], d1[1], d1[2], d1[3]),
                                     widen4(nx.l), widen4(nx.d)};
                Row4* const o[4] = {&SL[u], &SD[u], &IL[(u + 2) % 3], &ID[(u + 2) % 3]};
                rows_ring(v, o, std::integral_constant<int, 4>{});
            } else {
                to_rows4(make_float4(l1[0], l1[1], l1[2], l1[3]), make_float4(d1[0], d1[1], d1[2], d1[3]), SL[u], SD[u]);
                __builtin_amdgcn_sched_barrier(0);
                to_rows4(widen4(nx.l), widen4(nx.d), IL[(u + 2) % 3], ID[(u + 2) % 3]);
                if (!PACK) pin_edge_sums(IL[(u + 2) % 3], ID[(u + 2) % 3]);
            }
        }
    };
    using Yes = std::true_type;
    using No = std::false_type;
    iter(U1{}, Yes{}, No{}, 1, Yes{}, No{});
    iter(U2{}, Yes{}, No{}, 2, Yes{}, No{});
    iter(U0{}, Yes{}, No{}, 3, Yes{}, No{});
    const int jend = nr + 2;
    const int jloop = TRACE ? jend - 1 : jend;
    int j = 4;
    for (; j + 2 <= jloop; j += 3) {
        iter(U1{}, Yes{}, Yes{}, j, Yes{}, Yes{});
        iter(U2{}, Yes{}, Yes{}, j + 1, Yes{}, Yes{});
        iter(U0{}, Yes{}, Yes{}, j + 2, Yes{}, Yes{});
        if (EXACT && !STATS && __builtin_expect(nq >= (unsigned)flush_at, 0)) sweep_queue();
        if (CHEAP && st_sure1 && st_c2w >= (unsigned int)G.sure_need) { j += 3; break; }
    }
    if constexpr (CHEAP) {
        for (; j + 2 <= jend; j += 3) {
            iter(U1{}, Yes{}, Yes{}, j, No{}, No{});
            iter(U2{}, Yes{}, Yes{}, j + 1, No{}, No{});
            iter(U0{}, Yes{}, Yes{}, j + 2, No{}, No{});
        }
    }
    if (j <= jend) { iter(U1{}, Yes{}, Yes{}, j, Yes{}, No{}); ++j; }
    if (j <= jend) { iter(U2{}, Yes{}, Yes{}, j, Yes{}, No{}); ++j; }
    if constexpr (TRACE) {
        if (j <= jend) { iter(U0{}, Yes{}, Yes{}, j, Yes{}, No{}); ++j; }
    }
    if (j % 3 == 1) iter(U1{}, No{}, Yes{}, j, Yes{}, No{});
    else if (j % 3 == 2) iter(U2{}, No{}, Yes{}, j, Yes{}, No{});
    else iter(U0{}, No{}, Yes{}, j, Yes{}, No{});

    if (EXACT) {
        PhysF64 Pa = P64, Pb = P64;
        Pa.L = La;
        Pb.L = Lb;
        if (RING) {
            wait_row_stores_before_patching();
            __syncthreads();
        }
        sweep_queue();
        if (nmm > (unsigned)G.mcap) redo = true;
        if (RING) {
            wait_row_stores_before_patching();
            __syncthreads();
        }
        if (!redo) {
            unsigned int* s1 = reinterpret_cast<unsigned int*>(q);
            for (unsigned int m0 = 0; m0 < nmm; m0 += 2) {
                if constexpr (TRACE) wait_row_stores_before_patching();
                __builtin_amdgcn_wave_barrier();
                {
                    const unsigned int mi = lane / 25u, t = lane - mi * 25u;
// ... 75 lines not shown
            }
            for (int i = lane; i < nr * ncol; i += 64) {
                const int lrow = 2 + i / ncol, lc = (ROT ? 0 : (RING ? -1 : 4)) + i % ncol;
                if (!is_output(lrow, lc)) continue;
                int gr, gc;
                size_t wo;
                locate(lrow, lc, wo, gr, gc);
                float kl, kd;
                exact2_cell(inL + wo, inD + wo, G.H, G.W, gr, gc, Pa, Pb, kl, kd);
                const size_t off = wo + (size_t)gr * G.W + gc;
                outL[off] = (TO)kl;
                outD[off] = (TO)kd;
                if constexpr (TRACE) {
                    const unsigned int w1 = exact1_word(inL + wo, inD + wo, G.H, G.W, gr, gc, Pa);
                    const float l1 = (float)(w1 & 0xffffu), d1 = (float)(w1 >> 16);
                    tr_fix_l1 += l1;
                    tr_fix_d1 += d1;
                    tr_x1 = fmaxf(tr_x1, fmaxf(l1, d1));
                    tr_fix_l2 += kl;
                    tr_fix_d2 += kd;
                    tr_new2 = fmaxf(tr_new2, fmaxf(kl, kd));
                }
                if (STATS) {
                    const unsigned int w1 = exact1_word(inL + wo, inD + wo, G.H, G.W, gr, gc, Pa);
                    atomicMax(&pstats[2 * world_of(lc)], (w1 & 0xffffu) > (w1 >> 16) ? (w1 & 0xffffu) : (w1 >> 16));
                }
            }
            st_m1 = 0.f;
            st_x1 = 0.f;
            st_c2 = 0;
            st_c2w = 0;
        }
        st_nmm = nmm;
    }
    if constexpr (TRACE) {
        const bool own = writes && !redo;
        float l1 = own ? tr_l1.x + tr_l1.y : 0.f, d1 = own ? tr_d1.x + tr_d1.y : 0.f;
        float l2 = own ? tr_l2.x + tr_l2.y : 0.f, d2 = own ? tr_d2.x + tr_d2.y : 0.f;
        float m1 = own ? __int_as_float(tr_m1) : 0.f, m2 = own ? __int_as_float(tr_m2) : 0.f;
        if (EXACT) {
            l1 += tr_fix_l1; d1 += tr_fix_d1; l2 += tr_fix_l2; d2 += tr_fix_d2;
            m1 = fmaxf(m1, tr_x1);
        }
        m1 = wave_max(m1);
        m2 = wave_max(m2);
        if (EXACT) {
            m2 = fmaxf(m2, wave_max(tr_new2));
            const float lw = wave_max(tr_low2);
            if (__builtin_expect(!redo && (lw >= m2 || trace_rescan), 0)) {
                wait_row_stores_before_patching();
                float m = 0.f;
                for (int k0 = 0; k0 < nr; k0 += 8) {
                    unsigned long long wl[8], wd[8];
#pragma unroll
                    for (int jj = 0; jj < 8; ++jj) {
                        const int kk = min(k0 + jj, nr - 1);
                        const size_t off = woff + (size_t)(r0 + kk) * G.W + col;
                        wl[jj] = __hip_atomic_load(reinterpret_cast<const unsigned long long*>(outL + off), __ATOMIC_RELAXED,
                                                   __HIP_MEMORY_SCOPE_AGENT);
                        wd[jj] = __hip_atomic_load(reinterpret_cast<const unsigned long long*>(outD + off), __ATOMIC_RELAXED,
                                                   __HIP_MEMORY_SCOPE_AGENT);
                    }
#pragma unroll
                    for (int jj = 0; jj < 8; ++jj) {
                        const float4 fl = widen4(__builtin_bit_cast(dw_f16x4, wl[jj])), fd = widen4(__builtin_bit_cast(dw_f16x4, wd[jj]));
                        m = fmaxf(m, fmaxf(fmaxf(fmaxf(fl.x, fl.y), fmaxf(fl.z, fl.w)), fmaxf(fmaxf(fd.x, fd.y), fmaxf(fd.z, fd.w))));
                    }
                }
                m2 = wave_max(writes ? m : 0.f);
            }
        }
        l1 = wave_sum(l1); d1 = wave_sum(d1); l2 = wave_sum(l2); d2 = wave_sum(d2);
        if (lane == 0) {
            StatsDev* const t1 = trace + b;
            StatsDev* const t2 = t1 + G.B;
            atomicMax(&t1->max_k, (unsigned int)m1);
            atomicAdd(&t1->sum_l, (unsigned long long)l1);
            atomicAdd(&t1->sum_d, (unsigned long long)d1);
            atomicMax(&t2->max_k, (unsigned int)m2);
            atomicAdd(&t2->sum_l, (unsigned long long)l2);
            atomicAdd(&t2->sum_d, (unsigned long long)d2);
        }
    }
    if (STATS) {
        if (PACK) {
            float m = st_m1;
            unsigned int c = st_c2;
            if ((G.lpw & (G.lpw - 1)) == 0) {
                for (int o = G.lpw >> 1; o > 0; o >>= 1) {
                    m = fmaxf(m, __shfl_xor(m, o, 64));
                    c += (unsigned int)__shfl_xor((int)c, o, 64);
                }
            } else {
                for (int o = 1; o < G.lpw; ++o) {
                    const int src = min(lane + o, 63);
                    m = fmaxf(m, __shfl(st_m1, src, 64));
                    c += (unsigned int)__shfl((int)st_c2, src, 64);
                }
            }
            c = c > 9u * st_nmm ? c - 9u * st_nmm : 0u;
            if (pj == 0 && writes) {
                atomicMax(&pstats[2 * (b * G.wpr + pw)], (unsigned int)m);
                if (c) atomicAdd(&pstats[2 * (b * G.wpr + pw) + 1], c);
            }
        } else {
            const float mf = wave_max(st_m1), mx = wave_max(st_x1);
            const float m = (EXACT && !(mf > thr_hi + 1.0f)) ? mx : mf;
            unsigned int c = st_c2w;
            c = c > 9u * st_nmm ? c - 9u * st_nmm : 0u;
            if (lane == 0) {
                atomicMax(&pstats[2 * b], (unsigned int)m);
                if (c) atomicAdd(&pstats[2 * b + 1], c);
            }
        }
    }
}

#ifndef DW_FUSED_FAST_WAVES
#define DW_FUSED_FAST_WAVES 4
#endif
template <int MODE, bool PACK, bool STATS>
constexpr int fused_fast_waves() { return ((MODE == kFusedRing && STATS) || PACK) ? 3 : DW_FUSED_FAST_WAVES; }
template <int MODE, bool PACK = false, bool STATS = false>
__global__ __launch_bounds__(256)
__attribute__((amdgpu_waves_per_eu(fused_fast_waves<MODE, PACK, STATS>(), fused_fast_waves<MODE, PACK, STATS>())))
void step_stream_fused2(const plane_t* __restrict__ inL, const plane_t* __restrict__ inD,
                                                          plane_t* __restrict__ outL, plane_t* __restrict__ outD,
                                                          FusedGeom G, PhysF32 P1, PhysF32 P2,
                                                          unsigned long long* __restrict__ zero_me, int zero_n,
                                                          unsigned int* __restrict__ pstats, float thr_hi) {
    const PhysF64 dummy{};
    const double zero = 0.0;
    fused2_body<MODE, false, PACK, STATS>(inL, inD, outL, outD, G, P1, P2, dummy, zero, zero, zero_me, zero_n, pstats, thr_hi);
}

template <int MODE>
__global__ __launch_bounds__(256) __attribute__((amdgpu_waves_per_eu(DW_FUSED_FAST_WAVES, DW_FUSED_FAST_WAVES)))
void step_stream_fused2_fmt_pw(const plane_t* __restrict__ inL, const plane_t* __restrict__ inD,
                               plane_t* __restrict__ outL, plane_t* __restrict__ outD, FusedGeom G, PhysF32 P1, PhysF32 P2,
                               unsigned long long* __restrict__ zero_me, int zero_n) {
    const PhysF64 dummy{};
    const double zero = 0.0;
    fused2_body<MODE, false, false, false, false, plane_t, plane_t, false, true>(inL, inD, outL, outD, G, P1, P2, dummy, zero,
                                                                                  zero, zero_me, zero_n);
}

__global__ __launch_bounds__(256) __attribute__((amdgpu_waves_per_eu(DW_FUSED_FAST_WAVES, DW_FUSED_FAST_WAVES)))
void step_stream_fused2_seam_pw(const plane_t* __restrict__ inL, const plane_t* __restrict__ inD,
                                plane_t* __restrict__ outL, plane_t* __restrict__ outD, FusedGeom G, PhysF32 P1, PhysF32 P2,
                                unsigned long long* __restrict__ zero_me, int zero_n) {
    const PhysF64 dummy{};
    const double zero = 0.0;
    fused2_body<kFusedOvl, false, false, false, false, plane_t, plane_t, false, true, kSeamStrip>(inL, inD, outL, outD, G, P1, P2, dummy,
                                                                                                 zero, zero, zero_me, zero_n);
}
__global__ __launch_bounds__(256) __attribute__((amdgpu_waves_per_eu(DW_FUSED_FAST_WAVES, DW_FUSED_FAST_WAVES)))
void step_stream_fused2_left_pw(const plane_t* __restrict__ inL, const plane_t* __restrict__ inD,
                                plane_t* __restrict__ outL, plane_t* __restrict__ outD, FusedGeom G, PhysF32 P1, PhysF32 P2,
                                unsigned long long* __restrict__ zero_me, int zero_n) {
    const PhysF64 dummy{};
    const double zero = 0.0;
    fused2_body<kFusedOvl, false, false, false, false, plane_t, plane_t, false, true, kSeamLeft>(inL, inD, outL, outD, G, P1, P2, dummy,
                                                                                                zero, zero, zero_me, zero_n);
}

#ifndef DW_EXACT_PACK_WAVES
#define DW_EXACT_PACK_WAVES 3
#endif
template <int MODE, bool PACK, bool STATS>
constexpr int fused_exact_waves() {
    return (PACK && STATS) || (STATS && MODE == kFusedRing) ? 2 : (PACK ? DW_EXACT_PACK_WAVES : 3);
}
struct FusedExactArgs {
    const plane_t* inL; const plane_t* inD; plane_t* outL; plane_t* outD;
    FusedGeom G;
    PhysF32 P1; PhysLumF32 lum2;
    unsigned long long* zero_me; int zero_n;
    unsigned int* pstats; float thr_hi;
    PhysF64 P64; double La; double Lb;
};

template <int MODE, bool PACK = false, bool STATS = false, bool SYM = false>
__global__ __launch_bounds__(256)
__attribute__((amdgpu_waves_per_eu(fused_exact_waves<MODE, PACK, STATS>(), fused_exact_waves<MODE, PACK, STATS>())))
void step_stream_fused2_exact(FusedExactArgs A) {
    const FusedExactArgs& cold = kernarg_struct<FusedExactArgs>();
    const PhysF32 P2 = with_lum(A.P1, A.lum2);
    fused2_body<MODE, true, PACK, STATS, SYM>(A.inL, A.inD, A.outL, A.outD, A.G, A.P1, P2, cold.P64, cold.La, cold.Lb, A.zero_me,
                                             A.zero_n, A.pstats, A.thr_hi);
}

#ifndef DW_TRACE_FAST_WAVES
#define DW_TRACE_FAST_WAVES 3
#endif
#ifndef DW_TRACE_EXACT_WAVES
#define DW_TRACE_EXACT_WAVES 2
#endif
template <int MODE>
__global__ __launch_bounds__(256) __attribute__((amdgpu_waves_per_eu(DW_TRACE_FAST_WAVES, DW_TRACE_FAST_WAVES)))
void trace_pair_fast(const plane_t* __restrict__ inL, const plane_t* __restrict__ inD, plane_t* __restrict__ outL,
                     plane_t* __restrict__ outD, FusedGeom G, PhysF32 P1, PhysF32 P2,
                     unsigned long long* __restrict__ zero_me, int zero_n, StatsDev* __restrict__ trace) {
    const PhysF64 dummy{};
    const double zero = 0.0;
    fused2_body<MODE, false, false, false, false, plane_t, plane_t, true>(inL, inD, outL, outD, G, P1, P2, dummy, zero, zero,
                                                                           zero_me, zero_n, nullptr, 0.f, trace, 0);
}

struct TraceExactArgs {
    FusedExactArgs F;
    StatsDev* trace;
    int rescan;
};

template <int MODE, bool SYM = false>
__global__ __launch_bounds__(256) __attribute__((amdgpu_waves_per_eu(DW_TRACE_EXACT_WAVES, DW_TRACE_EXACT_WAVES)))
void trace_pair_exact(TraceExactArgs A) {
    const FusedExactArgs& cold = kernarg_struct<TraceExactArgs>().F;
    const PhysF32 P2 = with_lum(A.F.P1, A.F.lum2);
    fused2_body<MODE, true, false, false, SYM, plane_t, plane_t, true>(A.F.inL, A.F.inD, A.F.outL, A.F.outD, A.F.G, A.F.P1, P2,
                                                                       cold.P64, cold.La, cold.Lb, A.F.zero_me, A.F.zero_n,
                                                                       nullptr, 0.f, A.trace, A.rescan);
}

}
```

Before: 829.2 billion.

## Fuse the trailing single step into a reducing tail pair with deferred previous state

Multi-step runs used to finish with one or more standalone single steps after the fused pairs. Now a run with an even remainder ends in a fused tail pair whose kernels also produce the per-world statistics that the final single step would have written. The intermediate state is no longer materialised; a lagging flag makes every API entry point that might read it recompute the two steps on demand. This removes one full read/write pass over the grid at the end of each run, at the cost of extra shared-memory accumulation in the tail kernels and added bookkeeping complexity.

```diff
diff --git a/therldaisyworld_amd/csrc/dw_api.hip b/therldaisyworld_amd/csrc/dw_api.hip
--- a/therldaisyworld_amd/csrc/dw_api.hip
+++ b/therldaisyworld_amd/csrc/dw_api.hip
@@ -80,6 +80,8 @@
     double L_last = 0.0;
     bool L_per_world = false;
     bool P_per_world = false;
+    bool lagging = false;
+    double L_prev = 0.0;
     DevBuf<int> idx;
     DevBuf<double> st;
     DevBuf<int> action;
@@ -471,6 +473,7 @@
     h->sp = 1 - h->sp;
     h->unq = h->unq == OWN_CUR ? OWN_PREV : OWN_NONE;
     h->stepped = stepped;
+    h->lagging = false;
     h->L_last = L;
     h->L_per_world = per_world;
     h->P_per_world = per_world && per_world_constants;
@@ -480,6 +483,7 @@
 static void episode_done(dw_handle* h, double L_last, bool per_world) {
     h->unq = OWN_NONE;
     h->stepped = true;
+    h->lagging = false;
     h->L_last = per_world ? 0.0 : L_last;
     h->L_per_world = per_world;
     h->P_per_world = per_world;
@@ -511,6 +515,22 @@
     step_done(h, L, true);
     return DW_OK;
 }
+
+static int settle_previous(dw_handle* h) {
+    if (!h->lagging) return DW_OK;
+    HIPCHK(hipSetDevice(h->prm.device));
+    const double L1 = h->L_prev, L2 = h->L_last;
+    h->cur = 1 - h->cur;
+    if (int rc = launch_forward(h, L1)) {
+        h->cur = 1 - h->cur;
+        return rc;
+    }
+    return launch_forward(h, L2);
+}
+#define SETTLE(h)                                                                                                       \
+    do {                                                                                                                \
+        if (int settle_rc_ = settle_previous(h)) return settle_rc_;                                                     \
+    } while (0)
 
 static int launch_forward_pw(dw_handle* h, const PhysF32* row32, const PhysF64* row64, const FirstStepBound* rowfb, bool sym,
                              bool constants) {
@@ -598,7 +618,7 @@
 }
 
 static int launch_forward_fused2(dw_handle* h, double L1, double L2, unsigned int* pstats = nullptr,
-                                 float thr_hi = 0.f, StatsDev* trace = nullptr) {
+                                 float thr_hi = 0.f, StatsDev* trace = nullptr, bool tail = false) {
     const dw_params& p = h->prm;
     const StepPlan& pl = h->plan;
     const bool exact = p.precision == DW_PRECISION_EXACT;
@@ -624,6 +644,14 @@
             hipLaunchKernelGGL((trace_pair_fast<MODE>), grid, dim3(256), 0, h->stream, inL, inD, o.L, o.D, g, P1, P2, o.zero_me,
                                o.zero_n, trace);
         });
+    } else if (tail) {
+        NEED(pl.pair_tail && !pstats && !exact, DW_ESTATE, "the reducing tail pair exists for seam-strip plans only");
+        const FusedGeom &gs = pl.seam_geom, &gl = pl.left_geom;
+        hipLaunchKernelGGL(step_stream_fused2_seam_tail_pw, dim3((unsigned)gs.chunk * 8u), dim3(256), 0, h->stream, inL, inD, o.L,
+                           o.D, gs, P1, P2, o.zero_me, o.zero_n, o.stats);
+        if (gl.nstrips)
+            hipLaunchKernelGGL(step_stream_fused2_left_tail_pw, dim3((unsigned)gl.chunk * 8u), dim3(256), 0, h->stream, inL, inD,
+                               o.L, o.D, gl, P1, P2, o.zero_me, 0, o.stats);
     } else if (pl.seam_strips && !pstats && !exact) {
         const FusedGeom &gs = pl.seam_geom, &gl = pl.left_geom;
         hipLaunchKernelGGL(step_stream_fused2_seam_pw, dim3((unsigned)gs.chunk * 8u), dim3(256), 0, h->stream, inL, inD, o.L, o.D,
@@ -653,6 +681,10 @@
     }
     HIPCHK(hipGetLastError());
     step_done(h, L2, false);
+    if (tail) {
+        h->lagging = true;
+        h->L_prev = L1;
+    }
     return DW_OK;
 }
 
@@ -696,6 +728,7 @@
     h->unq = unq;
     h->have_state = true;
     h->stepped = false;
+    h->lagging = false;
     for (auto& sn : h->snap) sn.valid = false;
 }
 
@@ -838,6 +871,7 @@
 
 int dw_set_params(dw_handle* h, const dw_params* p) {
     NEED(h, DW_EINVAL, "null handle");
+    SETTLE(h);
     int rc = check_params(p);
     if (rc) return rc;
     const dw_params& o = h->prm;
@@ -875,6 +909,7 @@
 
 int dw_upload_state_f64(dw_handle* h, const double* light, const double* dark) {
     NEED(h && light && dark, DW_EINVAL, "null argument");
+    SETTLE(h);
     HIPCHK(hipSetDevice(h->prm.device));
     if (int arc = ensure_f64(h)) return arc;
     HIPCHK(hipMemcpyAsync(h->L64.get(), light, sizeof(double) * h->cells, hipMemcpyHostToDevice, h->stream));
@@ -888,6 +923,7 @@
 
 int dw_upload_state_f32(dw_handle* h, const float* light, const float* dark, int quantised) {
     NEED(h && light && dark, DW_EINVAL, "null argument");
+    SETTLE(h);
     HIPCHK(hipSetDevice(h->prm.device));
     const unsigned blocks = (unsigned)((h->cells + 255) / 256);
     if (quantised) {
@@ -919,6 +955,7 @@
 
 int dw_upload_agents(dw_handle* h, const int32_t* indices, const double* states) {
     NEED(h, DW_EINVAL, "null handle");
+    SETTLE(h);
     const dw_params& p = h->prm;
     HIPCHK(hipSetDevice(p.device));
     const size_t bn = (size_t)p.batch * p.n_agents;
@@ -940,6 +977,7 @@
 
 int dw_download_agents(dw_handle* h, int32_t* indices, double* states) {
     NEED(h, DW_EINVAL, "null handle");
+    SETTLE(h);
     const dw_params& p = h->prm;
     HIPCHK(hipSetDevice(p.device));
     const size_t bn = (size_t)p.batch * p.n_agents;
@@ -954,6 +992,7 @@
 
 int dw_init_random(dw_handle* h, uint64_t seed) {
     NEED(h, DW_EINVAL, "null handle");
+    SETTLE(h);
     HIPCHK(hipSetDevice(h->prm.device));
     if (int rc = ensure_u32(h)) return rc;
     if (int rc = init_random_into(h, seed, h->U32L.get(), h->U32D.get())) return rc;
@@ -963,6 +1002,7 @@
 
 int dw_init_random_quantised(dw_handle* h, uint64_t seed) {
     NEED(h, DW_EINVAL, "null handle");
+    SETTLE(h);
     HIPCHK(hipSetDevice(h->prm.device));
     if (int rc = init_random_into(h, seed, h->L16[h->cur].get(), h->D16[h->cur].get())) return rc;
     state_arrived(h, OWN_NONE);
@@ -975,6 +1015,7 @@
     NEED(h->have_state, DW_ESTATE, "no state");
     HIPCHK(hipSetDevice(h->prm.device));
     NEED(which == DW_STATE_CURRENT || which == DW_STATE_PREVIOUS, DW_EINVAL, "bad state selector");
+    if (which == DW_STATE_PREVIOUS) SETTLE(h);
     NEED(which == DW_STATE_CURRENT || h->stepped, DW_ESTATE, "no previous state before the first step");
     const int buf = which == DW_STATE_CURRENT ? h->cur : 1 - h->cur;
     const bool unq = (which == DW_STATE_CURRENT && h->unq == OWN_CUR) || (which == DW_STATE_PREVIOUS && h->unq == OWN_PREV);
@@ -1025,6 +1066,7 @@
 
 int dw_download_grid(dw_handle* h, double L_init, double* grid7) {
     NEED(h && grid7, DW_EINVAL, "null argument");
+    SETTLE(h);
     NEED(h->have_state, DW_ESTATE, "no state");
     NEED_SHARED_L(h, "dw_download_grid");
     HIPCHK(hipSetDevice(h->prm.device));
@@ -1041,6 +1083,7 @@
 int dw_download_caches(dw_handle* h, double L, double* temps, double* betas, double* growth,
                        double* temp_effective) {
     NEED(h, DW_EINVAL, "null handle");
+    SETTLE(h);
     NEED(h->have_state, DW_ESTATE, "no state");
     NEED_SHARED_CONSTANTS(h, "dw_download_caches");
     HIPCHK(hipSetDevice(h->prm.device));
@@ -1064,6 +1107,7 @@
 
 int dw_reduce_temperature(dw_handle* h, double L, dw_temp_stats* per_world) {
     NEED(h && per_world, DW_EINVAL, "null argument");
+    SETTLE(h);
     NEED(h->have_state, DW_ESTATE, "no state");
     NEED_SHARED_CONSTANTS(h, "dw_reduce_temperature");
     static_assert(sizeof(dw_temp_stats) == sizeof(TempStatsDev), "temperature record layout");
@@ -1079,6 +1123,7 @@
 
 int dw_update_agents(dw_handle* h, const int32_t* action, int32_t action_b, int32_t action_n) {
     NEED(h && action, DW_EINVAL, "null argument");
+    SETTLE(h);
     HIPCHK(hipSetDevice(h->prm.device));
     int rc = stage_host_actions(h, action, action_b, action_n);
     if (rc) return rc;
@@ -1107,6 +1152,7 @@
 
 int dw_upload_actions(dw_handle* h, const int32_t* action) {
     NEED(h && action, DW_EINVAL, "null argument");
+    SETTLE(h);
     HIPCHK(hipSetDevice(h->prm.device));
     const size_t bn = (size_t)h->prm.batch * h->prm.n_agents;
     if (bn) {
@@ -1118,6 +1164,7 @@
 
 int dw_download_actions(dw_handle* h, int32_t* action) {
     NEED(h && action, DW_EINVAL, "null argument");
+    SETTLE(h);
     HIPCHK(hipSetDevice(h->prm.device));
     const size_t bn = (size_t)h->prm.batch * h->prm.n_agents;
     if (bn) HIPCHK(hipMemcpyAsync(action, h->action.get(), sizeof(int) * bn, hipMemcpyDeviceToHost, h->stream));
@@ -1134,7 +1181,9 @@
     auto advance = [&]() { L += dL; L = L > max_L ? max_L : L; L = L < min_L ? min_L : L; };
     int s0 = 0;
     h->fused_launches = 0;
-    if (!use_device_actions && nsteps >= 1 && h->have_state && !cur_quantised(h)) {
+    const bool fuse = !use_device_actions && h->plan.allow_fuse && h->have_state;
+    const RunCut cut = cut_run(nsteps, use_device_actions || !h->have_state || cur_quantised(h), fuse, fuse && h->plan.pair_tail);
+    if (cut.first_single) {
         int rc = launch_forward(h, L);
         if (rc) return rc;
         advance();
@@ -1155,16 +1204,16 @@
         *L_io = L;
         return DW_OK;
     }
-    if (!use_device_actions && h->plan.allow_fuse && h->have_state && nsteps - s0 >= 3) {
+    if (cut.pairs + cut.tail_pair) {
         drop_unquantised_previous(h);
         HIPCHK(hipEventRecord(h->evf0, h->stream));
         int launched = 0;
-        while (nsteps - s0 >= 3) {
+        for (int i = 0; i < cut.pairs + cut.tail_pair; ++i) {
             const double L1 = L;
             advance();
             const double L2 = L;
             advance();
-            int rc = launch_forward_fused2(h, L1, L2);
+            int rc = launch_forward_fused2(h, L1, L2, nullptr, 0.f, nullptr, i == cut.pairs);
             if (rc) return rc;
             s0 += 2;
             launched += 1;
@@ -1331,11 +1380,13 @@
 
 int dw_step_n_trace(dw_handle* h, int32_t nsteps, const double* L_schedule, dw_world_stats* trace) {
     NEED(h && L_schedule && trace, DW_EINVAL, "null argument");
+    SETTLE(h);
     return run_series(h, nsteps, L_schedule, trace, nullptr, true, h->plan.trace_pairs);
 }
 
 int dw_step_n_trace_per_world(dw_handle* h, int32_t nsteps, const double* L_schedule, dw_world_stats* trace) {
     NEED(h && L_schedule, DW_EINVAL, "null argument");
+    SETTLE(h);
     return run_series(h, nsteps, L_schedule, trace, nullptr, false, false, PER_WORLD_L);
 }
 
@@ -1349,12 +1400,14 @@
                              dw_world_stats* trace, dw_temp_stats* temps) {
     static_assert(sizeof(dw_world_params) == 96, "dw_world_params layout");
     NEED(h && worlds && L_schedule, DW_EINVAL, "null argument");
+    SETTLE(h);
     return run_series(h, nsteps, L_schedule, trace, temps, false, ensemble_pairs(h), PER_WORLD_CONSTANTS, worlds);
 }
 
 int dw_step_n_trace_temperature(dw_handle* h, int32_t nsteps, const double* L_schedule, int per_world, dw_world_stats* trace,
                                 dw_temp_stats* temps) {
     NEED(h && L_schedule && temps, DW_EINVAL, "null argument");
+    SETTLE(h);
     return run_series(h, nsteps, L_schedule, trace, temps, false, false, per_world ? PER_WORLD_L : SHARED_L);
 }
 
@@ -1374,6 +1427,7 @@
 int dw_forward_f64(dw_handle* h, const double* light, const double* dark, double L, double* grid7,
                    double* temps, double* betas, double* growth, double* temp_effective) {
     NEED(h && light && dark && grid7, DW_EINVAL, "null argument");
+    SETTLE(h);
     const dw_params& p = h->prm;
     HIPCHK(hipSetDevice(p.device));
     const size_t n = h->cells;
@@ -1427,6 +1481,7 @@
 
 int dw_conv3x3_f64(dw_handle* h, const double* plane, const double kernel[9], double* out) {
     NEED(h && plane && kernel && out, DW_EINVAL, "null argument");
+    SETTLE(h);
     const dw_params& p = h->prm;
     HIPCHK(hipSetDevice(p.device));
     const size_t n = h->cells;
@@ -1449,6 +1504,7 @@
 
 int dw_stage_f64(dw_handle* h, int stage, const double* in, double* out, double L, const double kernel[9]) {
     NEED(h && in && out, DW_EINVAL, "null argument");
+    SETTLE(h);
     NEED(stage >= kStageAlbedo && stage <= kStageGrowth, DW_EINVAL, "bad stage %d", stage);
     NEED(kernel || stage > kStageDensity, DW_EINVAL, "the stencil stages need their 3x3 kernel");
     const dw_params& p = h->prm;
@@ -1476,6 +1532,7 @@
 
 int dw_get_obs(dw_handle* h, double L_init, double* obs) {
     NEED(h, DW_EINVAL, "null handle");
+    SETTLE(h);
     const dw_params& p = h->prm;
     HIPCHK(hipSetDevice(p.device));
     const size_t bn = (size_t)p.batch * p.n_agents;
@@ -1492,6 +1549,7 @@
 int dw_env_step(dw_handle* h, const int32_t* action, int32_t action_b, int32_t action_n, double L, double* obs,
                 double* reward, uint8_t* done) {
     NEED(h, DW_EINVAL, "null handle");
+    SETTLE(h);
     const dw_params& p = h->prm;
     HIPCHK(hipSetDevice(p.device));
     const size_t bn = (size_t)p.batch * p.n_agents;
@@ -1536,6 +1594,7 @@
 
 int dw_get_reward_done(dw_handle* h, double* reward, uint8_t* done) {
     NEED(h, DW_EINVAL, "null handle");
+    SETTLE(h);
     const dw_params& p = h->prm;
     HIPCHK(hipSetDevice(p.device));
     const int bn = p.batch * p.n_agents;
@@ -1576,6 +1635,7 @@
 
 int dw_policy_greedy(dw_handle* h, int mode) {
     NEED(h, DW_EINVAL, "null handle");
+    SETTLE(h);
     const dw_params& p = h->prm;
     HIPCHK(hipSetDevice(p.device));
     const int bn = p.batch * p.n_agents;
@@ -1589,6 +1649,7 @@
 
 int dw_policy_per_agent(dw_handle* h, const int32_t* agent_mode) {
     NEED(h && agent_mode, DW_EINVAL, "null argument");
+    SETTLE(h);
     const dw_params& p = h->prm;
     HIPCHK(hipSetDevice(p.device));
     const int bn = p.batch * p.n_agents;
@@ -1660,6 +1721,7 @@
 int dw_policy_mlp(dw_handle* h, const double* params, int32_t n_params, int32_t agent_begin, int32_t agent_end,
                   double L_init) {
     NEED(h && params, DW_EINVAL, "null argument");
+    SETTLE(h);
     HIPCHK(hipSetDevice(h->prm.device));
     NEED(n_params == 63 * 16 + 16 * 32 + 32 * 9, DW_EINVAL, "the MLP policy has 1808 parameters (63-16-32-9), got %d", n_params);
     return policy_mlp_impl(h, params, 1, nullptr, agent_begin, agent_end, L_init);
@@ -1668,6 +1730,7 @@
 int dw_policy_mlp_population(dw_handle* h, const double* params, int32_t n_members, const int32_t* world_member,
                              int32_t agent_begin, int32_t agent_end, double L_init) {
     NEED(h && params && world_member, DW_EINVAL, "null argument");
+    SETTLE(h);
     HIPCHK(hipSetDevice(h->prm.device));
     NEED(n_members >= 1, DW_EINVAL, "n_members < 1");
     return policy_mlp_impl(h, params, n_members, world_member, agent_begin, agent_end, L_init);
@@ -1677,6 +1740,7 @@
                        const int32_t* member_a, const int32_t* member_b, int32_t split, double L_init, double* reward,
                        uint8_t* done) {
     NEED(h && L_schedule, DW_EINVAL, "null argument");
+    SETTLE(h);
     const dw_params& p = h->prm;
     HIPCHK(hipSetDevice(p.device));
     NEED(nsteps >= 1 && nsteps <= 4096, DW_EINVAL, "nsteps must be in 1..4096");
@@ -1783,6 +1847,7 @@
 
 int dw_lifespan_reset(dw_handle* h) {
     NEED(h, DW_EINVAL, "null handle");
+    SETTLE(h);
     const dw_params& p = h->prm;
     HIPCHK(hipSetDevice(p.device));
     const size_t bn = (size_t)p.batch * (p.n_agents > 0 ? p.n_agents : 1);
@@ -1794,6 +1859,7 @@
 
 int dw_lifespan_accumulate(dw_handle* h, uint32_t threshold_k) {
     NEED(h, DW_EINVAL, "null handle");
+    SETTLE(h);
     const dw_params& p = h->prm;
     HIPCHK(hipSetDevice(p.device));
     HIPCHK(hipMemsetAsync(h->n_alive.get(), 0, sizeof(int), h->stream));
@@ -1806,6 +1872,7 @@
 
 int dw_lifespan_download(dw_handle* h, int32_t* done_at, int32_t* agents_done_at, int32_t* n_worlds_alive) {
     NEED(h, DW_EINVAL, "null handle");
+    SETTLE(h);
     const dw_params& p = h->prm;
     HIPCHK(hipSetDevice(p.device));
     if (done_at) HIPCHK(hipMemcpyAsync(done_at, h->done_at.get(), sizeof(int) * p.batch, hipMemcpyDeviceToHost, h->stream));
@@ -1821,6 +1888,7 @@
                    const uint8_t* use_table, const int8_t* table, uint32_t threshold_k, uint8_t* world_alive,
                    uint8_t* agent_ok) {
     NEED(h && L_schedule, DW_EINVAL, "null argument");
+    SETTLE(h);
     NEED(policy_mode >= 0 && policy_mode <= 3, DW_EINVAL, "bad policy mode");
     return run_episode_impl(h, nsteps, L_schedule, policy_mode, use_table, table, threshold_k, world_alive, agent_ok);
 }
@@ -2051,6 +2119,7 @@
                          const uint8_t* use_table, const int8_t* table, uint32_t threshold_k, uint8_t* world_alive,
                          uint8_t* agent_ok, dw_world_stats* trace) {
     NEED(h && L_schedule, DW_EINVAL, "null argument");
+    SETTLE(h);
     NEED(trace, DW_EINVAL, "dw_run_episode_trace needs a trace array");
     NEED(policy_mode >= 0 && policy_mode <= 3, DW_EINVAL, "bad policy mode");
     return run_episode_impl(h, nsteps, L_schedule, policy_mode, use_table, table, threshold_k, world_alive, agent_ok, trace);
@@ -2060,6 +2129,7 @@
                             const uint8_t* use_table, const int8_t* table, uint32_t threshold_k, uint8_t* world_alive,
                             uint8_t* agent_ok) {
     NEED(h && worlds && L_schedule, DW_EINVAL, "null argument");
+    SETTLE(h);
     NEED(policy_mode >= 0 && policy_mode <= 3, DW_EINVAL, "bad policy mode");
     const dw_params& p = h->prm;
     HIPCHK(hipSetDevice(p.device));
@@ -2143,6 +2213,7 @@
 
 int dw_snapshot_save_slot(dw_handle* h, int32_t slot) {
     NEED(h, DW_EINVAL, "null handle");
+    SETTLE(h);
     NEED(slot >= 0 && slot < DW_SNAPSHOT_SLOTS, DW_EINVAL, "snapshot slot out of range");
     const dw_params& p = h->prm;
     HIPCHK(hipSetDevice(p.device));
@@ -2186,6 +2257,7 @@
 
 int dw_snapshot_restore_slot(dw_handle* h, int32_t slot) {
     NEED(h, DW_EINVAL, "null handle");
+    SETTLE(h);
     NEED(slot >= 0 && slot < DW_SNAPSHOT_SLOTS, DW_EINVAL, "snapshot slot out of range");
     const dw_params& p = h->prm;
     HIPCHK(hipSetDevice(p.device));
@@ -2223,6 +2295,7 @@
 
 int dw_set_stream(dw_handle* h, void* hip_stream) {
     NEED(h, DW_EINVAL, "null handle");
+    SETTLE(h);
     HIPCHK(hipSetDevice(h->prm.device));
     HIPCHK(hipStreamSynchronize(h->stream));
     if (h->own_stream) HIPCHK(hipStreamDestroy(h->stream));
@@ -2257,6 +2330,7 @@
 int dw_device_planes(dw_handle* h, int which, void** light, void** dark) {
     NEED(h && light && dark, DW_EINVAL, "null argument");
     NEED(which == DW_STATE_CURRENT || which == DW_STATE_PREVIOUS, DW_EINVAL, "bad state selector");
+    if (which == DW_STATE_PREVIOUS) SETTLE(h);
     const int buf = which == DW_STATE_CURRENT ? h->cur : 1 - h->cur;
     NEED(which != DW_STATE_CURRENT || cur_quantised(h), DW_ESTATE,
          "the current state is an un-quantised upload: it has no binary16 planes before the first step");
@@ -2287,8 +2361,8 @@
                      pl.seam_strips ? "_seam_pw, format buffer accesses" : (pl.fmt_planes ? "_fmt_pw, format buffer accesses" : ""));
             if (pl.seam_strips) {
                 const size_t m = std::strlen(buf);
-                snprintf(buf + m, buflen - m, ", seam strips: %d x %d columns + %d columns of %d row bands per wave", pl.seam_geom.ncs,
-                         kSeamCols, pl.left_geom.cols_per_strip, pl.left_geom.wpr);
+                snprintf(buf + m, buflen - m, ", seam strips: %d x %d columns + %d columns of %d row bands per wave%s", pl.seam_geom.ncs,
+                         kSeamCols, pl.left_geom.cols_per_strip, pl.left_geom.wpr, pl.pair_tail ? ", even runs end on a reducing pair" : "");
             }
             const size_t m = std::strlen(buf);
             snprintf(buf + m, buflen - m, ")");
@@ -2337,11 +2411,16 @@
         snprintf(buf + n, buflen - n, "; per-world constants: %s",
                  ensemble_pairs(h) ? "step pairs" : (pl.pw_stream ? "wave strips" : "generic"));
     }
+    if (h->lagging) {
+        const size_t n = std::strlen(buf);
+        snprintf(buf + n, buflen - n, "; predecessor deferred");
+    }
     return DW_OK;
 }
 
 int dw_audit_tie_bound(dw_handle* h, double L, double out[4]) {
     NEED(h && out, DW_EINVAL, "null argument");
+    SETTLE(h);
     const dw_params& p = h->prm;
     HIPCHK(hipSetDevice(p.device));
     NEED(h->have_state && cur_quantised(h), DW_ESTATE, "the audit needs a quantised current state");
diff --git a/therldaisyworld_amd/csrc/dw_plan.hpp b/therldaisyworld_amd/csrc/dw_plan.hpp
--- a/therldaisyworld_amd/csrc/dw_plan.hpp
+++ b/therldaisyworld_amd/csrc/dw_plan.hpp
@@ -13,7 +13,7 @@
 
 struct Switches {
     bool no_sym = false, no_pack = false, no_fuse = false, no_ring = false, no_fmt_planes = false, no_seam_strips = false,
-         no_episode_kernel = false,
+         no_pair_tail = false, no_episode_kernel = false,
          no_episode_wave = false, no_agent_fuse = false, no_agent_preapply = false, first_f64 = false,
          first_generic = false, force_rescan = false, test_hooks = false;
     int pack_min_strips = -1, strip_rows = 0, tile_rpt = 0, queue_cap = -1, mismatch_cap = -1, trace_rows = 0;
@@ -37,6 +37,7 @@
     w.test_hooks = std::getenv("DW_TEST_HOOKS") != nullptr;
     flag("DW_NO_SYM", w.no_sym); flag("DW_NO_PACK", w.no_pack); flag("DW_NO_FUSE", w.no_fuse); flag("DW_NO_RING", w.no_ring);
     flag("DW_NO_FMT_PLANES", w.no_fmt_planes); flag("DW_NO_SEAM_STRIPS", w.no_seam_strips);
+    flag("DW_NO_PAIR_TAIL", w.no_pair_tail);
     flag("DW_NO_EPISODE_KERNEL", w.no_episode_kernel); flag("DW_NO_EPISODE_WAVE", w.no_episode_wave);
     flag("DW_NO_AGENT_FUSE", w.no_agent_fuse); flag("DW_NO_AGENT_PREAPPLY", w.no_agent_preapply);
     flag("DW_FIRST_STEP_F64", w.first_f64); flag("DW_FIRST_GENERIC", w.first_generic);
@@ -244,6 +245,7 @@
     bool fmt_planes = false;
     bool seam_strips = false;
     FusedGeom seam_geom{}, left_geom{};
+    bool pair_tail = false;
     bool trace_pairs = false;
     bool sym_albedo = false;
     int tcq = 0, rpt = 0;
@@ -295,6 +297,21 @@
     left->wpr = 64 / left->lpw;
     launch(*left, L ? (long)f.B * ((f.nrs + left->wpr - 1) / left->wpr) : 0);
     return true;
+}
+
+struct RunCut { int first_single, pairs, tail_pair, singles; };
+inline RunCut cut_run(int nsteps, bool quantised, bool fuse, bool tail) {
+    RunCut c{0, 0, 0, 0};
+    c.first_single = !quantised && nsteps >= 1 ? 1 : 0;
+    const int r = nsteps - c.first_single;
+    if (fuse && tail && r >= 2 && r % 2 == 0) {
+        c.pairs = r / 2 - 1;
+        c.tail_pair = 1;
+    } else if (fuse && r >= 3) {
+        c.pairs = (r - 1) / 2;
+    }
+    c.singles = r - 2 * (c.pairs + c.tail_pair);
+    return c;
 }
 
 inline StepPlan plan_steps(const dw_params& p, const Switches& sw) {
@@ -345,6 +362,7 @@
         s.fmt_planes = p.precision == DW_PRECISION_FAST && s.allow_fuse && !s.packed && s.fused_mode == kFusedOvl && !sw.no_fmt_planes &&
                        (size_t)p.height * p.width * sizeof(plane_t) < ((size_t)1 << 31);
         s.seam_strips = s.fmt_planes && !sw.no_seam_strips && seam_layout(f, &s.seam_geom, &s.left_geom);
+        s.pair_tail = s.seam_strips && !sw.no_pair_tail;
     } else if (quads && p.width >= 64) {
         s.kind = STEP_TILED;
         const int Wq = p.width / 4;
diff --git a/therldaisyworld_amd/csrc/dw_step_fused.hpp b/therldaisyworld_amd/csrc/dw_step_fused.hpp
--- a/therldaisyworld_amd/csrc/dw_step_fused.hpp
+++ b/therldaisyworld_amd/csrc/dw_step_fused.hpp
@@ -56,7 +56,7 @@
 }
 
 template <int MODE, bool EXACT, bool PACK = false, bool STATS = false, bool SYM = false, typename TI = plane_t,
-          typename TO = plane_t, bool TRACE = false, bool FMT = false, int SEAM = kSeamNone>
+          typename TO = plane_t, bool TRACE = false, bool FMT = false, int SEAM = kSeamNone, bool TAIL = false>
 __device__ __forceinline__ void fused2_body(const TI* __restrict__ inL, const TI* __restrict__ inD,
                                             TO* __restrict__ outL, TO* __restrict__ outD, const FusedGeom& G,
                                             const PhysF32& P1_, const PhysF32& P2_, const PhysF64& P64,
@@ -68,10 +68,12 @@
     static_assert(!RING || !PACK, "the ring exchange is written for un-packed worlds");
     static_assert(!TRACE || (!PACK && !STATS && !RING), "the trace form exists for un-packed overlapped / rotating strips");
     static_assert(SEAM == kSeamNone || FMT, "the seam strips exist for the format-access kernel");
+    static_assert(!TAIL || FMT, "the reducing tail form exists for the format-access kernels");
     static_assert(!FMT || (MODE == kFusedOvl && !EXACT && !PACK && !STATS && !TRACE), "the format-access form exists for the plain float32 kernel on overlapped strips");
     __shared__ float s_edge[RING ? 2 * 4 * 8 : 1];
     __shared__ uint4 s_queue[EXACT ? 4 * kWaveQueueCap * 3 : 1];
     __shared__ unsigned int s_mm[EXACT ? 4 * kMismatchCap : 1];
+    __shared__ dw_f32x2 s_tail[TAIL ? 256 : 1];
     const int bid = blockIdx.x;
     const int wg = (bid & 7) * G.chunk + (bid >> 3);
     if (wg >= G.nwg) return;
@@ -80,6 +82,7 @@
         for (int i = tid; i < zero_n; i += 256) zero_me[i] = 0ull;
     const int s = RING ? wg : __builtin_amdgcn_readfirstlane(wg * 4 + wv);
     if (!RING && s >= G.nstrips) return;
+    if constexpr (TAIL) s_tail[tid] = dw_f32x2(0.f);
     uint4* q = s_queue + (EXACT ? wv * kWaveQueueCap * 3 : 0);
     unsigned int* mm = s_mm + (EXACT ? wv * kMismatchCap : 0);
     const int spw = SEAM == kSeamLeft ? (G.nrs + G.wpr - 1) / G.wpr : G.nrs * G.ncs;
@@ -248,6 +251,12 @@
                 asm("v_max3_i32 %0, %0, %1, %2" : "+v"(tr_m1) : "v"(ol[i]), "v"(od[i]));
             }
         }
+    };
+    auto tail_step2 = [&](const float* ol, const float* od) {
+        const dw_f32x2 pl = dw_f32x2{ol[0], ol[1]} + dw_f32x2{ol[2], ol[3]}, pd = dw_f32x2{od[0], od[1]} + dw_f32x2{od[2], od[3]};
+        s_tail[tid] += dw_f32x2{pl.x + pl.y, pd.x + pd.y};
+#pragma unroll
+        for (int i = 0; i < 4; ++i) asm("v_max3_i32 %0, %0, %1, %2" : "+v"(tr_m2) : "v"(ol[i]), "v"(od[i]));
     };
     auto trace_step2 = [&](const float* ol, const float* od) {
         tr_l2 += dw_f32x2{ol[0], ol[1]} + dw_f32x2{ol[2], ol[3]};
@@ -438,11 +447,13 @@
                       j - 2);
             if (st_on) stats_step2(sm2);
             if constexpr (TRACE) trace_step2(l2, d2);
+            if constexpr (TAIL && SEAM != kSeamLeft) tail_step2(l2, d2);
             if constexpr (SEAM == kSeamLeft) {
                 if (writes && j - 4 < band_nr) {
                     const int voff = fmt_col + (r0 + band_dr + j - 4) * fmt_row;
                     fmt_store4(fmt_outL, voff, 0, make_float4(l2[0], l2[1], l2[2], l2[3]));
                     fmt_store4(fmt_outD, voff, 0, make_float4(d2[0], d2[1], d2[2], d2[3]));
+                    if constexpr (TAIL) tail_step2(l2, d2);
                 }
             } else if constexpr (FMT) {
                 if (writes) {
@@ -684,6 +695,16 @@
             atomicAdd(&t2->sum_d, (unsigned long long)d2);
         }
     }
+    if constexpr (TAIL) {
+        const float m2 = wave_max(writes ? __int_as_float(tr_m2) : 0.f);
+        const float l2 = wave_sum(writes ? s_tail[tid].x : 0.f), d2 = wave_sum(writes ? s_tail[tid].y : 0.f);
+        if (lane == 0) {
+            StatsDev* const t2 = trace + b;
+            atomicMax(&t2->max_k, (unsigned int)m2);
+            atomicAdd(&t2->sum_l, (unsigned long long)l2);
+            atomicAdd(&t2->sum_d, (unsigned long long)d2);
+        }
+    }
     if (STATS) {
         if (PACK) {
             float m = st_m1;
@@ -766,6 +787,25 @@
                                                                                                 zero, zero, zero_me, zero_n);
 }
 
+__global__ __launch_bounds__(256) __attribute__((amdgpu_waves_per_eu(DW_FUSED_FAST_WAVES, DW_FUSED_FAST_WAVES)))
+void step_stream_fused2_seam_tail_pw(const plane_t* __restrict__ inL, const plane_t* __restrict__ inD,
+                                     plane_t* __restrict__ outL, plane_t* __restrict__ outD, FusedGeom G, PhysF32 P1, PhysF32 P2,
+                                     unsigned long long* __restrict__ zero_me, int zero_n, StatsDev* __restrict__ stats) {
+    const PhysF64 dummy{};
+    const double zero = 0.0;
+    fused2_body<kFusedOvl, false, false, false, false, plane_t, plane_t, false, true, kSeamStrip, true>(
+        inL, inD, outL, outD, G, P1, P2, dummy, zero, zero, zero_me, zero_n, nullptr, 0.f, stats, 0);
+}
+__global__ __launch_bounds__(256) __attribute__((amdgpu_waves_per_eu(DW_FUSED_FAST_WAVES, DW_FUSED_FAST_WAVES)))
+void step_stream_fused2_left_tail_pw(const plane_t* __restrict__ inL, const plane_t* __restrict__ inD,
+                                     plane_t* __restrict__ outL, plane_t* __restrict__ outD, FusedGeom G, PhysF32 P1, PhysF32 P2,
+                                     unsigned long long* __restrict__ zero_me, int zero_n, StatsDev* __restrict__ stats) {
+    const PhysF64 dummy{};
+    const double zero = 0.0;
+    fused2_body<kFusedOvl, false, false, false, false, plane_t, plane_t, false, true, kSeamLeft, true>(
+        inL, inD, outL, outD, G, P1, P2, dummy, zero, zero, zero_me, zero_n, nullptr, 0.f, stats, 0);
+}
+
 #ifndef DW_EXACT_PACK_WAVES
 #define DW_EXACT_PACK_WAVES 3
 #endif
```

Result: no change. 832.1 billion, median of 6 (+0.4%).
